# wei-zeng98/piano-a2s

Measured on AMD Instinct MI355X. Metric: training clips/sec (12 s, 5-bar), higher is better.
Workload: dtype f32

## Files before the change

### include/a2s.h

```cpp
#ifndef A2S_H
#define A2S_H
#include <stddef.h>
#include <stdint.h>
#ifdef __cplusplus
extern "C" {
#endif

#define A2S_OK 0
#define A2S_ERR_ARG (-1)
#define A2S_ERR_HIP (-2)
#define A2S_ERR_WORKSPACE (-3)

const char* a2s_last_error(void);
int a2s_version(void);
long long a2s_launch_count(void);

int a2s_gemm_f32(void* stream, int M, int N, int K, float alpha, const float* A, long sAm, long sAk,
                 const float* B, long sBk, long sBn, float beta, float* C, long ldc, const float* bias, int act,
                 int batch, long bsA, long bsB, long bsC, int splitk, float* workspace, size_t workspace_bytes);
int a2s_gemm_f32_affine(void* stream, int M, int N, int K, float alpha, const float* A, long sAm, long sAk, const float* B, long sBk,
                        long sBn, float beta, float* C, long ldc, const float* bias, int act, int batch, long bsA, long bsB, long bsC,
                        int splitk, float* workspace, size_t workspace_bytes, const float* a_scale, const float* a_shift, int a_period,
                        const float* b_scale, const float* b_shift, int b_period);
int a2s_gemm_f32_bnstats(void* stream, int M, int N, int K, const float* A, long sAm, long sAk, const float* B, long sBk, long sBn, float* C, long ldc,
                         const float* y, const float* mean, const float* invstd, const float* scale, const float* shift, int period, float* partial);
int a2s_gemm_f32_affine_scaled(void* stream, int M, int N, int K, float alpha, const float* A, long sAm, long sAk, const float* B, long sBk,
                               long sBn, float beta, float* C, long ldc, const float* bias, int act, int batch, long bsA, long bsB, long bsC,
                               int splitk, float* workspace, size_t workspace_bytes, const float* a_scale, const float* a_shift, int a_period,
                               const float* b_scale, const float* b_shift, int b_period, const float* a_absmax, const float* b_absmax);
int a2s_gemm_f32_bnstats_scaled(void* stream, int M, int N, int K, const float* A, long sAm, long sAk, const float* B, long sBk, long sBn, float* C, long ldc,
                                const float* y, const float* mean, const float* invstd, const float* scale, const float* shift, int period, float* partial,
                                const float* a_absmax, const float* b_absmax);
int a2s_linear_dgrad_bnstats(void* stream, int M, int N, int K, const float* dz, long lda, const float* Wt, float* da, long ldc, const float* y,
                             const float* mean, const float* invstd, const float* scale, const float* shift, int period, float* partial,
                             const float* dz_absmax, const float* w_absmax, float* workspace, size_t workspace_bytes, float* da_absmax_out);
int a2s_linear_fwd(void* stream, int M, int N, int K, const float* y, long lda, const float* W, float* z, long ldc, const float* scale, const float* shift,
                   int period, const float* y_absmax, const float* w_absmax, float* workspace, size_t workspace_bytes);
int a2s_linear_fwd_eligible(int M, int N, int K, int period);
int a2s_linear_wgrad(void* stream, int M, int N, int K, const float* dz, long ldz, const float* y, long lda, float* G, long ldg, const float* scale,
                     const float* shift, int period, const float* dz_absmax, const float* y_absmax, float* workspace, size_t workspace_bytes);
size_t a2s_linear_wgrad_ws_bytes(int M, int K);
int a2s_linear_wgrad_eligible(int M, int N, int K, int period);
int a2s_tallk_wgrad(void* stream, int M, int Np, int K, const float* P, long ldp, const float* A, long lda, float* G, long ldg, int transposed, float* bias,
                    const float* p_absmax, const float* a_absmax, float* workspace, size_t workspace_bytes);
size_t a2s_tallk_wgrad_ws_bytes(int M, int Np, int K);
int a2s_tallk_wgrad_eligible(int M, int Np, int K, long ldp, long lda, long ldg, int transposed);
size_t a2s_linear_dgrad_ws_bytes(int N, int K);
int a2s_linear_dgrad_blocks(int M);
int a2s_linear_dgrad_eligible(int M, int N, int K, int period);
int a2s_absmax(void* stream, const float* x, long n, float* out);
int a2s_gemm_bnstats_blocks(int M, int period);
size_t a2s_gemm_workspace_bytes(int M, int N, int batch, int splitk);
int a2s_gemm_pick_splitk(int M, int N, int K, int batch);
void a2s_gemm_debug_tile(int cfg);
int a2s_debug_set(const char* key, int value);
int a2s_debug_get(const char* key);
int a2s_env_check(void);
int a2s_persist_abort_latch(void* device_word);

int a2s_conv3x3(void* stream, const float* x, const float* w, float* y, const float* in_scale, const float* in_shift,
                float* stat_partial, int B, int T, int F, int Cin, int Cout, int flip, float* workspace);
int a2s_conv3x3_ranged(void* stream, const float* x, const float* w, float* y, const float* in_scale, const float* in_shift, const float* in_absmax,
                       float* stat_partial, float* out_absmax, int B, int T, int F, int Cin, int Cout, float* workspace);
int a2s_conv3x3_stat_blocks(int B, int T, int F, int Cin);
int a2s_conv3x3_dgrad_bnstats(void* stream, const float* dy, const float* w, float* g, const float* yl, const float* yl_mean, const float* yl_invstd,
                              const float* yl_scale, const float* yl_shift, float* stat_partial, int B, int T, int F, int Cin, int Cout,
                              float* workspace);
int a2s_bn_bwd_from_partial(void* stream, const float* g, const float* x, const float* mean, const float* invstd, const float* scale, const float* shift,
                            float* dgamma, float* dbeta, float* dx , const float* partial, int nblocks, float* c12, long rows, int C, int F);
int a2s_conv3x3_dgrad_bnstats_scaled(void* stream, const float* dy, const float* w, float* g, const float* yl, const float* yl_mean, const float* yl_invstd,
                                     const float* yl_scale, const float* yl_shift, float* stat_partial, int B, int T, int F, int Cin, int Cout,
                                     float* workspace, const float* dy_absmax);
int a2s_conv3x3_dgrad_bnstats_ranged(void* stream, const float* dy, const float* w, float* g, const float* yl, const float* yl_mean, const float* yl_invstd,
                                     const float* yl_scale, const float* yl_shift, float* stat_partial, int B, int T, int F, int Cin, int Cout,
                                     float* workspace, const float* dy_absmax, float* g_absmax_out);
int a2s_bn_bwd_from_partial_amax(void* stream, const float* g, const float* x, const float* mean, const float* invstd, const float* scale, const float* shift,
                                 float* dgamma, float* dbeta, float* dx, const float* partial, int nblocks, float* c12, long rows, int C, int F,
                                 float* dx_absmax);
size_t a2s_conv3x3_workspace_floats(int Cin);
int a2s_bn_finalize(void* stream, const float* partial, int nblocks, int C, double count, const float* gamma,
                    const float* beta, float* running_mean, float* running_var, long long* num_batches_tracked,
                    float* mean, float* invstd, float* scale, float* shift, float eps, float momentum, int training);
int a2s_bn_relu_apply(void* stream, const float* x, float* y, const float* scale, const float* shift, long n, int C, int F);
int a2s_col_stats(void* stream, const float* x, float* partial, long rows, int C, int rows_per_block);
int a2s_bn1d_relu_dropout(void* stream, const float* x, float* y, const float* scale, const float* shift,
                          const uint8_t* keep_mask, float inv_keep, long n, int C);

int a2s_gru_gates_fwd(void* stream, const float* gi, long ldgi, const float* gh, long ldgh, const float* hprev, long ldhp,
                      float* hout, long ldho, float* hout2, long ldho2, float* save, int R, int H);
int a2s_gru_seq_fwd(void* stream, const float* gi_all, long gi_bstride, long gi_tstride, const float* w_hh,
                    const float* b_hh, float* out, long out_bstride, long out_tstride, float* hbuf, float* gh,
                    float* save, float* hn, int B, int T, int H, int reverse, float* workspace, size_t workspace_bytes);

int a2s_attn_step_fwd(void* stream, const float* keys, const float* enc, const float* q, long ldq, const float* v,
                      float* ctx, long ldctx, float* ctx2, long ldctx2, float* attw, int B, int T, int H,
                      const int* n_done, int n_rows_total, float* workspace);
int a2s_attn_step_fwd_rows(void* stream, const float* keys, const float* enc, const float* q, long ldq, const float* v, float* ctx,
                           long ldctx, float* ctx2, long ldctx2, float* attw, int R, int T, int H, float* workspace, int n_clips,
                           const int* clip_order, const int* clip_rank, const int* row_until, int n_active, int step);
size_t a2s_attn_workspace_floats(int B, int T, int H);
size_t a2s_attn_workspace_floats_fused(int n_clips, int T, int H, int groups);

int a2s_log_softmax_rows(void* stream, const float* x, long ldx, float* y, long ldy, int* argmax_out, int R, int V);
int a2s_embed_rows(void* stream, const float* table, const long long* ids64, const int* ids32, long id_stride,
                   int const_id, float* out, long ldo, int col0, int R, int E, const uint8_t* keep_mask, float inv_keep);

typedef struct a2s_note_dec_args {
    const float* attn_w; const float* attn_b; const float* attn_v;
    const float* w_ih; const float* w_hh; const float* b_ih; const float* b_hh;
    const float* out_w; const float* out_b; const float* emb;
    const float* keys; const float* enc;
    float* h; float* x; float* q; float* gates; float* attw; float* o;
    float* gh; float* gi; float* logits;
    float* probs; long probs_bstride;
    const long long* gt; long gt_bstride;
    const uint8_t* tf_flags;
    const uint8_t* drop; float inv_keep;
    int* argmax_out; long am_bstride;
    int* eos_seen; long long* lengths; int* n_done;
    int* steps_exec;
    float* attn_ws;
    float* gemm_ws; size_t gemm_ws_bytes;
    int* t_base;
    const int* clip_order;
    const int* clip_rank;
    const int* row_until;
    const int* n_active;
    int n_clips;
    const int* m_active;
    const int* row_list;
    const int* n_rows_active;
    int R, T, H, E, V, steps, poll, eos_id;
    int use_graph;
    float* step_ws; size_t step_ws_floats;
    const int* tf_flags_dev;
    float* persist_ws; size_t persist_ws_bytes;
} a2s_note_dec_args;
int a2s_note_decoder_fwd(void* stream, const a2s_note_dec_args* args, int* steps_done);
int a2s_grammar_argmax_rows(void* stream, const float* x, long ldx, float* y, long ldy, const signed char* next_state, int n_states, int* row_state,
                            int* choice_out, int R, int V);
int a2s_note_decoder_fwd_grammar(void* stream, const a2s_note_dec_args* args, const signed char* next_state, int n_states, int* row_state, int* steps_done);
int a2s_grammar_launches(void);
#define A2S_BEAM_MAX 4
typedef struct a2s_beam_args {
    int K; float alpha;
    const signed char* next_state; int n_states;
    int pad_id;
    int* row_state;
    float* score; int* finished;
    int* done_count;
    int* token_hist; int* parent_hist; float* score_hist;
    float* probs_scratch;
    int* ids_out; long long* lengths_out; float* score_out;
} a2s_beam_args;
int a2s_note_decoder_fwd_beam(void* stream, const a2s_note_dec_args* args, const a2s_beam_args* beam, int* steps_done);
int a2s_beam_step(void* stream, const a2s_beam_args* beam, const float* logits, long ldl, const float* emb, float* xnext, long ldx, float* h, int h_cols,
                  float* q, int q_cols, int* n_done, int* steps_exec, int B, int V, int E, int t, int max_steps, int eos_id);
int a2s_beam_backtrack(void* stream, const a2s_beam_args* beam, float* probs, long probs_bstride, const int* steps_exec, int B, int V, int max_steps, int eos_id);
int a2s_beam_launches(void);
typedef struct a2s_align_args {
    float* attw_step;
    int* peak; float* weight; float* centroid;
    long out_stride;
    const signed char* next_state; int n_states;
    int* row_state;
} a2s_align_args;
int a2s_attn_align_rows(void* stream, const float* attw, long ldw, int R, int T, int* peak_out, float* weight_out, float* centroid_out, long out_stride);
int a2s_note_decoder_fwd_align(void* stream, const a2s_note_dec_args* args, const a2s_align_args* align, int* steps_done);
int a2s_align_launches(void);

int a2s_render_notes(void* stream, const int* programs, int rows_per_clip, int n_samples, float* wave, long wave_bstride, int B);
int a2s_render_launches(void);

int a2s_transpose_targets(void* stream, const int* new_key, const int* interval, const int* token_map, int n_rows, int V, const int* semitones,
                          const float* detune, long long* key, long long* upper, long long* lower, int bars, int U, int L, int bins_per_semitone,
                          float* eff_bins, int* counters, int B);
int a2s_shift_bins(void* stream, const float* x, float* y, const float* eff_bins, int B, int rows, int F);
int a2s_augment_launches(void);

int a2s_tempo_plan(void* stream, const float* x, int B, int rows, int F, const float* u, float R, int min_frames, int* content, int* step,
                   int* counters);
int a2s_stretch_frames(void* stream, const float* x, float* y, const int* step, int B, int rows, int F);
int a2s_tempo_launches(void);

int a2s_specaug_plan(void* stream, const float* x, int B, int rows, int F, const float* table, const unsigned* draws, int Wt, int Wf, int m,
                     int* content, int* plan, float* stats, int* counters);
int a2s_specaug_apply(void* stream, const float* x, float* y, const float* table, const int* content, const int* plan, const float* stats, int B,
                      int rows, int F);
int a2s_specaug_launches(void);

int a2s_room_ir(void* stream, const unsigned* room_seed, const int* params, int B, float* ir, long ir_bstride, int L_max);
int a2s_fir_rows(void* stream, const float* x, long x_bstride, const float* ir, long ir_bstride, const int* params, float* y, long y_bstride, int B,
                 int n_samples, int L_max);
int a2s_fir_tile_samples(void);
int a2s_fir_tap_chunk(void);
int a2s_room_launches(void);

int a2s_resample_rows(void* stream, const float* x, long x_bstride, const int* n_in, int n_in_max, int C, const float* table, int L, int M, int K, int Hh,
                      float* y, long y_bstride, int n_out_max, int B);
int a2s_resample_tile_samples(void);
int a2s_resample_launches(void);
int a2s_note_decoder_fwd_pair(void* stream_upper, void* stream_lower, const a2s_note_dec_args* upper, const a2s_note_dec_args* lower,
                              const int* pair_order, const int* pair_rank, const int* pair_n_active, int* steps_done_upper, int* steps_done_lower);
size_t a2s_note_step_workspace_floats(int H, int E);
size_t a2s_note_decoder_persist_ws_bytes(int n_clips, int R, int steps);
size_t a2s_note_decoder_bwd_persist_ws_bytes(int n_clips);

int a2s_staff_emb_fwd(void* stream, const float* note_emb, const float* const* gru_w, const long long* ids64,
                      const int* ids32, long id_bstride, const long long* lengths, long len_stride, float* out,
                      long ldo, int col0, float* hsave, int R, int maxlen, int E, int S);


int a2s_log_softmax_bwd_rows(void* stream, const float* g, const float* y, long outer_stride, int inner, float* dx,
                             int R, int V, int n_outer, int time_major);
int a2s_gru_gates_bwd(void* stream, const float* dh_a, long lda, const float* dh_b, long ldb, const float* save,
                      const float* hprev, long ldhp, float* dgi, long ldgi, float* dgh, long ldgh, float* dgh2, long ldgh2,
                      float* dhprev, long lddp, int R, int H);
int a2s_attn_step_bwd(void* stream, const float* keys, const float* enc, const float* q, long ldq, const float* v,
                      const float* attw, const float* ctx, long ldctx, const float* dctx_a, long ldda, const float* dctx_b,
                      long lddb, float* dctx_out, long lddo, float* dq, long lddq, float* ds_out, int B, int T, int H, float* workspace);
int a2s_attn_step_bwd_rows(void* stream, const float* keys, const float* enc, const float* q, long ldq, const float* v, const float* attw,
                           const float* ctx, long ldctx, const float* dctx_a, long ldda, const float* dctx_b, long lddb, float* dctx_out,
                           long lddo, float* dq, long lddq, float* ds_out, int R, int T, int H, float* workspace, int n_clips,
                           const int* clip_order, const int* clip_rank, const int* row_until, int n_active, int step);
int a2s_attn_dk_accum(void* stream, const float* keys, const float* q_all, const float* ds_all, const float* v, float* dK,
                      float* dv_partial, int B, int T, int S, int H, const int* row_until, int groups);
int a2s_attn_dk_blocks(int B, int T);
int a2s_attn_denc_accum(void* stream, const float* attw_all, const float* dctx_all, float* dEnc, int B, int T, int S, int H2,
                        const int* row_until, int groups);
int a2s_col_sum(void* stream, const float* x, long ld, float* out, long rows, int C, float alpha, float beta, float* workspace, size_t workspace_floats);
int a2s_embed_scatter_add(void* stream, float* table_grad, const long long* ids64, const int* ids32, long id_stride,
                          int const_id, const float* g, long ldg, int col0, int R, int E, const uint8_t* keep_mask, float inv_keep);
int a2s_ew_act_bwd(void* stream, const float* g, const float* y, float* dx, long n, int act);

typedef struct a2s_note_dec_bwd_args {
    const float* attn_w; const float* attn_v; const float* w_ih; const float* w_hh;
    const float* keys; const float* enc;
    const float* h; const float* x; const float* q; const float* gates; const float* attw;
    const float* do_all;
    float* dgi_all; float* dgh_all; float* dq_all; float* ds_all; float* dctx_all; float* dx;
    float* dh;
    float* attn_ws;
    float* gemm_ws; size_t gemm_ws_bytes;
    const int* clip_order;
    const int* clip_rank;
    const int* row_until;
    const int* n_active;
    int n_clips;
    const int* m_active;
    const int* row_list;
    const int* n_rows_active;
    int R, T, H, E, steps;
    float* step_ws; size_t step_ws_floats;
    float* persist_ws; size_t persist_ws_bytes;
    const float* w_ih_full;
} a2s_note_dec_bwd_args;
int a2s_note_decoder_bwd(void* stream, const a2s_note_dec_bwd_args* args);
int a2s_note_decoder_bwd_pair(void* stream_upper, void* stream_lower, const a2s_note_dec_bwd_args* upper, const a2s_note_dec_bwd_args* lower,
                              const int* pair_order, const int* pair_rank, const int* pair_n_active);

int a2s_gru_seq_bwd(void* stream, const float* dout, long do_bstride, long do_tstride, const float* out, long out_bstride,
                    long out_tstride, const float* gates, const float* w_hh, const float* dhn, float* dgi_all, float* dgh_shift,
                    float* dgh_first, float* dhbuf, float* dgh_tmp, int B, int T, int H, int reverse, float* workspace, size_t workspace_bytes);
int a2s_gru_seq_bwd_ranged(void* stream, const float* dout, long do_bstride, long do_tstride, const float* out, long out_bstride,
                           long out_tstride, const float* gates, const float* w_hh, const float* dhn, float* dgi_all, float* dgh_shift,
                           float* dgh_first, float* dhbuf, float* dgh_tmp, int B, int T, int H, int reverse, float* workspace, size_t workspace_bytes,
                           float* ranges_out, int* ranges_valid);
int a2s_staff_emb_bwd(void* stream, const float* note_emb, const float* const* gru_w, float* const* grads, float* note_emb_grad,
                      const long long* ids64, const int* ids32, long id_bstride, const long long* lengths, long len_stride,
                      const float* dout, long lddo, int col0, const float* hsave, int R, int maxlen, int E, int S);

int a2s_bn_bwd(void* stream, const float* g, const float* x, const float* mean, const float* invstd, const float* scale,
               const float* shift, const uint8_t* keep_mask, float inv_keep, float* dgamma, float* dbeta, float* dx,
               float* partial, float* c12, long rows, int C, int F);
int a2s_bn_bwd_amax(void* stream, const float* g, const float* x, const float* mean, const float* invstd, const float* scale,
                    const float* shift, const uint8_t* keep_mask, float inv_keep, float* dgamma, float* dbeta, float* dx,
                    float* partial, float* c12, long rows, int C, int F, float* dx_absmax);
size_t a2s_bn_bwd_partial_floats(long rows, int C, int F);
int a2s_bn_bwd_stats(void* stream, const float* g, const float* x, const float* mean, const float* invstd, const float* scale,
                     const float* shift, const uint8_t* keep_mask, float inv_keep, float* partial, float* sums, long rows, int C, int F);
int a2s_bn_bwd_apply(void* stream, const float* g, const float* x, const float* mean, const float* invstd, const float* scale,
                     const float* shift, const uint8_t* keep_mask, float inv_keep, const float* sums_local, const float* sums_global,
                     double count_global, float* dgamma, float* dbeta, float* dx, float* c12, long rows, int C, int F);
int a2s_bn_bwd_sums_from_partial(void* stream, const float* partial, int nblocks, int C, float* sums);
int a2s_bn_bwd_c12_from_sums(void* stream, const float* sums_local, const float* sums_global, double count_global, float* dgamma, float* dbeta,
                             float* c12, int C);
int a2s_conv3x3_wgrad(void* stream, const float* dy, const float* x, const float* in_scale, const float* in_shift, float* dW,
                      float* workspace, size_t workspace_bytes, int B, int T, int F, int Cin, int Cout);
int a2s_conv3x3_wgrad_scaled(void* stream, const float* dy, const float* x, const float* in_scale, const float* in_shift, float* dW,
                             float* workspace, size_t workspace_bytes, int B, int T, int F, int Cin, int Cout, const float* dy_absmax);
int a2s_conv3x3_wgrad_ranged(void* stream, const float* dy, const float* x, const float* in_scale, const float* in_shift, float* dW, float* workspace,
                             size_t workspace_bytes, int B, int T, int F, int Cin, int Cout, const float* dy_absmax, const float* act_absmax);
int a2s_act_bound(void* stream, const float* scale, const float* shift, const float* absmax, int C, float* out);
size_t a2s_conv3x3_wgrad_workspace_bytes(int Cin, int Cout);
int a2s_conv3x3_wgrad_bn(void* stream, const float* g, const float* y, const float* mean, const float* invstd, const float* scale, const float* shift,
                         const float* c12, float* dy_out, const float* x, const float* in_scale, const float* in_shift, float* dW, float* workspace,
                         size_t workspace_bytes, int B, int T, int F, int Cin, int Cout);
int a2s_conv3x3_wgrad_bn_ranged(void* stream, const float* g, const float* y, const float* mean, const float* invstd, const float* scale, const float* shift,
                                const float* c12, const float* g_absmax, int g_absmax_n, const float* y_absmax, float* dy_out, float* dy_absmax_out, const float* x,
                                const float* in_scale, const float* in_shift, float* dW, float* workspace, size_t workspace_bytes, int B, int T, int F,
                                int Cin, int Cout, const float* act_absmax);
int a2s_conv3x3_wgrad_bn_ranged_eligible(int F, int Cin, int Cout);

int a2s_nll_loss(void* stream, const float* logp, const long long* target, long rows, int V, long long ignore_index,
                 float* loss_out, float* dlogp, float gscale, double* partial, int nblocks);
int a2s_nll_grad(void* stream, float* dlogp, const long long* target, const float* loss_out, float gscale, long rows, int V,
                 long long ignore_index);
int a2s_clip_adadelta(void* stream, float* params, float* grads, float* square_avg, float* acc_delta, long n, const float* loss,
                      float max_norm, float lr, float rho, float eps, float* ctl, double* partial, int nblocks, int zero_grad);

int a2s_vqt_logmag(void* stream, const float* C, float* out, float* partial, int B, long rows, int bins, float top_db);
int a2s_vqt_logmag_octaves(void* stream, const float* C, float* out, float* partial, int B, long rows, int bins, int bins_per_octave, float top_db);
int a2s_vqt_decimate(void* stream, const float* ypad, long padded_len, const float* taps, int ntaps, float* out, long n_out, int B);

int a2s_edit_distance(void* stream, const int* ref, const long long* ref_off, const int* hyp, const long long* hyp_off, const int* order,
                      int n_pairs, int max_ref_len, int max_hyp_len, int* dist);
int a2s_edit_distance_max_len(void);

#define A2S_NOTE_CLS_OTHER 0
#define A2S_NOTE_CLS_TAB 1
#define A2S_NOTE_CLS_NL 2
#define A2S_NOTE_CLS_FERM 3
#define A2S_NOTE_CLS_CLOSE 4
#define A2S_NOTE_CLS_EOS 5
#define A2S_NOTE_CLS_IGNORE 6
#define A2S_NOTE_MIDI_REST (-2)
int a2s_note_match(void* stream, const int* ref, const long long* ref_off, const int* hyp, const long long* hyp_off, int n_pairs,
                   const int* dur_ticks, const int* midi, const int* cls, int V, int* out);
int a2s_note_match_max_len(void);
long a2s_note_match_launches(void);

#ifdef __cplusplus
}
#endif
#endif
```

### piano_a2s_amd/csrc/a2s_api.hip

```cpp
#define A2S_SWITCHES_IMPL
#include "a2s_internal.h"

thread_local char a2s_err_msg[512] = {0};
long long a2s_launch_counter = 0;

#define ST ((hipStream_t)stream)

extern "C" {

const char* a2s_last_error(void) { return a2s_err_msg; }
int a2s_version(void) { return 1; }
long long a2s_launch_count(void) { return __atomic_load_n(&a2s_launch_counter, __ATOMIC_RELAXED); }

int a2s_gemm_f32(void* stream, int M, int N, int K, float alpha, const float* A, long sAm, long sAk, const float* B, long sBk,
                 long sBn, float beta, float* C, long ldc, const float* bias, int act, int batch, long bsA, long bsB, long bsC,
                 int splitk, float* workspace, size_t workspace_bytes) {
    return a2s_gemm_impl(ST, M, N, K, alpha, A, sAm, sAk, B, sBk, sBn, beta, C, ldc, bias, act, batch, bsA, bsB, bsC, splitk,
                         workspace, workspace_bytes);
}
int a2s_gemm_f32_affine(void* stream, int M, int N, int K, float alpha, const float* A, long sAm, long sAk, const float* B, long sBk,
                        long sBn, float beta, float* C, long ldc, const float* bias, int act, int batch, long bsA, long bsB, long bsC,
                        int splitk, float* workspace, size_t workspace_bytes, const float* a_scale, const float* a_shift, int a_period,
                        const float* b_scale, const float* b_shift, int b_period) {
    return a2s_gemm_affine_impl(ST, M, N, K, alpha, A, sAm, sAk, B, sBk, sBn, beta, C, ldc, bias, act, batch, bsA, bsB, bsC, splitk,
                                workspace, workspace_bytes, a_scale, a_shift, a_period, b_scale, b_shift, b_period,
                                nullptr, nullptr, nullptr, nullptr, nullptr, nullptr, 0, 0, nullptr, nullptr);
}
int a2s_gemm_f32_affine_scaled(void* stream, int M, int N, int K, float alpha, const float* A, long sAm, long sAk, const float* B, long sBk,
                               long sBn, float beta, float* C, long ldc, const float* bias, int act, int batch, long bsA, long bsB, long bsC,
                               int splitk, float* workspace, size_t workspace_bytes, const float* a_scale, const float* a_shift, int a_period,
                               const float* b_scale, const float* b_shift, int b_period, const float* a_absmax, const float* b_absmax) {
    return a2s_gemm_affine_impl(ST, M, N, K, alpha, A, sAm, sAk, B, sBk, sBn, beta, C, ldc, bias, act, batch, bsA, bsB, bsC, splitk,
                                workspace, workspace_bytes, a_scale, a_shift, a_period, b_scale, b_shift, b_period,
                                nullptr, nullptr, nullptr, nullptr, nullptr, nullptr, 0, 1, a_absmax, b_absmax);
}
int a2s_gemm_f32_bnstats_scaled(void* stream, int M, int N, int K, const float* A, long sAm, long sAk, const float* B, long sBk, long sBn, float* C, long ldc,
                                const float* y, const float* mean, const float* invstd, const float* scale, const float* shift, int period, float* partial,
                                const float* a_absmax, const float* b_absmax) {
    return a2s_gemm_affine_impl(ST, M, N, K, 1.f, A, sAm, sAk, B, sBk, sBn, 0.f, C, ldc, nullptr, 0, 1, 0, 0, 0, 1, nullptr, 0,
                                nullptr, nullptr, 0, nullptr, nullptr, 0, y, mean, invstd, scale, shift, partial, period, 1, a_absmax, b_absmax);
}
int a2s_absmax(void* stream, const float* x, long n, float* out) { return a2s_absmax_impl(ST, x, n, out); }
int a2s_linear_dgrad_bnstats(void* stream, int M, int N, int K, const float* dz, long lda, const float* Wt, float* da, long ldc, const float* y,
                             const float* mean, const float* invstd, const float* scale, const float* shift, int period, float* partial,
                             const float* dz_absmax, const float* w_absmax, float* workspace, size_t workspace_bytes, float* da_absmax_out) {
    return a2s_linear_dgrad_bnstats_impl(ST, M, N, K, dz, lda, Wt, 1, K, da, ldc, y, mean, invstd, scale, shift, period, partial, dz_absmax, w_absmax,
                                         workspace, workspace_bytes, da_absmax_out);
}
size_t a2s_linear_dgrad_ws_bytes(int N, int K) { return a2s_linear_dgrad_ws_bytes_impl(N, K); }
int a2s_linear_fwd(void* stream, int M, int N, int K, const float* y, long lda, const float* W, float* z, long ldc, const float* scale, const float* shift,
                   int period, const float* y_absmax, const float* w_absmax, float* workspace, size_t workspace_bytes) {
    return a2s_linear_fwd_impl(ST, M, N, K, y, lda, W, z, ldc, scale, shift, period, y_absmax, w_absmax, workspace, workspace_bytes);
}
int a2s_linear_wgrad(void* stream, int M, int N, int K, const float* dz, long ldz, const float* y, long lda, float* G, long ldg, const float* scale,
                     const float* shift, int period, const float* dz_absmax, const float* y_absmax, float* workspace, size_t workspace_bytes) {
    return a2s_linear_wgrad_impl(ST, M, N, K, dz, ldz, y, lda, G, ldg, scale, shift, period, dz_absmax, y_absmax, workspace, workspace_bytes);
}
size_t a2s_linear_wgrad_ws_bytes(int M, int K) { return a2s_linear_wgrad_ws_bytes_impl(M, K); }
int a2s_linear_wgrad_eligible(int M, int N, int K, int period) { return a2s_linear_wgrad_ok(M, N, K, 256, 4, 4, period, nullptr, nullptr, nullptr) ? 1 : 0; }
int a2s_tallk_wgrad(void* stream, int M, int Np, int K, const float* P, long ldp, const float* A, long lda, float* G, long ldg, int transposed, float* bias,
                    const float* p_absmax, const float* a_absmax, float* workspace, size_t workspace_bytes) {
    return a2s_tallk_wgrad_impl(ST, M, Np, K, P, ldp, A, lda, G, ldg, transposed, bias, p_absmax, a_absmax, workspace, workspace_bytes);
}
size_t a2s_tallk_wgrad_ws_bytes(int M, int Np, int K) { return a2s_tallk_wgrad_ws_bytes_impl(M, Np, K); }
int a2s_tallk_wgrad_eligible(int M, int Np, int K, long ldp, long lda, long ldg, int transposed) {
    return a2s_tallk_wgrad_ok(M, Np, K, ldp, lda, ldg, transposed, nullptr, nullptr, nullptr, nullptr) ? 1 : 0;
}
int a2s_linear_fwd_eligible(int M, int N, int K, int period) { return a2s_linear_fwd_ok(M, N, K, 4, 4, period, nullptr, nullptr, nullptr) ? 1 : 0; }
int a2s_linear_dgrad_blocks(int M) { return a2s_linear_dgrad_blocks_impl(M); }
int a2s_linear_dgrad_eligible(int M, int N, int K, int period) {
    return a2s_linear_dgrad_ok(M, N, K, 4, 1, K, 4, period, nullptr, nullptr, nullptr, nullptr) ? 1 : 0;
}
int a2s_gemm_f32_bnstats(void* stream, int M, int N, int K, const float* A, long sAm, long sAk, const float* B, long sBk, long sBn, float* C, long ldc,
                         const float* y, const float* mean, const float* invstd, const float* scale, const float* shift, int period, float* partial) {
    return a2s_gemm_affine_impl(ST, M, N, K, 1.f, A, sAm, sAk, B, sBk, sBn, 0.f, C, ldc, nullptr, 0, 1, 0, 0, 0, 1, nullptr, 0,
                                nullptr, nullptr, 0, nullptr, nullptr, 0, y, mean, invstd, scale, shift, partial, period, 0, nullptr, nullptr);
}
int a2s_gemm_bnstats_blocks(int M, int period) { return a2s_cdiv(M, 128) * a2s_gemm_bnstats_slots(period); }
size_t a2s_gemm_workspace_bytes(int M, int N, int batch, int splitk) { return a2s_gemm_workspace_bytes_impl(M, N, batch, splitk); }
int a2s_gemm_pick_splitk(int M, int N, int K, int batch) { return a2s_gemm_pick_splitk_impl(M, N, K, batch); }
void a2s_gemm_debug_tile(int cfg) { a2s_gemm_debug_tile_impl(cfg); }
size_t a2s_note_step_workspace_floats(int H, int E) { return a2s_note_step_workspace_floats_impl(H, E); }
int a2s_debug_set(const char* key, int value) {
    if (!key) return A2S_ERR_ARG;
    const int id = a2s_switch_find(key);
    if (id >= 0) { a2s_switch_store(id, value); return A2S_OK; }
    if (!strcmp(key, "attn_deferred_fast")) { a2s_attn_deferred_fast = value ? 1 : 0; return A2S_OK; }
    if (!strcmp(key, "tallk_wgrad")) { a2s_tallk_wgrad_on = value ? 1 : 0; return A2S_OK; }
    if (!strcmp(key, "tallk_wgrad_max_splits")) { a2s_tallk_wgrad_max_splits = value > 0 ? value : 0; return A2S_OK; }
    if (!strcmp(key, "gemm_tile")) { a2s_gemm_debug_tile_impl(value); return A2S_OK; }
    snprintf(a2s_err_msg, sizeof(a2s_err_msg), "a2s_debug_set: unknown key %s", key);
    return A2S_ERR_ARG;
}
int a2s_env_check(void) {
    if (const char* e = a2s_switch_env_error()) A2S_FAIL(A2S_ERR_ARG, "%s: expected a decimal number >= 0", e);
    return A2S_OK;
}

int a2s_persist_abort_latch(void* device_word) { a2s_persist_latch_set(device_word); return A2S_OK; }

int a2s_debug_get(const char* key) {
    if (!key) return -1;
    const int id = a2s_switch_find(key);
    if (id == A2S_SW_attn_pair_fused_rows) return a2s_attn_pair_fused_rows();
    if (id >= 0) return a2s_sw((a2s_switch)id);
    if (!strcmp(key, "attn_pair_launches")) return (int)a2s_attn_pair_launches();
    if (!strcmp(key, "attn_pair_bwd_launches")) return (int)a2s_attn_pair_bwd_launches();
    if (!strcmp(key, "attn_deferred_fast")) return a2s_attn_deferred_fast;
    if (!strcmp(key, "tallk_wgrad")) return a2s_tallk_wgrad_on;
    if (!strcmp(key, "tallk_wgrad_max_splits")) return a2s_tallk_wgrad_max_splits;
    if (!strcmp(key, "tallk_wgrad_launches")) return (int)a2s_tallk_wgrad_launches();
    if (!strcmp(key, "attn_dk_ahead_launches")) return (int)a2s_attn_dk_ahead_launches();
    if (!strcmp(key, "attn_denc_launches")) return (int)a2s_attn_denc_launches();
    if (!strcmp(key, "dec_mid_launches")) return a2s_dec_mid_launches();
    if (!strcmp(key, "dec_persist_launches")) return a2s_dec_persist_launches();
    if (!strcmp(key, "edit_distance_launches")) return (int)a2s_edit_distance_launches();
    if (!strcmp(key, "conv_rows16_c20_launches")) return (int)a2s_conv_rows16_c20_launches();
    if (!strcmp(key, "device_cus")) return a2s_device_geometry().cus;
    if (!strcmp(key, "device_xccs")) return a2s_device_geometry().xccs;
    return -1;
}

int a2s_conv3x3(void* stream, const float* x, const float* w, float* y, const float* in_scale, const float* in_shift,
                float* stat_partial, int B, int T, int F, int Cin, int Cout, int flip, float* workspace) {
    return a2s_conv3x3_impl(ST, x, w, y, in_scale, in_shift, stat_partial, B, T, F, Cin, Cout, flip, workspace, nullptr, nullptr, nullptr, nullptr, nullptr, nullptr,
                            nullptr, nullptr);
}
int a2s_conv3x3_ranged(void* stream, const float* x, const float* w, float* y, const float* in_scale, const float* in_shift, const float* in_absmax,
                       float* stat_partial, float* out_absmax, int B, int T, int F, int Cin, int Cout, float* workspace) {
    return a2s_conv3x3_impl(ST, x, w, y, in_scale, in_shift, stat_partial, B, T, F, Cin, Cout, 0, workspace, nullptr, nullptr, nullptr, nullptr, nullptr, nullptr,
                            in_absmax, out_absmax);
}
int a2s_conv3x3_dgrad_bnstats(void* stream, const float* dy, const float* w, float* g, const float* yl, const float* yl_mean, const float* yl_invstd,
                              const float* yl_scale, const float* yl_shift, float* stat_partial, int B, int T, int F, int Cin, int Cout,
                              float* workspace) {
    if (!yl) { snprintf(a2s_err_msg, sizeof(a2s_err_msg), "conv3x3_dgrad_bnstats: yl is required"); return A2S_ERR_ARG; }
    return a2s_conv3x3_impl(ST, dy, w, g, nullptr, nullptr, stat_partial, B, T, F, Cin, Cout, 1, workspace, yl, yl_mean, yl_invstd, yl_scale, yl_shift, nullptr, nullptr, nullptr);
}
int a2s_conv3x3_dgrad_bnstats_scaled(void* stream, const float* dy, const float* w, float* g, const float* yl, const float* yl_mean, const float* yl_invstd,
                                     const float* yl_scale, const float* yl_shift, float* stat_partial, int B, int T, int F, int Cin, int Cout,
                                     float* workspace, const float* dy_absmax) {
    if (!yl) { snprintf(a2s_err_msg, sizeof(a2s_err_msg), "conv3x3_dgrad_bnstats_scaled: yl is required"); return A2S_ERR_ARG; }
    return a2s_conv3x3_impl(ST, dy, w, g, nullptr, nullptr, stat_partial, B, T, F, Cin, Cout, 1, workspace, yl, yl_mean, yl_invstd, yl_scale, yl_shift, dy_absmax, nullptr, nullptr);
}
int a2s_conv3x3_dgrad_bnstats_ranged(void* stream, const float* dy, const float* w, float* g, const float* yl, const float* yl_mean, const float* yl_invstd,
                                     const float* yl_scale, const float* yl_shift, float* stat_partial, int B, int T, int F, int Cin, int Cout,
                                     float* workspace, const float* dy_absmax, float* g_absmax_out) {
    if (!yl) { snprintf(a2s_err_msg, sizeof(a2s_err_msg), "conv3x3_dgrad_bnstats_ranged: yl is required"); return A2S_ERR_ARG; }
    return a2s_conv3x3_impl(ST, dy, w, g, nullptr, nullptr, stat_partial, B, T, F, Cin, Cout, 1, workspace, yl, yl_mean, yl_invstd, yl_scale, yl_shift, dy_absmax, nullptr, g_absmax_out);
}
int a2s_bn_bwd_from_partial(void* stream, const float* g, const float* x, const float* mean, const float* invstd, const float* scale, const float* shift,
                            float* dgamma, float* dbeta, float* dx, const float* partial, int nblocks, float* c12, long rows, int C, int F) {
    return a2s_bn_bwd_from_partial_impl(ST, g, x, mean, invstd, scale, shift, dgamma, dbeta, dx, partial, nblocks, c12, rows, C, F, nullptr);
}
int a2s_bn_bwd_from_partial_amax(void* stream, const float* g, const float* x, const float* mean, const float* invstd, const float* scale, const float* shift,
                                 float* dgamma, float* dbeta, float* dx, const float* partial, int nblocks, float* c12, long rows, int C, int F,
                                 float* dx_absmax) {
    return a2s_bn_bwd_from_partial_impl(ST, g, x, mean, invstd, scale, shift, dgamma, dbeta, dx, partial, nblocks, c12, rows, C, F, dx_absmax);
}
size_t a2s_conv3x3_workspace_floats(int Cin) { return a2s_conv3x3_workspace_floats_impl(Cin); }
int a2s_conv3x3_stat_blocks(int B, int T, int F, int Cin) { return a2s_conv3x3_stat_blocks_impl(B, T, F, Cin); }
int a2s_bn_finalize(void* stream, const float* partial, int nblocks, int C, double count, const float* gamma, const float* beta,
                    float* running_mean, float* running_var, long long* nbt, float* mean, float* invstd, float* scale,
                    float* shift, float eps, float momentum, int training) {
    return a2s_bn_finalize_impl(ST, partial, nblocks, C, count, gamma, beta, running_mean, running_var, nbt, mean, invstd, scale,
                                shift, eps, momentum, training);
}
int a2s_bn_relu_apply(void* stream, const float* x, float* y, const float* scale, const float* shift, long n, int C, int F) {
    return a2s_bn_relu_apply_impl(ST, x, y, scale, shift, n, C, F);
}
int a2s_col_stats(void* stream, const float* x, float* partial, long rows, int C, int rows_per_block) {
    return a2s_col_stats_impl(ST, x, partial, rows, C, rows_per_block);
}
int a2s_bn1d_relu_dropout(void* stream, const float* x, float* y, const float* scale, const float* shift, const uint8_t* keep_mask,
                          float inv_keep, long n, int C) {
    return a2s_bn1d_relu_dropout_impl(ST, x, y, scale, shift, keep_mask, inv_keep, n, C);
}
int a2s_gru_gates_fwd(void* stream, const float* gi, long ldgi, const float* gh, long ldgh, const float* hprev, long ldhp,
                      float* hout, long ldho, float* hout2, long ldho2, float* save, int R, int H) {
    return a2s_gru_gates_fwd_impl(ST, gi, ldgi, gh, ldgh, hprev, ldhp, hout, ldho, hout2, ldho2, save, R, H);
}
int a2s_gru_seq_fwd(void* stream, const float* gi_all, long gi_bstride, long gi_tstride, const float* w_hh, const float* b_hh,
                    float* out, long out_bstride, long out_tstride, float* hbuf, float* gh, float* save, float* hn, int B, int T,
                    int H, int reverse, float* workspace, size_t workspace_bytes) {
    return a2s_gru_seq_fwd_impl(ST, gi_all, gi_bstride, gi_tstride, w_hh, b_hh, out, out_bstride, out_tstride, hbuf, gh, save, hn,
                                B, T, H, reverse, workspace, workspace_bytes);
}
int a2s_attn_step_fwd(void* stream, const float* keys, const float* enc, const float* q, long ldq, const float* v, float* ctx,
                      long ldctx, float* ctx2, long ldctx2, float* attw, int B, int T, int H, const int* n_done, int n_rows_total, float* workspace) {
    return a2s_attn_step_fwd_impl(ST, keys, enc, q, ldq, v, ctx, ldctx, ctx2, ldctx2, attw, B, T, H, n_done, n_rows_total, workspace, nullptr);
}
int a2s_attn_step_fwd_rows(void* stream, const float* keys, const float* enc, const float* q, long ldq, const float* v, float* ctx,
                           long ldctx, float* ctx2, long ldctx2, float* attw, int R, int T, int H, float* workspace, int n_clips,
                           const int* clip_order, const int* clip_rank, const int* row_until, int n_active, int step) {
    a2s_attn_rows rows = {clip_order, clip_rank, row_until, n_clips, n_active, step};
    return a2s_attn_step_fwd_impl(ST, keys, enc, q, ldq, v, ctx, ldctx, ctx2, ldctx2, attw, R, T, H, nullptr, 0, workspace, &rows);
}
size_t a2s_attn_workspace_floats(int B, int T, int H) { return a2s_attn_workspace_floats_impl(B, T, H, 1); }
size_t a2s_attn_workspace_floats_fused(int n_clips, int T, int H, int groups) { return a2s_attn_workspace_floats_impl(n_clips, T, H, groups); }
int a2s_log_softmax_rows(void* stream, const float* x, long ldx, float* y, long ldy, int* argmax_out, int R, int V) {
    return a2s_log_softmax_rows_impl(ST, x, ldx, y, ldy, argmax_out, R, V);
}
int a2s_embed_rows(void* stream, const float* table, const long long* ids64, const int* ids32, long id_stride, int const_id,
                   float* out, long ldo, int col0, int R, int E, const uint8_t* keep_mask, float inv_keep) {
    return a2s_embed_rows_impl(ST, table, ids64, ids32, id_stride, const_id, out, ldo, col0, R, E, keep_mask, inv_keep);
}
int a2s_note_decoder_fwd(void* stream, const a2s_note_dec_args* args, int* steps_done) {
    if (!args) { snprintf(a2s_err_msg, sizeof(a2s_err_msg), "note_decoder_fwd: null args"); return A2S_ERR_ARG; }
    return a2s_note_decoder_fwd_impl(ST, *args, steps_done);
}
int a2s_grammar_argmax_rows(void* stream, const float* x, long ldx, float* y, long ldy, const signed char* next_state, int n_states, int* row_state,
                            int* choice_out, int R, int V) {
    return a2s_grammar_argmax_rows_impl(ST, x, ldx, y, ldy, next_state, n_states, row_state, choice_out, R, V);
}
int a2s_note_decoder_fwd_grammar(void* stream, const a2s_note_dec_args* args, const signed char* next_state, int n_states, int* row_state, int* steps_done) {
    if (!args) { snprintf(a2s_err_msg, sizeof(a2s_err_msg), "note_decoder_fwd_grammar: null args"); return A2S_ERR_ARG; }
    const a2s_grammar_ref g = {next_state, n_states, row_state};
    return a2s_note_decoder_fwd_grammar_impl(ST, *args, g, steps_done);
}
int a2s_grammar_launches(void) { return a2s_grammar_launches_impl(); }
int a2s_note_decoder_fwd_beam(void* stream, const a2s_note_dec_args* args, const a2s_beam_args* beam, int* steps_done) {
    if (!args || !beam) { snprintf(a2s_err_msg, sizeof(a2s_err_msg), "note_decoder_fwd_beam: null args"); return A2S_ERR_ARG; }
    return a2s_note_decoder_fwd_beam_impl(ST, *args, *beam, steps_done);
}
int a2s_beam_step(void* stream, const a2s_beam_args* beam, const float* logits, long ldl, const float* emb, float* xnext, long ldx, float* h, int h_cols,
                  float* q, int q_cols, int* n_done, int* steps_exec, int B, int V, int E, int t, int max_steps, int eos_id) {
    if (!beam) { snprintf(a2s_err_msg, sizeof(a2s_err_msg), "beam_step: null args"); return A2S_ERR_ARG; }
    const a2s_beam_args& g = *beam;
    const BeamStepArgs a = {logits, ldl, emb, xnext, ldx, h, h_cols, q, q_cols, g.next_state, g.n_states, g.row_state, g.score, g.finished, g.done_count,
                            g.token_hist, g.parent_hist, g.score_hist, g.probs_scratch, n_done, steps_exec, B, g.K, V, E, t, max_steps, eos_id, g.pad_id};
    return a2s_beam_step_finalize_impl(ST, a);
}
int a2s_beam_backtrack(void* stream, const a2s_beam_args* beam, float* probs, long probs_bstride, const int* steps_exec, int B, int V, int max_steps, int eos_id) {
    if (!beam) { snprintf(a2s_err_msg, sizeof(a2s_err_msg), "beam_backtrack: null args"); return A2S_ERR_ARG; }
    const a2s_beam_args& g = *beam;
    const BeamBackArgs a = {g.score, g.token_hist, g.parent_hist, g.probs_scratch, probs, probs_bstride, g.ids_out, (long)max_steps, g.lengths_out, g.score_out,
                            steps_exec, g.alpha, B, g.K, V, max_steps, eos_id, g.pad_id};
    return a2s_beam_backtrack_impl(ST, a);
}
int a2s_beam_launches(void) { return a2s_beam_launches_impl(); }
int a2s_attn_align_rows(void* stream, const float* attw, long ldw, int R, int T, int* peak_out, float* weight_out, float* centroid_out, long out_stride) {
    return a2s_attn_align_rows_impl(ST, attw, ldw, R, T, peak_out, weight_out, centroid_out, out_stride);
}
int a2s_note_decoder_fwd_align(void* stream, const a2s_note_dec_args* args, const a2s_align_args* align, int* steps_done) {
    if (!args || !align) { snprintf(a2s_err_msg, sizeof(a2s_err_msg), "note_decoder_fwd_align: null args"); return A2S_ERR_ARG; }
    return a2s_note_decoder_fwd_align_impl(ST, *args, *align, steps_done);
}
int a2s_align_launches(void) { return a2s_align_launches_impl(); }
int a2s_render_notes(void* stream, const int* programs, int rows_per_clip, int n_samples, float* wave, long wave_bstride, int B) {
    return a2s_render_notes_impl(ST, programs, rows_per_clip, n_samples, wave, wave_bstride, B);
}
int a2s_render_launches(void) { return a2s_render_launches_impl(); }
int a2s_transpose_targets(void* stream, const int* new_key, const int* interval, const int* token_map, int n_rows, int V, const int* semitones,
                          const float* detune, long long* key, long long* upper, long long* lower, int bars, int U, int L, int bins_per_semitone,
                          float* eff_bins, int* counters, int B) {
    return a2s_transpose_targets_impl(ST, new_key, interval, token_map, n_rows, V, semitones, detune, key, upper, lower, bars, U, L, bins_per_semitone, eff_bins,
                                      counters, B);
}
int a2s_shift_bins(void* stream, const float* x, float* y, const float* eff_bins, int B, int rows, int F) {
    return a2s_shift_bins_impl(ST, x, y, eff_bins, B, rows, F);
}
int a2s_augment_launches(void) { return a2s_augment_launches_impl(); }
int a2s_tempo_plan(void* stream, const float* x, int B, int rows, int F, const float* u, float R, int min_frames, int* content, int* step,
                   int* counters) {
    return a2s_tempo_plan_impl(ST, x, B, rows, F, u, R, min_frames, content, step, counters);
}
int a2s_stretch_frames(void* stream, const float* x, float* y, const int* step, int B, int rows, int F) {
    return a2s_stretch_frames_impl(ST, x, y, step, B, rows, F);
}
int a2s_tempo_launches(void) { return a2s_tempo_launches_impl(); }
int a2s_specaug_plan(void* stream, const float* x, int B, int rows, int F, const float* table, const unsigned* draws, int Wt, int Wf, int m,
                     int* content, int* plan, float* stats, int* counters) {
    return a2s_specaug_plan_impl(ST, x, B, rows, F, table, draws, Wt, Wf, m, content, plan, stats, counters);
}
int a2s_specaug_apply(void* stream, const float* x, float* y, const float* table, const int* content, const int* plan, const float* stats, int B,
                      int rows, int F) {
    return a2s_specaug_apply_impl(ST, x, y, table, content, plan, stats, B, rows, F);
}
int a2s_specaug_launches(void) { return a2s_specaug_launches_impl(); }
int a2s_room_ir(void* stream, const unsigned* room_seed, const int* params, int B, float* ir, long ir_bstride, int L_max) {
    return a2s_room_ir_impl(ST, room_seed, params, B, ir, ir_bstride, L_max);
}
int a2s_fir_rows(void* stream, const float* x, long x_bstride, const float* ir, long ir_bstride, const int* params, float* y, long y_bstride, int B,
                 int n_samples, int L_max) {
    return a2s_fir_rows_impl(ST, x, x_bstride, ir, ir_bstride, params, y, y_bstride, B, n_samples, L_max);
}
int a2s_fir_tile_samples(void) { return a2s_fir_tile_samples_impl(); }
int a2s_fir_tap_chunk(void) { return a2s_fir_tap_chunk_impl(); }
int a2s_room_launches(void) { return a2s_room_launches_impl(); }
int a2s_resample_rows(void* stream, const float* x, long x_bstride, const int* n_in, int n_in_max, int C, const float* table, int L, int M, int K, int Hh,
                      float* y, long y_bstride, int n_out_max, int B) {
    return a2s_resample_rows_impl(ST, x, x_bstride, n_in, n_in_max, C, table, L, M, K, Hh, y, y_bstride, n_out_max, B);
}
int a2s_resample_tile_samples(void) { return a2s_resample_tile_samples_impl(); }
int a2s_resample_launches(void) { return a2s_resample_launches_impl(); }
int a2s_note_decoder_fwd_pair(void* stream_upper, void* stream_lower, const a2s_note_dec_args* upper, const a2s_note_dec_args* lower,
                              const int* pair_order, const int* pair_rank, const int* pair_n_active, int* steps_done_upper, int* steps_done_lower) {
    if (!upper || !lower) { snprintf(a2s_err_msg, sizeof(a2s_err_msg), "note_decoder_fwd_pair: null args"); return A2S_ERR_ARG; }
    return a2s_note_decoder_fwd_pair_impl((hipStream_t)stream_upper, (hipStream_t)stream_lower, *upper, *lower, pair_order, pair_rank, pair_n_active,
                                          steps_done_upper, steps_done_lower);
}
int a2s_staff_emb_fwd(void* stream, const float* note_emb, const float* const* gru_w, const long long* ids64, const int* ids32,
                      long id_bstride, const long long* lengths, long len_stride, float* out, long ldo, int col0, float* hsave,
                      int R, int maxlen, int E, int S) {
    if (!gru_w) { snprintf(a2s_err_msg, sizeof(a2s_err_msg), "staff_emb_fwd: null weight table"); return A2S_ERR_ARG; }
    return a2s_staff_emb_fwd_impl(ST, note_emb, gru_w, ids64, ids32, id_bstride, lengths, len_stride, out, ldo, col0, hsave, R,
                                  maxlen, E, S);
}

int a2s_log_softmax_bwd_rows(void* stream, const float* g, const float* y, long outer_stride, int inner, float* dx, int R, int V,
                             int n_outer, int time_major) {
    return a2s_log_softmax_bwd_rows_impl(ST, g, y, outer_stride, inner, dx, R, V, n_outer, time_major);
}
int a2s_gru_gates_bwd(void* stream, const float* dh_a, long lda, const float* dh_b, long ldb, const float* save, const float* hprev,
                      long ldhp, float* dgi, long ldgi, float* dgh, long ldgh, float* dgh2, long ldgh2, float* dhprev, long lddp, int R, int H) {
    return a2s_gru_gates_bwd_impl(ST, dh_a, lda, dh_b, ldb, save, hprev, ldhp, dgi, ldgi, dgh, ldgh, dgh2, ldgh2, dhprev, lddp, R, H);
}
int a2s_attn_step_bwd(void* stream, const float* keys, const float* enc, const float* q, long ldq, const float* v, const float* attw,
                      const float* ctx, long ldctx, const float* dctx_a, long ldda, const float* dctx_b, long lddb, float* dctx_out,
                      long lddo, float* dq, long lddq, float* ds_out, int B, int T, int H, float* workspace) {
    return a2s_attn_step_bwd_impl(ST, keys, enc, q, ldq, v, attw, ctx, ldctx, dctx_a, ldda, dctx_b, lddb, dctx_out, lddo, dq, lddq, ds_out, B, T, H, workspace, nullptr);
}
int a2s_attn_step_bwd_rows(void* stream, const float* keys, const float* enc, const float* q, long ldq, const float* v, const float* attw,
                           const float* ctx, long ldctx, const float* dctx_a, long ldda, const float* dctx_b, long lddb, float* dctx_out,
                           long lddo, float* dq, long lddq, float* ds_out, int R, int T, int H, float* workspace, int n_clips,
                           const int* clip_order, const int* clip_rank, const int* row_until, int n_active, int step) {
    a2s_attn_rows rows = {clip_order, clip_rank, row_until, n_clips, n_active, step};
    return a2s_attn_step_bwd_impl(ST, keys, enc, q, ldq, v, attw, ctx, ldctx, dctx_a, ldda, dctx_b, lddb, dctx_out, lddo, dq, lddq, ds_out, R, T, H, workspace, &rows);
}
int a2s_attn_dk_accum(void* stream, const float* keys, const float* q_all, const float* ds_all, const float* v, float* dK,
                      float* dv_partial, int B, int T, int S, int H, const int* row_until, int groups) {
    return a2s_attn_dk_accum_impl(ST, keys, q_all, ds_all, v, dK, dv_partial, B, T, S, H, row_until, groups);
}
int a2s_attn_dk_blocks(int B, int T) { return B * ((T + 15) / 16); }
int a2s_attn_denc_accum(void* stream, const float* attw_all, const float* dctx_all, float* dEnc, int B, int T, int S, int H2,
                        const int* row_until, int groups) {
    return a2s_attn_denc_accum_impl(ST, attw_all, dctx_all, dEnc, B, T, S, H2, row_until, groups);
}
int a2s_col_sum(void* stream, const float* x, long ld, float* out, long rows, int C, float alpha, float beta, float* workspace, size_t workspace_floats) {
    return a2s_col_sum_impl(ST, x, ld, out, rows, C, alpha, beta, workspace, workspace_floats);
}
int a2s_embed_scatter_add(void* stream, float* table_grad, const long long* ids64, const int* ids32, long id_stride, int const_id,
                          const float* g, long ldg, int col0, int R, int E, const uint8_t* keep_mask, float inv_keep) {
    return a2s_embed_scatter_add_impl(ST, table_grad, ids64, ids32, id_stride, const_id, g, ldg, col0, R, E, keep_mask, inv_keep);
}
int a2s_ew_act_bwd(void* stream, const float* g, const float* y, float* dx, long n, int act) { return a2s_ew_act_bwd_impl(ST, g, y, dx, n, act); }
int a2s_note_decoder_bwd(void* stream, const a2s_note_dec_bwd_args* args) {
    if (!args) { snprintf(a2s_err_msg, sizeof(a2s_err_msg), "note_decoder_bwd: null args"); return A2S_ERR_ARG; }
    return a2s_note_decoder_bwd_impl(ST, *args);
}
int a2s_note_decoder_bwd_pair(void* stream_upper, void* stream_lower, const a2s_note_dec_bwd_args* upper, const a2s_note_dec_bwd_args* lower,
                              const int* pair_order, const int* pair_rank, const int* pair_n_active) {
    if (!upper || !lower) { snprintf(a2s_err_msg, sizeof(a2s_err_msg), "note_decoder_bwd_pair: null args"); return A2S_ERR_ARG; }
    return a2s_note_decoder_bwd_pair_impl((hipStream_t)stream_upper, (hipStream_t)stream_lower, *upper, *lower, pair_order, pair_rank, pair_n_active);
}
int a2s_gru_seq_bwd(void* stream, const float* dout, long do_bstride, long do_tstride, const float* out, long out_bstride, long out_tstride,
                    const float* gates, const float* w_hh, const float* dhn, float* dgi_all, float* dgh_shift, float* dgh_first,
                    float* dhbuf, float* dgh_tmp, int B, int T, int H, int reverse, float* workspace, size_t workspace_bytes) {
    return a2s_gru_seq_bwd_impl(ST, dout, do_bstride, do_tstride, out, out_bstride, out_tstride, gates, w_hh, dhn, dgi_all, dgh_shift,
                                dgh_first, dhbuf, dgh_tmp, B, T, H, reverse, workspace, workspace_bytes, nullptr, nullptr);
}
int a2s_gru_seq_bwd_ranged(void* stream, const float* dout, long do_bstride, long do_tstride, const float* out, long out_bstride, long out_tstride,
                           const float* gates, const float* w_hh, const float* dhn, float* dgi_all, float* dgh_shift, float* dgh_first,
                           float* dhbuf, float* dgh_tmp, int B, int T, int H, int reverse, float* workspace, size_t workspace_bytes,
                           float* ranges_out, int* ranges_valid) {
    if (!ranges_out || !ranges_valid) { snprintf(a2s_err_msg, sizeof(a2s_err_msg), "gru_seq_bwd_ranged: null ranges_out / ranges_valid"); return A2S_ERR_ARG; }
    return a2s_gru_seq_bwd_impl(ST, dout, do_bstride, do_tstride, out, out_bstride, out_tstride, gates, w_hh, dhn, dgi_all, dgh_shift,
                                dgh_first, dhbuf, dgh_tmp, B, T, H, reverse, workspace, workspace_bytes, ranges_out, ranges_valid);
}
int a2s_staff_emb_bwd(void* stream, const float* note_emb, const float* const* gru_w, float* const* grads, float* note_emb_grad,
                      const long long* ids64, const int* ids32, long id_bstride, const long long* lengths, long len_stride,
                      const float* dout, long lddo, int col0, const float* hsave, int R, int maxlen, int E, int S) {
    if (!gru_w) { snprintf(a2s_err_msg, sizeof(a2s_err_msg), "staff_emb_bwd: null weight table"); return A2S_ERR_ARG; }
    return a2s_staff_emb_bwd_impl(ST, note_emb, gru_w, grads, note_emb_grad, ids64, ids32, id_bstride, lengths, len_stride, dout, lddo,
                                  col0, hsave, R, maxlen, E, S);
}

int a2s_bn_bwd(void* stream, const float* g, const float* x, const float* mean, const float* invstd, const float* scale, const float* shift,
               const uint8_t* keep_mask, float inv_keep, float* dgamma, float* dbeta, float* dx, float* partial, float* c12, long rows, int C, int F) {
    return a2s_bn_bwd_impl(ST, g, x, mean, invstd, scale, shift, keep_mask, inv_keep, dgamma, dbeta, dx, partial, c12, rows, C, F, nullptr);
}
int a2s_bn_bwd_amax(void* stream, const float* g, const float* x, const float* mean, const float* invstd, const float* scale, const float* shift,
                    const uint8_t* keep_mask, float inv_keep, float* dgamma, float* dbeta, float* dx, float* partial, float* c12, long rows, int C, int F,
                    float* dx_absmax) {
    return a2s_bn_bwd_impl(ST, g, x, mean, invstd, scale, shift, keep_mask, inv_keep, dgamma, dbeta, dx, partial, c12, rows, C, F, dx_absmax);
}
size_t a2s_bn_bwd_partial_floats(long rows, int C, int F) { return a2s_bn_bwd_partial_floats_impl(rows, C, F); }
int a2s_conv3x3_wgrad(void* stream, const float* dy, const float* x, const float* in_scale, const float* in_shift, float* dW, float* workspace,
                      size_t workspace_bytes, int B, int T, int F, int Cin, int Cout) {
    return a2s_conv3x3_wgrad_impl(ST, dy, x, in_scale, in_shift, dW, workspace, workspace_bytes, B, T, F, Cin, Cout, nullptr, nullptr, nullptr, nullptr,
                                  nullptr, nullptr, nullptr, nullptr, nullptr);
}
int a2s_conv3x3_wgrad_ranged(void* stream, const float* dy, const float* x, const float* in_scale, const float* in_shift, float* dW, float* workspace,
                             size_t workspace_bytes, int B, int T, int F, int Cin, int Cout, const float* dy_absmax, const float* act_absmax) {
    return a2s_conv3x3_wgrad_impl(ST, dy, x, in_scale, in_shift, dW, workspace, workspace_bytes, B, T, F, Cin, Cout, nullptr, nullptr, nullptr, nullptr,
                                  nullptr, nullptr, nullptr, dy_absmax, act_absmax);
}
int a2s_act_bound(void* stream, const float* scale, const float* shift, const float* absmax, int C, float* out) {
    return a2s_act_bound_impl(ST, scale, shift, absmax, C, out);
}
int a2s_conv3x3_wgrad_scaled(void* stream, const float* dy, const float* x, const float* in_scale, const float* in_shift, float* dW, float* workspace,
                             size_t workspace_bytes, int B, int T, int F, int Cin, int Cout, const float* dy_absmax) {
    return a2s_conv3x3_wgrad_impl(ST, dy, x, in_scale, in_shift, dW, workspace, workspace_bytes, B, T, F, Cin, Cout, nullptr, nullptr, nullptr, nullptr,
                                  nullptr, nullptr, nullptr, dy_absmax, nullptr);
}
int a2s_conv3x3_wgrad_bn(void* stream, const float* g, const float* y, const float* mean, const float* invstd, const float* scale, const float* shift,
                         const float* c12, float* dy_out, const float* x, const float* in_scale, const float* in_shift, float* dW, float* workspace,
                         size_t workspace_bytes, int B, int T, int F, int Cin, int Cout) {
    if (!y) { snprintf(a2s_err_msg, sizeof(a2s_err_msg), "conv3x3_wgrad_bn: y is required"); return A2S_ERR_ARG; }
    return a2s_conv3x3_wgrad_impl(ST, g, x, in_scale, in_shift, dW, workspace, workspace_bytes, B, T, F, Cin, Cout, y, mean, invstd, scale, shift, c12, dy_out, nullptr, nullptr);
}
size_t a2s_conv3x3_wgrad_workspace_bytes(int Cin, int Cout) { return a2s_conv3x3_wgrad_workspace_bytes_impl(Cin, Cout); }
int a2s_conv3x3_wgrad_bn_ranged_eligible(int F, int Cin, int Cout) { return (a2s_wgrad_rows_eligible(F, Cin, Cout) && !(Cin == 40 && Cout == 20)) ? 1 : 0; }
// ... 64 lines not shown
```

### piano_a2s_amd/csrc/a2s_internal.h

```cpp
#pragma once
#include "a2s_common.h"
#include "../../include/a2s.h"
#include "a2s_switches.h"

static inline int a2s_attn_pair_fused_rows(void) {
    const int cap = a2s_sw(A2S_SW_dec_fused_max_rows), v = a2s_sw(A2S_SW_attn_pair_fused_rows);
    return v < cap ? v : cap;
}
static inline unsigned a2s_persist_dbg(void) {
    return (a2s_sw(A2S_SW_persist_force_agent) ? PERSIST_DBG_FORCE_AGENT : 0u) | (a2s_sw(A2S_SW_persist_inject_abort) ? PERSIST_DBG_INJECT_ABORT : 0u);
}

int a2s_absmax_impl(hipStream_t st, const float* x, long n, float* out);
size_t a2s_gemm_workspace_bytes_impl(int M, int N, int batch, int splitk);
int a2s_gemm_pick_splitk_impl(int M, int N, int K, int batch);
int a2s_gemm_bnstats_slots(int period);
void a2s_gemm_debug_tile_impl(int cfg);
int a2s_gemm_affine_impl(hipStream_t st, int M, int N, int K, float alpha, const float* A, long sAm, long sAk,
    const float* B, long sBk, long sBn, float beta, float* C, long ldc, const float* bias, int act,
    int batch, long bsA, long bsB, long bsC, int splitk, float* ws, size_t ws_bytes,
    const float* a_scale, const float* a_shift, int a_period, const float* b_scale, const float* b_shift, int b_period,
    const float* ep_y, const float* ep_mean, const float* ep_invstd, const float* ep_scale, const float* ep_shift,
    float* ep_partial, int ep_period, int two_term, const float* a_absmax, const float* b_absmax);
int a2s_gemm_impl(hipStream_t st, int M, int N, int K, float alpha, const float* A, long sAm, long sAk,
    const float* B, long sBk, long sBn, float beta, float* C, long ldc, const float* bias, int act,
    int batch, long bsA, long bsB, long bsC, int splitk, float* ws, size_t ws_bytes);

size_t a2s_linear_dgrad_ws_bytes_impl(int N, int K);
int a2s_linear_dgrad_blocks_impl(int M);
bool a2s_linear_dgrad_ok(int M, int N, int K, long lda, long sBk, long sBn, long ldc, int period, const void* A, const void* B, const void* C, const void* y);
int a2s_linear_dgrad_bnstats_impl(hipStream_t st, int M, int N, int K, const float* A, long lda, const float* Wt, long sBk, long sBn, float* C, long ldc,
    const float* ep_y, const float* mean, const float* invstd, const float* scale, const float* shift, int period,
    float* partial, const float* a_absmax, const float* b_absmax, float* ws, size_t ws_bytes, float* c_absmax_out);
bool a2s_linear_fwd_ok(int M, int N, int K, long lda, long ldc, int period, const void* A, const void* W, const void* C);
int a2s_linear_fwd_impl(hipStream_t st, int M, int N, int K, const float* A, long lda, const float* W, float* C, long ldc, const float* a_scale,
    const float* a_shift, int period, const float* a_absmax, const float* w_absmax, float* ws, size_t ws_bytes);
size_t a2s_linear_wgrad_ws_bytes_impl(int M, int K);
bool a2s_linear_wgrad_ok(int M, int N, int K, long ldz, long lda, long ldg, int period, const void* dz, const void* A, const void* G);
int a2s_linear_wgrad_impl(hipStream_t st, int M, int N, int K, const float* dz, long ldz, const float* A, long lda, float* G, long ldg, const float* a_scale,
    const float* a_shift, int period, const float* dz_absmax, const float* a_absmax, float* ws, size_t ws_bytes);
extern int a2s_tallk_wgrad_on;
extern int a2s_tallk_wgrad_max_splits;
long a2s_tallk_wgrad_launches(void);
size_t a2s_tallk_wgrad_ws_bytes_impl(int M, int Np, int K);
bool a2s_tallk_wgrad_ok(int M, int Np, int K, long ldp, long lda, long ldg, int transposed, const void* P, const void* A, const void* G, const void* bias);
int a2s_tallk_wgrad_impl(hipStream_t st, int M, int Np, int K, const float* P, long ldp, const float* A, long lda, float* G, long ldg, int transposed,
    float* bias, const float* p_absmax, const float* a_absmax, float* ws, size_t ws_bytes);

int a2s_act_bound_impl(hipStream_t st, const float* scale, const float* shift, const float* absmax, int C, float* out);
size_t a2s_conv3x3_workspace_floats_impl(int Cin);
int a2s_conv3x3_impl(hipStream_t st, const float* x, const float* w, float* y, const float* in_scale,
    const float* in_shift, float* stat_partial, int B, int T, int F, int Cin, int Cout, int flip, float* ws,
    const float* yl, const float* yl_mean, const float* yl_invstd, const float* yl_scale, const float* yl_shift,
    const float* x_absmax, const float* in_absmax, float* out_absmax);
int a2s_conv3x3_stat_blocks_impl(int B, int T, int F, int Cin);
int a2s_bn_finalize_impl(hipStream_t st, const float* partial, int nblocks, int C, double count, const float* gamma,
    const float* beta, float* running_mean, float* running_var, long long* nbt, float* mean,
    float* invstd, float* scale, float* shift, float eps, float momentum, int training);
int a2s_bn_relu_apply_impl(hipStream_t st, const float* x, float* y, const float* scale, const float* shift, long n, int C, int F);
int a2s_col_stats_impl(hipStream_t st, const float* x, float* partial, long rows, int C, int rows_per_block);
int a2s_bn1d_relu_dropout_impl(hipStream_t st, const float* x, float* y, const float* scale, const float* shift,
    const uint8_t* mask, float inv_keep, long n, int C);
size_t a2s_conv3x3_wgrad_workspace_bytes_impl(int Cin, int Cout);
int a2s_conv3x3_wgrad_impl(hipStream_t st, const float* dy, const float* x, const float* in_scale, const float* in_shift, float* dW,
    float* ws, size_t ws_bytes, int B, int T, int F, int Cin, int Cout, const float* bn_y, const float* bn_mean,
    const float* bn_invstd, const float* bn_scale, const float* bn_shift, const float* bn_c12, float* dy_out,
    const float* dy_absmax, const float* act_absmax);
int a2s_bn_bwd_impl(hipStream_t st, const float* g, const float* x, const float* mean, const float* invstd, const float* scale,
    const float* shift, const uint8_t* mask, float inv_keep, float* dgamma, float* dbeta, float* dx, float* partial,
    float* c12, long rows, int C, int F, float* dx_absmax);
int a2s_bn_bwd_from_partial_impl(hipStream_t st, const float* g, const float* x, const float* mean, const float* invstd, const float* scale,
    const float* shift, float* dgamma, float* dbeta, float* dx, const float* partial, int nblocks, float* c12,
    long rows, int C, int F, float* dx_absmax);
int a2s_bn_bwd_stats_impl(hipStream_t st, const float* g, const float* x, const float* mean, const float* invstd, const float* scale,
    const float* shift, const uint8_t* mask, float inv_keep, float* partial, float* sums, long rows, int C, int F);
int a2s_bn_bwd_apply_impl(hipStream_t st, const float* g, const float* x, const float* mean, const float* invstd, const float* scale,
    const float* shift, const uint8_t* mask, float inv_keep, const float* sums_local, const float* sums_global,
    double count_global, float* dgamma, float* dbeta, float* dx, float* c12, long rows, int C, int F);
int a2s_bn_bwd_sums_from_partial_impl(hipStream_t st, const float* partial, int nblocks, int C, float* sums);
int a2s_bn_bwd_c12_from_sums_impl(hipStream_t st, const float* sums_local, const float* sums_global, double count_global, float* dgamma, float* dbeta,
    float* c12, int C);
size_t a2s_bn_bwd_partial_floats_impl(long rows, int C, int F);

int a2s_channel_absmax_impl(hipStream_t st, const float* x, long rows, int C, int F, float* out);
bool a2s_conv_rows_eligible(int F, int Cin);
int a2s_conv_rows_blocks(int B, int T, int F);
size_t a2s_conv_rows_workspace_floats(int Cin);
long a2s_conv_rows16_c20_launches(void);
int a2s_conv3x3_rows_impl(hipStream_t st, const float* x, const float* w, float* y, const float* in_scale, const float* in_shift,
    const float* in_absmax, float* stat_partial, float* out_absmax, int B, int T, int F, int Cin, int Cout, int flip,
    float* ws, const float* yl, const float* yl_mean, const float* yl_invstd, const float* yl_scale, const float* yl_shift,
    const float* x_absmax);

bool a2s_wgrad_rows_eligible(int F, int Cin, int Cout);
int a2s_conv3x3_wgrad_rows_bn_impl(hipStream_t st, const float* g, const float* y, const float* mean, const float* invstd, const float* scale,
    const float* shift, const float* c12, const float* g_absmax, int g_absmax_n, const float* y_absmax, float* dz_out,
    float* dz_absmax_out, const float* x, const float* in_scale, const float* in_shift, float* dW, float* ws, size_t ws_bytes,
    int B, int T, int F, int Cin, int Cout, const float* act_absmax);
int a2s_conv3x3_wgrad_rows_impl(hipStream_t st, const float* dy, const float* x, const float* in_scale, const float* in_shift, float* dW, float* ws,
    size_t ws_bytes, int B, int T, int F, int Cin, int Cout, const float* dy_absmax, const float* act_absmax);

struct StepFinArgs {
    const float* logits; long ldl;
    float* probs; long probs_bstride;
    const long long* gt; long gt_bstride;
    const float* emb;
    float* xnext; long ldx;
    const uint8_t* drop; float inv_keep;
    int* argmax_out; long am_bstride;
    int* eos_seen; long long* lengths; int* n_done; int* steps_exec;
    const int* t_base;
    const int* row_until;
    int n_clips;
    int R, V, E, t, teacher_force, eos_id, max_t;
};
struct a2s_grammar_ref { const signed char* next; int n_states; int* row_state; };
int a2s_gru_gates_fwd_impl(hipStream_t st, const float* gi, long ldgi, const float* gh, long ldgh, const float* hprev,
    long ldhp, float* hout, long ldho, float* hout2, long ldho2, float* save, int R, int H);
int a2s_gru_bptt_step_impl(hipStream_t st, const float* dgh, const float* w_hh_t, const float* dhz_in, const float* dout, long ld_dout,
    const float* save, const float* hprev, long ld_hprev, float* dgi, long ld_dgi, float* dgh_out, float* dgh2,
    long ld_dgh2, float* dhz_out, int R, int H);
int a2s_skinny_gemm_acc_impl(hipStream_t st, const float* A, long lda, const float* Bt, long ldb, float* Cm, long ldc, int R, int N, int K);
int a2s_gru_seq_fwd_impl(hipStream_t st, const float* gi_all, long gi_bstride, long gi_tstride, const float* w_hh,
    const float* b_hh, float* out, long out_bstride, long out_tstride, float* hbuf, float* gh,
    float* save, float* hn, int B, int T, int H, int reverse, float* ws, size_t ws_bytes);
int a2s_attn_step_fwd_impl(hipStream_t st, const float* Kmat, const float* enc, const float* q, long ldq, const float* v,
    float* ctx, long ldctx, float* ctx2, long ldctx2, float* attw, int B, int T, int H,
    const int* n_done, int n_rows_total, float* ws, const a2s_attn_rows* rows = nullptr, a2s_attn_deferred* defer = nullptr);
int a2s_log_softmax_rows_impl(hipStream_t st, const float* x, long ldx, float* y, long ldy, int* argmax_out, int R, int V);
int a2s_embed_rows_impl(hipStream_t st, const float* table, const long long* ids64, const int* ids32, long id_stride,
    int const_id, float* out, long ldo, int col0, int R, int E, const uint8_t* drop, float inv_keep);
int a2s_note_decoder_fwd_impl(hipStream_t st, const a2s_note_dec_args& a, int* steps_done);
int a2s_note_decoder_fwd_grammar_impl(hipStream_t st, const a2s_note_dec_args& a, const a2s_grammar_ref& g, int* steps_done);
int a2s_note_decoder_fwd_pair_impl(hipStream_t su, hipStream_t sl, const a2s_note_dec_args& au, const a2s_note_dec_args& al, const int* pair_order,
    const int* pair_rank, const int* pair_n_active, int* done_u, int* done_l);
int a2s_staff_emb_fwd_impl(hipStream_t st, const float* note_emb, const float* const* w ,
    const long long* ids64, const int* ids32, long id_bstride, const long long* lengths,
    long len_stride, float* out, long ldo, int col0, float* hsave, int R, int maxlen, int E, int S);
int a2s_note_decoder_zero_unwritten(hipStream_t st, const a2s_note_dec_args& a, const char* who );
size_t a2s_attn_workspace_floats_impl(int B, int T, int H, int groups);
size_t a2s_attn_bulk_lds(size_t shm, int n_active, int backward);
long a2s_attn_pair_launches(void);
struct AttnPairStep { const int* clip_order; const int* clip_rank; int n_clips; int n_active; int step; int G; int chunk; };
int a2s_pair_events(const char* who, hipEvent_t** ev_out);
static inline int a2s_record_wait(hipEvent_t ev, hipStream_t from, hipStream_t to, const char* who) {
    hipError_t e = hipEventRecord(ev, from);
    if (e == hipSuccess) e = hipStreamWaitEvent(to, ev, 0);
    if (e != hipSuccess) A2S_FAIL(A2S_ERR_HIP, "%s: event: %s", who, hipGetErrorString(e));
    return A2S_OK;
}

int a2s_log_softmax_bwd_rows_impl(hipStream_t st, const float* g, const float* y, long outer_stride, int inner, float* dx,
    int R, int V, int n_outer, int time_major);
int a2s_gru_gates_bwd_impl(hipStream_t st, const float* dh_a, long lda, const float* dh_b, long ldb, const float* save,
    const float* hprev, long ldhp, float* dgi, long ldgi, float* dgh, long ldgh, float* dgh2, long ldgh2,
    float* dhprev, long lddp, int R, int H);
int a2s_attn_step_bwd_impl(hipStream_t st, const float* Kmat, const float* enc, const float* q, long ldq, const float* v,
    const float* attw, const float* ctx, long ldctx, const float* dctx_a, long ldda, const float* dctx_b,
    long lddb, float* dctx_out, long lddo, float* dq, long lddq, float* ds_out, int B, int T, int H, float* ws,
    const a2s_attn_rows* rows = nullptr);
int a2s_attn_dk_accum_impl(hipStream_t st, const float* Kmat, const float* q_all, const float* ds_all, const float* v,
    float* dK, float* dv_partial, int B, int T, int S, int H, const int* row_until, int groups);
int a2s_attn_denc_accum_impl(hipStream_t st, const float* attw_all, const float* dctx_all, float* dEnc, int B, int T, int S, int H2,
    const int* row_until, int groups);
long a2s_attn_dk_ahead_launches(void);
long a2s_attn_denc_launches(void);
int a2s_col_sum_impl(hipStream_t st, const float* x, long ld, float* out, long rows, int C, float alpha, float beta, float* ws, size_t ws_floats);
int a2s_embed_scatter_add_impl(hipStream_t st, float* table_grad, const long long* ids64, const int* ids32, long id_stride,
    int const_id, const float* g, long ldg, int col0, int R, int E, const uint8_t* drop, float inv_keep);
int a2s_ew_act_bwd_impl(hipStream_t st, const float* g, const float* y, float* dx, long n, int act);
int a2s_note_decoder_bwd_impl(hipStream_t st, const a2s_note_dec_bwd_args& a);
int a2s_note_decoder_bwd_pair_impl(hipStream_t su, hipStream_t sl, const a2s_note_dec_bwd_args& au, const a2s_note_dec_bwd_args& al, const int* pair_order,
    const int* pair_rank, const int* pair_n_active);
int a2s_gru_seq_bwd_impl(hipStream_t st, const float* dout, long do_bstride, long do_tstride, const float* out, long out_bstride,
    long out_tstride, const float* gates, const float* w_hh, const float* dhn, float* dgi_all, float* dgh_shift,
    float* dgh_first, float* dhbuf, float* dgh_tmp, int B, int T, int H, int reverse, float* ws, size_t ws_bytes,
    float* ranges_out, int* ranges_valid);
int a2s_staff_emb_bwd_impl(hipStream_t st, const float* note_emb, const float* const* w, float* const* grads_dev, float* note_emb_grad,
    const long long* ids64, const int* ids32, long id_bstride, const long long* lengths, long len_stride,
    const float* dout, long lddo, int col0, const float* hsave, int R, int maxlen, int E, int S);
long a2s_attn_pair_bwd_launches(void);

size_t a2s_note_step_fused_head_floats(void);
size_t a2s_note_step_workspace_floats_impl(int H, int E);
int a2s_dec_mid_launches(void);
bool a2s_dec_step_fusable(int R, int H, int E, int V, const void* const* ptrs, int nptrs, const float* ws, size_t ws_floats, bool greedy = false);
int a2s_note_step_fused_fwd(hipStream_t st, const a2s_note_dec_args& a, int si, int so, int sv, int sv_next, int t, const int* t_base, int tf, bool last,
    int nrows, const int* rowmap, const a2s_attn_deferred* defer = nullptr);
int a2s_note_step_fused_bwd_prepare(hipStream_t st, const a2s_note_dec_bwd_args& a);
int a2s_note_step_fused_bwd(hipStream_t st, const a2s_note_dec_bwd_args& a, int s, const float* dh_in, float* dh_out, const a2s_attn_rows* rows,
    int nrows, const int* rowmap);
bool a2s_note_step_mid_ok(int H, int E, const void* const* ptrs, int nptrs);
int a2s_note_step_mid_gru(hipStream_t st, const a2s_note_dec_args& a, int si, int so, int sv, int sv_next, int nrows, const int* rowmap);
bool a2s_note_step_mid_bwd_ok(const a2s_note_dec_bwd_args& a);
int a2s_note_step_mid_bwd(hipStream_t st, const a2s_note_dec_bwd_args& a, int s, float* dh_out, int nrows, const int* rowmap);
int a2s_note_step_mid_bwd_query(hipStream_t st, const a2s_note_dec_bwd_args& a, int s, float* dh_out, int nrows, const int* rowmap);

bool a2s_grammar_ref_ok(const a2s_grammar_ref& g, int R, int V);
int a2s_grammar_argmax_rows_impl(hipStream_t st, const float* x, long ldx, float* y, long ldy, const signed char* next, int n_states, int* row_state,
    int* choice_out, int R, int V);
int a2s_grammar_step_finalize_impl(hipStream_t st, const StepFinArgs& a, const a2s_grammar_ref& g);
int a2s_grammar_launches_impl(void);

int a2s_attn_align_rows_impl(hipStream_t st, const float* attw, long ldw, int R, int T, int* peak_out, float* weight_out, float* centroid_out,
    long out_stride, const int* n_done = nullptr, int n_rows_total = 0);
int a2s_align_launches_impl(void);
int a2s_note_decoder_fwd_align_impl(hipStream_t st, const a2s_note_dec_args& a, const a2s_align_args& g, int* steps_done);

int a2s_render_notes_impl(hipStream_t st, const int* programs, int rows_per_clip, int n_samples, float* wave, long wave_bstride, int B);
int a2s_render_launches_impl(void);

int a2s_transpose_targets_impl(hipStream_t st, const int* new_key, const int* interval, const int* token_map, int n_rows, int V, const int* semitones,
    const float* detune, long long* key, long long* upper, long long* lower, int bars, int U, int L, int bins_per_semitone, float* eff_bins, int* counters,
    int B);
int a2s_shift_bins_impl(hipStream_t st, const float* x, float* y, const float* eff_bins, int B, int rows, int F);
int a2s_augment_launches_impl(void);

#define A2S_ROW_TX 128
#define A2S_ROW_TY 2
#define A2S_ROW_TILE 16
#define A2S_ROW_NR (A2S_ROW_TILE / A2S_ROW_TY)
#ifdef __HIPCC__
template <int VEC> struct a2s_row_vec { typedef float type; };
template <> struct a2s_row_vec<4> { typedef f32x4 type; };
static inline int a2s_row_vec_width(int F, const void* y) { return (F % 4 == 0 && ((uintptr_t)y & 15) == 0) ? 4 : 1; }
static inline bool a2s_row_grid(int B, int rows, int F, int vec, dim3* grid) {
    *grid = dim3(a2s_cdiv(rows, A2S_ROW_TILE), B, a2s_cdiv(F, A2S_ROW_TX * vec));
    return grid->z <= 65535;
}
#define A2S_ROW_LAUNCH(kernel, vec, grid, st, ...)                                                                   \
    do {                                                                                                             \
        if ((vec) == 4) hipLaunchKernelGGL(kernel<4>, grid, dim3(A2S_ROW_TX, A2S_ROW_TY), 0, st, __VA_ARGS__);       \
        else hipLaunchKernelGGL(kernel<1>, grid, dim3(A2S_ROW_TX, A2S_ROW_TY), 0, st, __VA_ARGS__);                  \
    } while (0)
#endif

int a2s_tempo_plan_impl(hipStream_t st, const float* x, int B, int rows, int F, const float* u, float R, int min_frames, int* content, int* step,
    int* counters);
int a2s_stretch_frames_impl(hipStream_t st, const float* x, float* y, const int* step, int B, int rows, int F);
int a2s_tempo_launches_impl(void);

#define A2S_CONTENT_CHUNK 16
#ifdef __HIPCC__
template <int THREADS>
__device__ __forceinline__ int a2s_content_rows(const float* __restrict__ xb, int rows, int F, int* s_last) {
    const int tid = threadIdx.x;
    for (int r1 = rows; r1 > 0; r1 -= A2S_CONTENT_CHUNK) {
        const int r0 = r1 > A2S_CONTENT_CHUNK ? r1 - A2S_CONTENT_CHUNK : 0;
        const float* xc = xb + (long)r0 * F;
        const long len = (long)(r1 - r0) * F;
        long last = -1;
#pragma unroll 4
        for (long i = tid; i < len; i += THREADS)
            if (xc[i] != 0.0f) last = i;
        if (tid == 0) *s_last = -1;
        __syncthreads();
        if (last >= 0) atomicMax(s_last, (int)(last / F));
        __syncthreads();
        const int got = *s_last;
        __syncthreads();
        if (got >= 0) return r0 + got + 1;
    }
    return 0;
}
#endif

int a2s_specaug_plan_impl(hipStream_t st, const float* x, int B, int rows, int F, const float* table, const unsigned* draws, int Wt, int Wf, int m,
    int* content, int* plan, float* stats, int* counters);
int a2s_specaug_apply_impl(hipStream_t st, const float* x, float* y, const float* table, const int* content, const int* plan, const float* stats, int B,
    int rows, int F);
int a2s_specaug_launches_impl(void);

int a2s_room_ir_impl(hipStream_t st, const unsigned* room_seed, const int* params, int B, float* ir, long ir_bstride, int L_max);
int a2s_fir_rows_impl(hipStream_t st, const float* x, long x_bstride, const float* ir, long ir_bstride, const int* params, float* y, long y_bstride, int B,
                      int n_samples, int L_max);
int a2s_fir_tile_samples_impl(void);
int a2s_fir_tap_chunk_impl(void);
int a2s_room_launches_impl(void);

int a2s_resample_rows_impl(hipStream_t st, const float* x, long x_bstride, const int* n_in, int n_in_max, int C, const float* table, int L, int M, int K,
                           int Hh, float* y, long y_bstride, int n_out_max, int B);
int a2s_resample_tile_samples_impl(void);
int a2s_resample_launches_impl(void);

struct BeamStepArgs {
    const float* logits; long ldl;
    const float* emb;
    float* xnext; long ldx;
    float* h; int h_cols;
    float* q; int q_cols;
    const signed char* next; int n_states; int* row_state;
    float* score; int* finished; int* done_count;
    int* token_hist; int* parent_hist; float* score_hist;
    float* probs_scratch;
    int* n_done; int* steps_exec;
    int B, K, V, E, t, max_t, eos_id, pad_id;
};
struct BeamBackArgs {
    const float* score; const int* token_hist; const int* parent_hist; const float* probs_scratch;
    float* probs; long probs_bstride;
    int* ids_out; long ids_bstride; long long* lengths_out; float* score_out;
    const int* steps_exec;
    float alpha;
    int B, K, V, max_t, eos_id, pad_id;
};
bool a2s_beam_args_ok(const a2s_beam_args& g, int R, int n_clips, int V);
int a2s_beam_init_impl(hipStream_t st, const a2s_beam_args& g, int* n_done, int B, int steps);
int a2s_beam_step_finalize_impl(hipStream_t st, const BeamStepArgs& a);
int a2s_beam_backtrack_impl(hipStream_t st, const BeamBackArgs& a);
int a2s_beam_launches_impl(void);
int a2s_note_decoder_fwd_beam_impl(hipStream_t st, const a2s_note_dec_args& a, const a2s_beam_args& g, int* steps_done);

unsigned* a2s_persist_latch_ptr(void);
void a2s_persist_latch_set(void* p);
a2s_device_geom a2s_device_geometry(void);
bool a2s_gru_seq_fwd_persist_ok(const float* w_hh, const float* gi, int B, int T, int H, float* ws, size_t ws_bytes);
int a2s_gru_seq_fwd_persist_impl(hipStream_t st, const float* gi_all, long gi_bstride, long gi_tstride, const float* w_hh, const float* b_hh, float* out,
    long out_bstride, long out_tstride, float* save, float* hn, int B, int T, int H, int reverse, float* ws, size_t ws_bytes);
bool a2s_gru_seq_bwd_persist_ok(int B, int T, int H, float* ws, size_t ws_bytes, size_t ws_used);
int a2s_gru_seq_bwd_persist_impl(hipStream_t st, const float* dout, long do_bstride, long do_tstride, const float* out, long out_bstride, long out_tstride,
    const float* gates, const float* w_hh_t, const float* dhn, float* dgi_all, float* dgh_shift, float* dgh_first, int B, int T,
    int H, int reverse, float* ws, size_t ws_off, size_t ws_bytes, float* ranges_out);

int a2s_dec_persist_launches(void);
bool a2s_note_decoder_fwd_persist_ok(const a2s_note_dec_args& a);
int a2s_note_decoder_fwd_persist(hipStream_t st, const a2s_note_dec_args& a, int* steps_done);
bool a2s_note_decoder_bwd_persist_ok(const a2s_note_dec_bwd_args& a);
int a2s_note_decoder_bwd_persist(hipStream_t st, const a2s_note_dec_bwd_args& a);

int a2s_nll_loss_impl(hipStream_t st, const float* logp, const long long* target, long rows, int V, long long ignore_index,
    float* loss_out , float* dlogp , float gscale, double* partial, int nblocks);
int a2s_nll_grad_impl(hipStream_t st, float* dlogp, const long long* target, const float* loss_out, float gscale, long rows, int V, long long ignore_index);
int a2s_clip_adadelta_impl(hipStream_t st, float* params, float* grads, float* square_avg, float* acc_delta, long n, const float* loss,
    float max_norm, float lr, float rho, float eps, float* ctl , double* partial, int nblocks, int zero_grad);

int a2s_edit_distance_max_len_impl(void);
long a2s_edit_distance_launches(void);
int a2s_edit_distance_impl(hipStream_t st, const int* ref, const long long* ref_off, const int* hyp, const long long* hyp_off, const int* order,
    int n_pairs, int max_ref_len, int max_hyp_len, int* dist);

int a2s_note_match_max_len_impl(void);
long a2s_note_match_launches_impl(void);
int a2s_note_match_impl(hipStream_t st, const int* ref, const long long* ref_off, const int* hyp, const long long* hyp_off, int n_pairs,
    const int* dur_ticks, const int* midi, const int* cls, int V, int* out);

int a2s_vqt_logmag_impl(hipStream_t st, const float* C, float* out, float* partial, int B, long rows, int bins, float top_db);
int a2s_vqt_decimate_impl(hipStream_t st, const float* ypad, long plen, const float* taps, int ntaps, float* out, long n_out, int B);
int a2s_vqt_logmag_octaves_impl(hipStream_t st, const float* C, float* out, float* partial, int B, long rows, int bins, int bpo, float top_db);
```

### piano_a2s_amd/csrc/a2s_linear.hip

```cpp
#include "a2s_internal.h"

#define LIN_BM 128
#define LIN_K 256
#define LIN_RS 288
#define LIN_NTH 512
#define LIN_LDS (2 * 2 * LIN_BM * LIN_RS)

typedef unsigned lu32x4 __attribute__((ext_vector_type(4)));

struct LinDgradArgs {
    const float* A; long lda;
    const unsigned char* planes;
    float* C; long ldc;
    const float* ep_y;
    const float* mean; const float* invstd; const float* scale; const float* shift;
    float* partial;
    const float* a_absmax; const float* b_absmax;
    int M, N, period, channels;
    float* c_absmax_out;
};

__global__ __launch_bounds__(256) void lin_pack_planes_k(const float* __restrict__ W, long ld, int N, int K, const float* __restrict__ absmax,
                                                         unsigned char* __restrict__ out) {
    const long id = (long)blockIdx.x * 256 + threadIdx.x;
// ... 69 lines not shown
    if (wave * 32 < a.N) { load_b(wave * 32, 0, bf[0]); load_b(wave * 32, 1, bf[1]); }
    for (int j = 0; j < ntiles; ++j) {
        const int n0 = j * 256 + wave * 32;
        if (n0 >= a.N) break;
        f32x4 yq[8][2];
        auto load_y = [&](int mt) {
            const int m = m0 + mt * 16 + lr;
#pragma unroll
            for (int nt = 0; nt < 2; ++nt) {
#if defined(LIN_X) && LIN_X >= 1 && LIN_X != 4
                yq[mt][nt] = (f32x4){1.f, 1.f, 1.f, 1.f};
#else
                yq[mt][nt] = (f32x4){0.f, 0.f, 0.f, 0.f};
                if (m < a.M)
                    yq[mt][nt] = *reinterpret_cast<const f32x4*>(reinterpret_cast<const char*>(a.ep_y + (long)(m0 + mt * 16) * a.ldc + n0 + nt * 16) + lane_off);
#endif
            }
        };
#pragma unroll
        for (int mt = 0; mt < 3; ++mt) load_y(mt);
        f32x4 acc[8][2];
#pragma unroll
        for (int mt = 0; mt < 8; ++mt)
#pragma unroll
            for (int nt = 0; nt < 2; ++nt) acc[mt][nt] = (f32x4){0.f, 0.f, 0.f, 0.f};
#pragma unroll
        for (int ks = 0; ks < 8; ++ks) {
#if defined(LIN_X) && LIN_X >= 3
            if (ks + 2 < 8 && a.M < 0) load_b(n0, ks + 2, bf[(ks + 2) % 3]);
#else
            if (ks + 2 < 8) load_b(n0, ks + 2, bf[(ks + 2) % 3]);
#endif
#pragma unroll
            for (int half = 0; half < 2; ++half) {
                lu32x4 af[2][4];
#pragma unroll
                for (int sp = 0; sp < 2; ++sp)
#pragma unroll
                    for (int q = 0; q < 4; ++q)
                        af[sp][q] = *reinterpret_cast<const lu32x4*>(lds + (((ks >> 2) * 2 + sp) * LIN_BM + (half * 4 + q) * 16 + lr) * LIN_RS + (ks & 3) * 64 + lk * 16);
#define LIN_PRODUCT(SA, SB)                                                                                                   \
                _Pragma("unroll") for (int nt = 0; nt < 2; ++nt)                                                              \
                    _Pragma("unroll") for (int q = 0; q < 4; ++q)                                                             \
                        acc[half * 4 + q][nt] = __builtin_amdgcn_mfma_f32_16x16x32_f16(__builtin_bit_cast(f16x8, bf[ks % 3][nt][SB]), \
                                                                                       __builtin_bit_cast(f16x8, af[SA][q]), acc[half * 4 + q][nt], 0, 0, 0);
                LIN_PRODUCT(1, 0) LIN_PRODUCT(0, 1) LIN_PRODUCT(0, 0)
#undef LIN_PRODUCT
            }
        }
        if (n0 + 256 < a.N) { load_b(n0 + 256, 0, bf[0]); load_b(n0 + 256, 1, bf[1]); }
#pragma unroll
        for (int mt = 3; mt < 8; ++mt) load_y(mt);
        const int c = n0 / a.period;
        if (c != cur_c) { flush(); s1 = 0.f; s2 = 0.f; cur_c = c; }
        const float mean = a.mean[c], invstd = a.invstd[c], sc = a.scale[c], sh = a.shift[c];
#pragma unroll
        for (int mt = 0; mt < 8; ++mt) {
            const int m = m0 + mt * 16 + lr;
            if (m >= a.M) continue;
#pragma unroll
            for (int nt = 0; nt < 2; ++nt) {
                f32x4 v = acc[mt][nt];
#pragma unroll
                for (int r = 0; r < 4; ++r) { v[r] *= unscale; vmax = fmaxf(vmax, fabsf(v[r])); }
#if defined(LIN_X) && LIN_X >= 2
                if (v[0] == 123.456f)
#endif
                *reinterpret_cast<f32x4*>(reinterpret_cast<char*>(a.C + (long)(m0 + mt * 16) * a.ldc + n0 + nt * 16) + lane_off) = v;
#pragma unroll
                for (int r = 0; r < 4; ++r) {
                    const float gm = (fmaf(yq[mt][nt][r], sc, sh) > 0.f) ? v[r] : 0.f;
                    s1 += gm; s2 = fmaf(gm * (yq[mt][nt][r] - mean), invstd, s2);
                }
            }
        }
    }
    flush();
    if (a.c_absmax_out) {
        const float m = wave_max(vmax);
        if (lane == 0 && m > 0.f) atomicMax(reinterpret_cast<unsigned*>(a.c_absmax_out), __float_as_uint(m));
    }
}

size_t a2s_linear_dgrad_ws_bytes_impl(int N, int K) { return (K > 0 && K % 32 == 0 && N > 0) ? (size_t)N * K * 2 * 2 : 0; }
int a2s_linear_dgrad_blocks_impl(int M) { return M > 0 ? ((M + LIN_BM - 1) / LIN_BM) * 8 : 0; }

bool a2s_linear_dgrad_ok(int M, int N, int K, long lda, long sBk, long sBn, long ldc, int period, const void* A, const void* B, const void* C, const void* y) {
    return K == LIN_K && M >= LIN_BM && N >= 256 && N % 32 == 0 && period > 0 && period % 32 == 0 && N % period == 0 && N / period <= 4096 && sBk == 1 && sBn == K &&
           lda % 4 == 0 && ldc % 4 == 0 && (((uintptr_t)A | (uintptr_t)B | (uintptr_t)C | (uintptr_t)y) % 16 == 0);
}

int a2s_linear_dgrad_bnstats_impl(hipStream_t st, int M, int N, int K, const float* A, long lda, const float* Wt, long sBk, long sBn, float* C, long ldc,
                                  const float* ep_y, const float* mean, const float* invstd, const float* scale, const float* shift, int period,
                                  float* partial, const float* a_absmax, const float* b_absmax, float* ws, size_t ws_bytes, float* c_absmax_out) {
    A2S_REQUIRE(A && Wt && C && ep_y && mean && invstd && scale && shift && partial && a_absmax && b_absmax && ws, "linear_dgrad_bnstats: null argument");
    A2S_REQUIRE(a2s_linear_dgrad_ok(M, N, K, lda, sBk, sBn, ldc, period, A, Wt, C, ep_y),
                "linear_dgrad_bnstats: needs K = 256, M >= 128, N >= 256, N %% 32 == 0, period %% 32 == 0, a k-contiguous weight (N x K) and 16-byte aligned rows");
    A2S_REQUIRE(((uintptr_t)ws % 16 == 0) && ws_bytes >= a2s_linear_dgrad_ws_bytes_impl(N, K), "linear_dgrad_bnstats: workspace too small (%zu bytes needed)",
                a2s_linear_dgrad_ws_bytes_impl(N, K));
    const int channels = N / period, nblk = a2s_linear_dgrad_blocks_impl(M);
    hipError_t e = hipMemsetAsync(partial, 0, sizeof(float) * 2 * (size_t)nblk * channels, st);
    if (e != hipSuccess) A2S_FAIL(A2S_ERR_HIP, "linear_dgrad_bnstats memset: %s", hipGetErrorString(e));
    unsigned char* planes = reinterpret_cast<unsigned char*>(ws);
    hipLaunchKernelGGL(lin_pack_planes_k, dim3((unsigned)(((long)N * (K / 8) + 255) / 256)), dim3(256), 0, st, Wt, (long)K, N, K, b_absmax, planes);
    A2S_CHECK_LAUNCH("lin_pack_planes_k");
    LinDgradArgs a{A, lda, planes, C, ldc, ep_y, mean, invstd, scale, shift, partial, a_absmax, b_absmax, M, N, period, channels, c_absmax_out};
    hipLaunchKernelGGL(lin_dgrad_bnstats, dim3((M + LIN_BM - 1) / LIN_BM), dim3(LIN_NTH), 0, st, a);
    A2S_CHECK_LAUNCH("lin_dgrad_bnstats");
    return A2S_OK;
}

#define LF_RS 160
#define LF_STAGE (2 * LIN_BM * LF_RS)
#define LF_NS 3

struct LinFwdArgs {
    const float* A; long lda;
    const unsigned char* planes;
    float* C; long ldc;
    const float* a_scale; const float* a_shift;
    const float* a_absmax; const float* b_absmax;
    int M, K, period;
};

__global__ __launch_bounds__(LIN_NTH) void lin_fwd_roles(LinFwdArgs a) {
    __shared__ __attribute__((aligned(16))) unsigned char lds[LF_NS * LF_STAGE];
    const int tid = threadIdx.x, lane = tid & 63, lr = lane & 15, lk = lane >> 4;
    const int wave = __builtin_amdgcn_readfirstlane(tid >> 6);
    const int m0 = blockIdx.x * LIN_BM;
    const int ka = a.a_absmax ? pow2_scale_exp(*a.a_absmax, 12) : 0, kb = pow2_scale_exp(*a.b_absmax, 12);
    const float psa = ldexpf(1.f, ka), unscale = ldexpf(1.f, -(ka + kb));
    const int nks = a.K >> 5, nblk = a.K >> 6, kpc = a.period >> 5;
    const bool affine = a.a_scale != nullptr;
    if (wave >= 4) {
        const int st_ = tid - 256;
        const int sk = (st_ & 15) * 4;
        const bool second = sk >= 32;
        f32x4 ar[2][8];
        auto issue_a = [&](int blk, f32x4 (&r)[8]) {
#pragma unroll
            for (int i = 0; i < 8; ++i) {
                const int row = (st_ + 256 * i) >> 4;
                r[i] = (f32x4){0.f, 0.f, 0.f, 0.f};
                if (m0 + row < a.M && blk < nblk) r[i] = __builtin_nontemporal_load(reinterpret_cast<const f32x4*>(a.A + (long)(m0 + row) * a.lda + (long)blk * 64 + sk));
            }
        };
        auto commit_a = [&](int blk, const f32x4 (&r)[8]) {
            if (blk >= nblk) return;
            const int c0 = (2 * blk) / kpc, c1 = (2 * blk + 1) / kpc;
            const float sc = affine ? (second ? a.a_scale[c1] : a.a_scale[c0]) * psa : psa, sh = affine ? (second ? a.a_shift[c1] : a.a_shift[c0]) * psa : 0.f;
            const float floor_ = affine ? 0.f : -INFINITY;
            unsigned char* st = lds + (blk % LF_NS) * LF_STAGE;
#pragma unroll
            for (int i = 0; i < 8; ++i) {
                const int row = (st_ + 256 * i) >> 4;
                float x[4];
#pragma unroll
                for (int j = 0; j < 4; ++j) x[j] = __builtin_amdgcn_fmed3f(fmaxf(fmaf(r[i][j], sc, sh), floor_), -65000.f, 65000.f);
                uint2 hi, lo;
                split2_pair_f16(x[0], x[1], hi.x, lo.x);
                split2_pair_f16(x[2], x[3], hi.y, lo.y);
                *reinterpret_cast<uint2*>(st + (0 * LIN_BM + row) * LF_RS + sk * 2) = hi;
                *reinterpret_cast<uint2*>(st + (1 * LIN_BM + row) * LF_RS + sk * 2) = lo;
            }
        };
        issue_a(0, ar[0]);
        commit_a(0, ar[0]);
        issue_a(1, ar[1]); issue_a(2, ar[0]);
#pragma unroll 1
        for (int b0 = 0; b0 < nblk; b0 += 2) {
            __syncthreads();
            commit_a(b0 + 1, ar[1]); issue_a(b0 + 3, ar[1]);
            if (b0 + 1 < nblk) {
                __syncthreads();
                commit_a(b0 + 2, ar[0]); issue_a(b0 + 4, ar[0]);
            }
        }
        return;
    }
    lu32x4 bf[2][4][2];
    auto load_b = [&](int ks, lu32x4 (&dst)[4][2]) {
        if (ks >= nks) return;
#pragma unroll
        for (int nt = 0; nt < 4; ++nt)
#pragma unroll
            for (int sp = 0; sp < 2; ++sp)
                dst[nt][sp] = *reinterpret_cast<const lu32x4*>(a.planes + (((long)(wave * 4 + nt) * nks + ks) * 2 + sp) * 1024 + (unsigned)lane * 16u);
    };
    f32x4 acc[8][4];
#pragma unroll
    for (int mt = 0; mt < 8; ++mt)
#pragma unroll
        for (int nt = 0; nt < 4; ++nt) acc[mt][nt] = (f32x4){0.f, 0.f, 0.f, 0.f};
    load_b(0, bf[0]);
    auto load_af = [&](const unsigned char* st, int h, int qt, lu32x4 (&af)[2][2]) {
#pragma unroll
        for (int sp = 0; sp < 2; ++sp)
#pragma unroll
            for (int q = 0; q < 2; ++q) af[sp][q] = *reinterpret_cast<const lu32x4*>(st + (sp * LIN_BM + (qt * 2 + q) * 16 + lr) * LF_RS + h * 64 + lk * 16);
    };
    auto multiply = [&](int qt, const lu32x4 (&af)[2][2], const lu32x4 (&b)[4][2]) {
#define LR_PRODUCT(SA, SB)                                                                                                        \
        _Pragma("unroll") for (int nt = 0; nt < 4; ++nt)                                                                          \
            _Pragma("unroll") for (int q = 0; q < 2; ++q)                                                                         \
                acc[qt * 2 + q][nt] = __builtin_amdgcn_mfma_f32_16x16x32_f16(__builtin_bit_cast(f16x8, b[nt][SB]),                \
                                                                             __builtin_bit_cast(f16x8, af[SA][q]), acc[qt * 2 + q][nt], 0, 0, 0);
        LR_PRODUCT(1, 0) LR_PRODUCT(0, 1) LR_PRODUCT(0, 0)
#undef LR_PRODUCT
    };
#pragma unroll 1
    for (int blk = 0; blk < nblk; ++blk) {
        __syncthreads();
        const unsigned char* st = lds + (blk % LF_NS) * LF_STAGE;
        lu32x4 fa[2][2], fb[2][2];
        load_af(st, 0, 0, fa);
        load_b(2 * blk + 1, bf[1]);
        __builtin_amdgcn_sched_barrier(0);
        load_af(st, 0, 1, fb); multiply(0, fa, bf[0]);
        __builtin_amdgcn_sched_barrier(0);
        load_af(st, 0, 2, fa); multiply(1, fb, bf[0]);
        __builtin_amdgcn_sched_barrier(0);
        load_af(st, 0, 3, fb); multiply(2, fa, bf[0]);
        __builtin_amdgcn_sched_barrier(0);
        load_af(st, 1, 0, fa); multiply(3, fb, bf[0]);
        __builtin_amdgcn_sched_barrier(0);
        load_b(2 * blk + 2, bf[0]);
        load_af(st, 1, 1, fb); multiply(0, fa, bf[1]);
        __builtin_amdgcn_sched_barrier(0);
        load_af(st, 1, 2, fa); multiply(1, fb, bf[1]);
        __builtin_amdgcn_sched_barrier(0);
        load_af(st, 1, 3, fb); multiply(2, fa, bf[1]);
        __builtin_amdgcn_sched_barrier(0);
        multiply(3, fb, bf[1]);
        __builtin_amdgcn_sched_barrier(0);
    }
#pragma unroll
    for (int mt = 0; mt < 8; ++mt) {
        const int m = m0 + mt * 16 + lr;
        if (m >= a.M) continue;
#pragma unroll
        for (int nt = 0; nt < 4; ++nt) {
            f32x4 v = acc[mt][nt];
#pragma unroll
            for (int r = 0; r < 4; ++r) v[r] *= unscale;
            *reinterpret_cast<f32x4*>(a.C + (long)m * a.ldc + wave * 64 + nt * 16 + lk * 4) = v;
        }
    }
}

bool a2s_linear_fwd_ok(int M, int N, int K, long lda, long ldc, int period, const void* A, const void* W, const void* C) {
    return N == 256 && M >= 1 && K >= 128 && K % 64 == 0 && (period == 0 || (period % 32 == 0 && K % period == 0)) && lda % 4 == 0 && ldc % 4 == 0 &&
           (((uintptr_t)A | (uintptr_t)W | (uintptr_t)C) % 16 == 0);
}

int a2s_linear_fwd_impl(hipStream_t st, int M, int N, int K, const float* A, long lda, const float* W, float* C, long ldc, const float* a_scale,
                        const float* a_shift, int period, const float* a_absmax, const float* w_absmax, float* ws, size_t ws_bytes) {
    A2S_REQUIRE(A && W && C && w_absmax && ws && ((a_scale == nullptr) == (a_shift == nullptr)), "linear_fwd: null argument");
    A2S_REQUIRE(a2s_linear_fwd_ok(M, N, K, lda, ldc, a_scale ? period : 0, A, W, C),
                "linear_fwd: needs N = 256, K %% 64 == 0, period %% 32 == 0 and 16-byte aligned rows");
    A2S_REQUIRE(((uintptr_t)ws % 16 == 0) && ws_bytes >= (size_t)N * K * 4, "linear_fwd: workspace too small (%zu bytes needed)", (size_t)N * K * 4);
    unsigned char* planes = reinterpret_cast<unsigned char*>(ws);
    hipLaunchKernelGGL(lin_pack_planes_k, dim3((unsigned)(((long)N * (K / 8) + 255) / 256)), dim3(256), 0, st, W, (long)K, N, K, w_absmax, planes);
    A2S_CHECK_LAUNCH("lin_pack_planes_k");
    LinFwdArgs a{A, lda, planes, C, ldc, a_scale, a_shift, a_absmax, w_absmax, M, K, a_scale ? period : K};
    hipLaunchKernelGGL(lin_fwd_roles, dim3((M + LIN_BM - 1) / LIN_BM), dim3(LIN_NTH), 0, st, a);
    A2S_CHECK_LAUNCH("lin_fwd");
    return A2S_OK;
}

struct LinWgradArgs {
    const float* A; long lda;
    const unsigned char* planes;
    float* partial;
    const float* a_scale; const float* a_shift;
    const float* a_absmax; const float* d_absmax;
    int M, K, period, nblk, blk_per_split;
    long plane_stride; int np;
    float* bias_partial;
};

__global__ __launch_bounds__(256) void lin_pack_dz_planes(const float* __restrict__ dz, long ld, int M, int nsteps, const float* __restrict__ absmax,
                                                          unsigned char* __restrict__ out) {
    const long id = (long)blockIdx.x * 256 + threadIdx.x;
    const int n = (int)(id & 255), lk = (int)((id >> 8) & 3), s = (int)(id >> 10);
    if (s >= nsteps) return;
    dz += blockIdx.y * 256;
    out += (size_t)blockIdx.y * nsteps * (16 * 2 * 1024);
    float ps = ldexpf(1.f, pow2_scale_exp(*absmax, 12));
    if ((s >> 3) & 1) ps = -ps;
    float x[8];
#pragma unroll
    for (int j = 0; j < 8; ++j) {
        const int m = s * 32 + lk * 8 + j;
        x[j] = m < M ? __builtin_amdgcn_fmed3f(dz[(long)m * ld + n] * ps, -65000.f, 65000.f) : 0.f;
    }
    lu32x4 hi, lo;
#pragma unroll
    for (int i = 0; i < 4; ++i) { unsigned h, l; split2_pair_f16(x[2 * i], x[2 * i + 1], h, l); hi[i] = h; lo[i] = l; }
    unsigned char* o = out + ((((long)s * 16 + (n >> 4)) * 2) * 64 + (lk * 16 + (n & 15))) * 16;
    *reinterpret_cast<lu32x4*>(o) = hi;
    *reinterpret_cast<lu32x4*>(o + 64 * 16) = lo;
}

template <bool BIAS>
__global__ __launch_bounds__(LIN_NTH) void lin_wgrad_roles(LinWgradArgs a) {
    __shared__ __attribute__((aligned(16))) unsigned char lds[LF_NS * LF_STAGE];
    const int tid = threadIdx.x, lane = tid & 63, lr = lane & 15, lk = lane >> 4;
    const int wave = __builtin_amdgcn_readfirstlane(tid >> 6);
    const int k0 = blockIdx.x * LIN_BM;
    const int b_lo = blockIdx.y * a.blk_per_split, b_hi = min(a.nblk, b_lo + a.blk_per_split);
    const int ka = a.a_absmax ? pow2_scale_exp(*a.a_absmax, 12) : 0, kd = pow2_scale_exp(*a.d_absmax, 12);
    const float psa = ldexpf(1.f, ka), unscale = ldexpf(1.f, -(ka + kd));
    const bool affine = a.a_scale != nullptr;
    if (wave >= 4) {
        const int st_ = tid - 256;
        const int rq = st_ & 15, cq0 = st_ >> 4;
        float sc[2], sh[2];
#pragma unroll
        for (int u = 0; u < 2; ++u) {
            const int ch = affine ? (k0 + 4 * (cq0 + 16 * u)) / a.period : 0;
            sc[u] = affine ? a.a_scale[ch] * psa : psa; sh[u] = affine ? a.a_shift[ch] * psa : 0.f;
        }
        const float floor_ = affine ? 0.f : -INFINITY;
        f32x4 ar[2][8];
        f32x4 bs[2] = {(f32x4){0.f, 0.f, 0.f, 0.f}, (f32x4){0.f, 0.f, 0.f, 0.f}};
        auto issue_a = [&](int blk, f32x4 (&r)[8]) {
#pragma unroll
            for (int u = 0; u < 2; ++u)
#pragma unroll
                for (int j = 0; j < 4; ++j) {
                    const int m = blk * 64 + 4 * rq + j;
                    r[4 * u + j] = (f32x4){0.f, 0.f, 0.f, 0.f};
                    if (m < a.M && blk < b_hi) r[4 * u + j] = __builtin_nontemporal_load(reinterpret_cast<const f32x4*>(a.A + (long)m * a.lda + k0 + 4 * (cq0 + 16 * u)));
                }
        };
        auto commit_a = [&](int blk, const f32x4 (&r)[8]) {
            if (blk >= b_hi) return;
            unsigned char* st = lds + (blk % LF_NS) * LF_STAGE;
            if (BIAS) {
#pragma unroll
                for (int u = 0; u < 2; ++u)
#pragma unroll
                    for (int j = 0; j < 4; ++j)
#pragma unroll
                        for (int c = 0; c < 4; ++c) bs[u][c] += r[4 * u + j][c];
            }
#pragma unroll
            for (int u = 0; u < 2; ++u)
#pragma unroll
                for (int c = 0; c < 4; ++c) {
                    float x[4];
#pragma unroll
                    for (int j = 0; j < 4; ++j) x[j] = __builtin_amdgcn_fmed3f(fmaxf(fmaf(r[4 * u + j][c], sc[u], sh[u]), floor_), -65000.f, 65000.f);
                    uint2 hi, lo;
                    split2_pair_f16(x[0], x[1], hi.x, lo.x);
                    split2_pair_f16(x[2], x[3], hi.y, lo.y);
                    *reinterpret_cast<uint2*>(st + (0 * LIN_BM + 4 * (cq0 + 16 * u) + c) * LF_RS + rq * 8) = hi;
                    *reinterpret_cast<uint2*>(st + (1 * LIN_BM + 4 * (cq0 + 16 * u) + c) * LF_RS + rq * 8) = lo;
                }
        };
        if (b_lo < b_hi) {
            issue_a(b_lo, ar[0]);
            commit_a(b_lo, ar[0]);
            issue_a(b_lo + 1, ar[1]); issue_a(b_lo + 2, ar[0]);
        }
#pragma unroll 1
        for (int b = b_lo; b < b_hi; b += 2) {
            __syncthreads();
            commit_a(b + 1, ar[1]); issue_a(b + 3, ar[1]);
            if (b + 1 < b_hi) {
                __syncthreads();
                commit_a(b + 2, ar[0]); issue_a(b + 4, ar[0]);
            }
        }
        if (BIAS && blockIdx.z == 0) {
#pragma unroll
            for (int u = 0; u < 2; ++u) {
#pragma unroll
                for (int c = 0; c < 4; ++c)
#pragma unroll
                    for (int o = 1; o < 16; o <<= 1) bs[u][c] += __shfl_xor(bs[u][c], o, 64);
                if (rq == 0) *reinterpret_cast<f32x4*>(a.bias_partial + (long)blockIdx.y * a.K + k0 + 4 * (cq0 + 16 * u)) = bs[u];
            }
        }
        return;
    }
    lu32x4 df[2][4][2];
    const unsigned char* planes = a.planes + blockIdx.z * a.plane_stride;
    auto load_d = [&](int step, lu32x4 (&dst)[4][2]) {
        if (step >= 2 * b_hi) return;
#pragma unroll
        for (int nt = 0; nt < 4; ++nt)
#pragma unroll
            for (int sp = 0; sp < 2; ++sp)
                dst[nt][sp] = *reinterpret_cast<const lu32x4*>(planes + ((((long)step) * 16 + wave * 4 + nt) * 2 + sp) * 1024 + (unsigned)lane * 16u);
    };
    f32x4 acc[8][4];
#pragma unroll
    for (int kt = 0; kt < 8; ++kt)
#pragma unroll
        for (int nt = 0; nt < 4; ++nt) acc[kt][nt] = (f32x4){0.f, 0.f, 0.f, 0.f};
    bool neg = false;
    auto flip = [&]() {
#pragma unroll
        for (int kt = 0; kt < 8; ++kt)
#pragma unroll
            for (int nt = 0; nt < 4; ++nt)
#pragma unroll
                for (int r = 0; r < 4; ++r) acc[kt][nt][r] = -acc[kt][nt][r];
    };
    auto load_bf = [&](const unsigned char* st, int h, int qt, lu32x4 (&f)[2][2]) {
#pragma unroll
        for (int sp = 0; sp < 2; ++sp)
#pragma unroll
            for (int q = 0; q < 2; ++q) f[sp][q] = *reinterpret_cast<const lu32x4*>(st + (sp * LIN_BM + (qt * 2 + q) * 16 + lr) * LF_RS + h * 64 + lk * 16);
    };
    auto multiply = [&](int qt, const lu32x4 (&f)[2][2], const lu32x4 (&d)[4][2]) {
#define LW_PRODUCT(SX, SD)                                                                                                        \
        _Pragma("unroll") for (int nt = 0; nt < 4; ++nt)                                                                          \
            _Pragma("unroll") for (int q = 0; q < 2; ++q)                                                                         \
                acc[qt * 2 + q][nt] = __builtin_amdgcn_mfma_f32_16x16x32_f16(__builtin_bit_cast(f16x8, f[SX][q]),                 \
                                                                             __builtin_bit_cast(f16x8, d[nt][SD]), acc[qt * 2 + q][nt], 0, 0, 0);
        LW_PRODUCT(1, 0) LW_PRODUCT(0, 1) LW_PRODUCT(0, 0)
#undef LW_PRODUCT
    };
    load_d(2 * b_lo, df[0]);
#pragma unroll 1
    for (int blk = b_lo; blk < b_hi; ++blk) {
        const bool want = ((2 * blk) >> 3) & 1;
        if (want != neg) { flip(); neg = want; }
        __syncthreads();
        const unsigned char* st = lds + (blk % LF_NS) * LF_STAGE;
        lu32x4 fa[2][2], fb[2][2];
        load_bf(st, 0, 0, fa);
        load_d(2 * blk + 1, df[1]);
        __builtin_amdgcn_sched_barrier(0);
        load_bf(st, 0, 1, fb); multiply(0, fa, df[0]);
        __builtin_amdgcn_sched_barrier(0);
        load_bf(st, 0, 2, fa); multiply(1, fb, df[0]);
        __builtin_amdgcn_sched_barrier(0);
        load_bf(st, 0, 3, fb); multiply(2, fa, df[0]);
        __builtin_amdgcn_sched_barrier(0);
        load_bf(st, 1, 0, fa); multiply(3, fb, df[0]);
        __builtin_amdgcn_sched_barrier(0);
        load_d(2 * blk + 2, df[0]);
        load_bf(st, 1, 1, fb); multiply(0, fa, df[1]);
        __builtin_amdgcn_sched_barrier(0);
        load_bf(st, 1, 2, fa); multiply(1, fb, df[1]);
        __builtin_amdgcn_sched_barrier(0);
        load_bf(st, 1, 3, fb); multiply(2, fa, df[1]);
        __builtin_amdgcn_sched_barrier(0);
        multiply(3, fb, df[1]);
        __builtin_amdgcn_sched_barrier(0);
    }
    if (neg) flip();
    float* slab = a.partial + ((long)blockIdx.y * a.np + blockIdx.z * 256) * a.K;
#pragma unroll
    for (int kt = 0; kt < 8; ++kt)
#pragma unroll
        for (int nt = 0; nt < 4; ++nt) {
            f32x4 v = acc[kt][nt];
#pragma unroll
            for (int r = 0; r < 4; ++r) v[r] *= unscale;
            *reinterpret_cast<f32x4*>(slab + (long)(wave * 64 + nt * 16 + lr) * a.K + k0 + kt * 16 + lk * 4) = v;
        }
}

template <bool TR>
__global__ __launch_bounds__(256) void lin_wgrad_reduce(const float* __restrict__ partial, int splits, long n, float* __restrict__ G, long ldg, int K,
                                                        const float* __restrict__ bias_partial, float* __restrict__ bias) {
    const long i = ((long)blockIdx.x * 256 + threadIdx.x) * 4;
    if (i >= n) {
        const long k = i - n;
        if (!bias_partial || k >= K) return;
        f32x4 s = *reinterpret_cast<const f32x4*>(bias_partial + k);
        for (int p = 1; p < splits; ++p) {
            const f32x4 v = *reinterpret_cast<const f32x4*>(bias_partial + (long)p * K + k);
#pragma unroll
            for (int r = 0; r < 4; ++r) s[r] += v[r];
        }
#pragma unroll
        for (int r = 0; r < 4; ++r) bias[k + r] += s[r];
        return;
    }
    f32x4 s = *reinterpret_cast<const f32x4*>(partial + i);
    for (int p = 1; p < splits; ++p) {
        const f32x4 v = *reinterpret_cast<const f32x4*>(partial + (long)p * n + i);
#pragma unroll
        for (int r = 0; r < 4; ++r) s[r] += v[r];
    }
    if (TR) {
        float* g = G + (i % K) * ldg + (i / K);
#pragma unroll
        for (int r = 0; r < 4; ++r) g[r * ldg] += s[r];
        return;
    }
    float* g = G + (i / K) * ldg + (i % K);
    const f32x4 o = *reinterpret_cast<const f32x4*>(g);
#pragma unroll
    for (int r = 0; r < 4; ++r) s[r] += o[r];
    *reinterpret_cast<f32x4*>(g) = s;
}

static int lin_wgrad_splits(int M, int K) {
    const int ncol = K / LIN_BM, nblk = (M + 63) / 64;
    int s = (768 + ncol - 1) / ncol;
    if (s > 16) s = 16;
    if (s > nblk) s = nblk;
    return s < 1 ? 1 : s;
}
size_t a2s_linear_wgrad_ws_bytes_impl(int M, int K) {
    if (M < 1 || K < LIN_BM || K % LIN_BM) return 0;
    const size_t nsteps = 2 * (size_t)((M + 63) / 64);
    return nsteps * 16 * 2 * 1024 + (size_t)lin_wgrad_splits(M, K) * 256 * K * sizeof(float);
}
bool a2s_linear_wgrad_ok(int M, int N, int K, long ldz, long lda, long ldg, int period, const void* dz, const void* A, const void* G) {
    return N == 256 && M >= 64 && K >= LIN_BM && K % LIN_BM == 0 && (period == 0 || (period % 4 == 0 && K % period == 0)) && lda % 4 == 0 && ldg % 4 == 0 && ldz >= 256 &&
           (((uintptr_t)dz | (uintptr_t)A | (uintptr_t)G) % 16 == 0);
}
int a2s_linear_wgrad_impl(hipStream_t st, int M, int N, int K, const float* dz, long ldz, const float* A, long lda, float* G, long ldg, const float* a_scale,
                          const float* a_shift, int period, const float* dz_absmax, const float* a_absmax, float* ws, size_t ws_bytes) {
    A2S_REQUIRE(dz && A && G && dz_absmax && ws && ((a_scale == nullptr) == (a_shift == nullptr)), "linear_wgrad: null argument");
    A2S_REQUIRE(a2s_linear_wgrad_ok(M, N, K, ldz, lda, ldg, a_scale ? period : 0, dz, A, G), "linear_wgrad: needs N = 256, K %% 128 == 0, period %% 4 == 0, 16-byte aligned rows");
    A2S_REQUIRE(((uintptr_t)ws % 16 == 0) && ws_bytes >= a2s_linear_wgrad_ws_bytes_impl(M, K), "linear_wgrad: workspace too small (%zu bytes needed)",
                a2s_linear_wgrad_ws_bytes_impl(M, K));
    const int nblk = (M + 63) / 64, nsteps = 2 * nblk, splits = lin_wgrad_splits(M, K);
    unsigned char* planes = reinterpret_cast<unsigned char*>(ws);
    float* partial = reinterpret_cast<float*>(planes + (size_t)nsteps * 16 * 2 * 1024);
    hipLaunchKernelGGL(lin_pack_dz_planes, dim3((unsigned)(((long)nsteps * 1024 + 255) / 256)), dim3(256), 0, st, dz, ldz, M, nsteps, dz_absmax, planes);
    A2S_CHECK_LAUNCH("lin_pack_dz_planes");
    LinWgradArgs a{A, lda, planes, partial, a_scale, a_shift, a_absmax, dz_absmax, M, K, a_scale ? period : K, nblk, (nblk + splits - 1) / splits, 0, 256, nullptr};
    hipLaunchKernelGGL(lin_wgrad_roles<false>, dim3(K / LIN_BM, splits), dim3(LIN_NTH), 0, st, a);
    A2S_CHECK_LAUNCH("lin_wgrad");
    const long n = 256L * K;
    hipLaunchKernelGGL(lin_wgrad_reduce<false>, dim3((unsigned)((n / 4 + 255) / 256)), dim3(256), 0, st, partial, splits, n, G, ldg, K, nullptr, nullptr);
    A2S_CHECK_LAUNCH("lin_wgrad_reduce");
    return A2S_OK;
}

#define TALLK_SLAB_BYTES (64u << 20)
int a2s_tallk_wgrad_on = 1;
int a2s_tallk_wgrad_max_splits = 0;
static long long g_tallk_launches = 0;
long a2s_tallk_wgrad_launches(void) { return (long)__atomic_load_n(&g_tallk_launches, __ATOMIC_RELAXED); }

static int tallk_splits(int M, int Np, int K) {
    const int tiles = (K / LIN_BM) * (Np / 256), nblk = (M + 63) / 64;
    int cus = a2s_device_geometry().cus;
    if (cus < 1) cus = 256;
    int s = cus / tiles;
    const size_t slab = (size_t)Np * K * sizeof(float);
    if ((size_t)s * slab > TALLK_SLAB_BYTES) s = (int)(TALLK_SLAB_BYTES / slab);
    if (s > nblk) s = nblk;
    if (a2s_tallk_wgrad_max_splits > 0 && s > a2s_tallk_wgrad_max_splits) s = a2s_tallk_wgrad_max_splits;
    return s < 1 ? 1 : s;
}
bool a2s_tallk_wgrad_ok(int M, int Np, int K, long ldp, long lda, long ldg, int transposed, const void* P, const void* A, const void* G, const void* bias) {
    return a2s_tallk_wgrad_on && M >= 64 && Np >= 256 && Np % 256 == 0 && Np <= 2048 && K >= LIN_BM && K % LIN_BM == 0 && K <= 4096 && ldp >= Np && lda >= K &&
           lda % 4 == 0 && ldg % 4 == 0 && ldg >= (transposed ? Np : K) && (((uintptr_t)P | (uintptr_t)A | (uintptr_t)G | (uintptr_t)bias) % 16 == 0);
}
size_t a2s_tallk_wgrad_ws_bytes_impl(int M, int Np, int K) {
    if (M < 1 || Np < 256 || Np % 256 || K < LIN_BM || K % LIN_BM) return 0;
    const size_t nsteps = 2 * (size_t)((M + 63) / 64), splits = (size_t)tallk_splits(M, Np, K);
    return (size_t)(Np / 256) * nsteps * 16 * 2 * 1024 + splits * Np * K * sizeof(float) + splits * K * sizeof(float);
}
int a2s_tallk_wgrad_impl(hipStream_t st, int M, int Np, int K, const float* P, long ldp, const float* A, long lda, float* G, long ldg, int transposed,
                         float* bias, const float* p_absmax, const float* a_absmax, float* ws, size_t ws_bytes) {
    A2S_REQUIRE(P && A && G && p_absmax && a_absmax && ws, "tallk_wgrad: null argument");
    A2S_REQUIRE(a2s_tallk_wgrad_ok(M, Np, K, ldp, lda, ldg, transposed, P, A, G, bias),
                "tallk_wgrad: needs M >= 64, Np %% 256 == 0, K %% 128 == 0, 16-byte aligned bases and rows (or the switch \"tallk_wgrad\" is off)");
    A2S_REQUIRE(((uintptr_t)ws % 16 == 0) && ws_bytes >= a2s_tallk_wgrad_ws_bytes_impl(M, Np, K), "tallk_wgrad: workspace too small (%zu bytes needed)",
                a2s_tallk_wgrad_ws_bytes_impl(M, Np, K));
    const int nblk = (M + 63) / 64, nsteps = 2 * nblk, splits = tallk_splits(M, Np, K), npb = Np / 256;
    const size_t plane_stride = (size_t)nsteps * 16 * 2 * 1024;
    unsigned char* planes = reinterpret_cast<unsigned char*>(ws);
    float* partial = reinterpret_cast<float*>(planes + npb * plane_stride);
    float* bias_partial = partial + (size_t)splits * Np * K;
    hipLaunchKernelGGL(lin_pack_dz_planes, dim3((unsigned)(((long)nsteps * 1024 + 255) / 256), npb), dim3(256), 0, st, P, ldp, M, nsteps, p_absmax, planes);
    A2S_CHECK_LAUNCH("lin_pack_dz_planes");
    LinWgradArgs a{A, lda, planes, partial, nullptr, nullptr, a_absmax, p_absmax, M, K, K, nblk, (nblk + splits - 1) / splits, (long)plane_stride, Np,
                   bias ? bias_partial : nullptr};
    if (bias) hipLaunchKernelGGL(lin_wgrad_roles<true>, dim3(K / LIN_BM, splits, npb), dim3(LIN_NTH), 0, st, a);
    else hipLaunchKernelGGL(lin_wgrad_roles<false>, dim3(K / LIN_BM, splits, npb), dim3(LIN_NTH), 0, st, a);
    A2S_CHECK_LAUNCH("lin_wgrad (tall-K)");
    const long n = (long)Np * K, nthreads = (n + (bias ? K : 0)) / 4;
    const dim3 rgrid((unsigned)((nthreads + 255) / 256));
    if (transposed) hipLaunchKernelGGL(lin_wgrad_reduce<true>, rgrid, dim3(256), 0, st, partial, splits, n, G, ldg, K, bias ? bias_partial : nullptr, bias);
    else hipLaunchKernelGGL(lin_wgrad_reduce<false>, rgrid, dim3(256), 0, st, partial, splits, n, G, ldg, K, bias ? bias_partial : nullptr, bias);
    A2S_CHECK_LAUNCH("lin_wgrad_reduce");
    __atomic_fetch_add(&g_tallk_launches, 1LL, __ATOMIC_RELAXED);
    return A2S_OK;
}
```

### piano_a2s_amd/engine_bwd.py

```python
import ctypes as C
import os
import threading

import torch

from . import hip
from .spec import SOS, VOCAB_SIZE


def _os_env(name, default):
    return os.environ.get(name, default)


def _ptr(t, off=0):
    return C.c_void_p(t.data_ptr() + 4 * off)


_COLSUM_WS = {}


def _colsum(x, ld, out, rows, ncol, x_off=0, out_off=0, beta=1.0):
    ws = None
    if rows >= 2048:
        key = (x.device, torch.cuda.current_stream().cuda_stream, threading.get_ident())
# ... 209 lines not shown
        H2 = 2 * H
        self.names = [k for k in S if not is_buffer(k)]
        self.offs, self.total = flat_layout([S[k].numel() for k in self.names])
        self.flat_full = torch.zeros(self.total + 1, dtype=torch.float32, device=dev)
        self.flat = self.flat_full[:self.total]
        self.G = {k: self.flat[off:off + S[k].numel()].view(S[k].shape) for k, off in zip(self.names, self.offs)}
        ptrs_host = torch.tensor([self.G[f"decoder.staff_emb.{w}_{sfx}"].data_ptr() for sfx in ("l0", "l0_reverse")
                                  for w in ("weight_ih", "weight_hh", "bias_ih", "bias_hh")], dtype=torch.int64).pin_memory()
        self.G["__staff_emb_ptrs__"] = ptrs_host.to(dev, non_blocking=True)
        self.keep_alive = [ptrs_host]
        self.dEnc = torch.zeros((B, T, H2), dtype=torch.float32, device=dev)
        self.dK = {p: torch.zeros((B, T, H), dtype=torch.float32, device=dev) for p in ("decoder", "decoder.upper_decoder", "decoder.lower_decoder")}
        self.concurrent = bool(concurrent)
        self.dEnc_staff = [torch.zeros_like(self.dEnc), torch.zeros_like(self.dEnc)] if self.concurrent else [self.dEnc, self.dEnc]
        self.bar_major = bool(bar_major)
        self.use_deferred = False
        lw = getattr(eng, "late_wgrads", None)
        self.late_wgrads = True if lw is None else bool(lw)
        self.late = []
        self.clip_groups = list(clip_groups) if clip_groups else [(0, B)]
        self.two_term = True
        self.d_hidden = torch.empty((B, H2), dtype=torch.float32, device=dev)
        self.group_flat = [self.flat] + [torch.zeros_like(self.flat) for _ in self.clip_groups[1:]]
        self.group_ptrs = [self.G["__staff_emb_ptrs__"]]
        for gf in self.group_flat[1:]:
            ph = (ptrs_host + (gf.data_ptr() - self.flat.data_ptr())).pin_memory()
            self.keep_alive.append(ph)
            self.group_ptrs.append(ph.to(dev, non_blocking=True))

    def decoder_group(self, gidx, gs, dts_g, dkey_g, dup_g, dlo_g):
        from .engine import fork_on_streams, staff_streams
        eng, S, G, dev, T = self.eng, self.S, self.G, self.dev, self.T
        names, offs, group_flat, group_ptrs = self.names, self.offs, self.group_flat, self.group_ptrs
        dEnc, dK, dEnc_staff, d_hidden = self.dEnc, self.dK, self.dEnc_staff, self.d_hidden
        concurrent, bar_major, use_deferred = self.concurrent, self.bar_major, self.use_deferred
        L = hip.lib()
        cfg = eng.cfg
        H, Sz = cfg["hidden_size"], cfg["staff_emb_size"]
        te, ke, bars = cfg["time_sig_emb_size"], cfg["key_emb_size"], cfg["max_bars"]
        tokw = 4 * Sz + te + ke
        H2 = 2 * H
        b0, b1 = gs["range"]
        Bg = b1 - b0
        Gg = G if gidx == 0 else {k: group_flat[gidx][off:off + S[k].numel()].view(S[k].shape) for k, off in zip(names, offs)}
        Gg["__staff_emb_ptrs__"] = group_ptrs[gidx]
        enc_g, keys_g = gs["enc"], gs["keys"]
        enc_amax_g = hip.absmax(enc_g) if (self.two_term and enc_g.is_contiguous()) else None
        dEnc_g = dEnc[b0:b1]
        dK_g = {p: t[b0:b1] for p, t in dK.items()}
        dEnc_staff_g = [t[b0:b1] for t in dEnc_staff]
        ts_out_g, key_out_g, up_out_g, lo_out_g = gs["outs"]
        persist_g = any(seg["staff"][k][2].get("persist_ws") is not None for seg in gs["segments"] for k in ("up", "lo"))
        from .engine import staves_concurrent
        concurrent_g = concurrent and staves_concurrent(gidx, len(self.clip_groups)) and not persist_g
        streams = staff_streams(dev, gidx) if concurrent_g else None
        use_deferred_g = use_deferred and gidx == 0
        deferred_streams = _deferred_streams(dev, gidx) if use_deferred_g else None
        deferred_done = []
        seg_dh0 = {}

        def segment_decoders_bwd(si_seg):
            seg = gs["segments"][si_seg]
            bar0, nb = seg["bars"][0], len(seg["bars"])
            calls = []
            for si, (name, prefix, dout, out_t) in enumerate((("up", "decoder.upper_decoder", dup_g, up_out_g), ("lo", "decoder.lower_decoder", dlo_g, lo_out_g))):
                if bar_major:
                    maxs = out_t.shape[2]
                    dpr, pr = dout[bar0:bar0 + nb].view(nb * Bg, maxs, -1), out_t[bar0:bar0 + nb].view(nb * Bg, maxs, -1)
                else:
                    dpr, pr = dout[:, bar0], out_t[:, bar0]
                calls.append((eng, S, Gg, seg["staff"][name][2], keys_g[prefix], enc_g, dpr, pr, dK_g[prefix], dEnc_staff_g[si], Bg, T,
                              deferred_streams[si] if use_deferred_g else None, enc_amax_g, self.late if self.late_wgrads else None))
            if concurrent_g and seg.get("pair") is not None and L.a2s_debug_get(b"attn_pair"):
                (res,), events = fork_on_streams(dev, [streams[1]], [lambda: _note_decoder_bwd_pair(calls, streams, seg["pair"])])(wait=False)
                seg_dh0[si_seg] = ([r[0] for r in res], events)
                deferred_done.extend(r[1] for r in res if r[1] is not None)
            elif concurrent_g:
                res, events = fork_on_streams(dev, streams, [lambda args=args: _note_decoder_bwd(*args) for args in calls])(wait=False)
                seg_dh0[si_seg] = ([r[0] for r in res], events)
                deferred_done.extend(r[1] for r in res if r[1] is not None)
            else:
                seg_dh0[si_seg] = ([_note_decoder_bwd(*args)[0] for args in calls], [])

        for si_seg in reversed(range(len(gs["segments"]))):
            segment_decoders_bwd(si_seg)

        bar_attn = []
        d_hid_carry = None
        d_token_next = None
        for bar in reversed(range(bars)):
            b = gs["bars"][bar]
            if d_token_next is not None:
                for rec in b["tok_rec"]:
                    _staff_token_bwd(eng, S, Gg, rec, d_token_next)
                ts_ids, key_ids, i64, stride = b["next_ids"]
                for table, ids_, col, width in (("decoder.time_sig_emb.weight", ts_ids, 4 * Sz, te), ("decoder.key_emb.weight", key_ids, 4 * Sz + te, ke)):
                    hip.check(L.a2s_embed_scatter_add(hip.stream(), hip._p(Gg[table]), hip._p(ids_) if i64 else None, None if i64 else hip._p(ids_), stride, 0,
                                                      hip._p(d_token_next), tokw, col, Bg, width, None, 1.0), "scatter ts/key")
            d_headin = torch.zeros((Bg, 4 * H), dtype=torch.float32, device=dev)
            for hname, dout, out_t, nc in (("time_sig_out", dts_g, ts_out_g, cfg["num_time_sig"]), ("key_out", dkey_g, key_out_g, cfg["num_keys"])):
                t1, t2, lg, _ = b["heads"][hname]
                dlg = torch.empty((Bg, nc), dtype=torch.float32, device=dev)
                hip.check(L.a2s_log_softmax_bwd_rows(hip.stream(), _ptr(dout, bar * nc), _ptr(out_t, bar * nc), bars * nc, 1, hip._p(dlg), Bg, nc, Bg, 0),
                          "lsm bwd head")
                p = f"decoder.{hname}"
                dt2 = torch.empty_like(t2)
                _linear_bwd(t2, S[p + ".4.weight"], dlg, Gg, p + ".4.weight", p + ".4.bias", dx=dt2)
                hip.check(L.a2s_ew_act_bwd(hip.stream(), hip._p(dt2), hip._p(t2), hip._p(dt2), dt2.numel(), 1), "relu bwd")
                dt1 = torch.empty_like(t1)
                _linear_bwd(t1, S[p + ".2.weight"], dt2, Gg, p + ".2.weight", p + ".2.bias", dx=dt1)
                hip.check(L.a2s_ew_act_bwd(hip.stream(), hip._p(dt1), hip._p(t1), hip._p(dt1), dt1.numel(), 1), "relu bwd")
                _linear_bwd(b["headin"], S[p + ".0.weight"], dt1, Gg, p + ".0.weight", p + ".0.bias", dx=d_headin, dx_beta=1.0)
            d_hnew = torch.zeros((Bg, H2), dtype=torch.float32, device=dev)
            si_seg, j = b["seg"]
            dh0s, events = seg_dh0[si_seg]
            for ev in events:
                torch.cuda.current_stream().wait_event(ev)
            for dh0 in dh0s:
                d_hnew.add_(dh0[j * Bg:(j + 1) * Bg])
            d_hnew.add_(d_headin[:, :H2])
            if d_hid_carry is not None:
                d_hnew.add_(d_hid_carry)
            ldxb = tokw + H2
            dgi, dgh = torch.empty((Bg, 3 * H2), device=dev), torch.empty((Bg, 3 * H2), device=dev)
            dhp = torch.empty((Bg, H2), device=dev)
            hip.check(L.a2s_gru_gates_bwd(hip.stream(), hip._p(d_hnew), H2, None, 0, hip._p(b["gates"]), hip._p(b["hprev"]), H2, hip._p(dgi), 3 * H2, hip._p(dgh),
                                          3 * H2, None, 0, hip._p(dhp), H2, Bg, H2), "gates bwd bar")
            d_xbar = torch.empty((Bg, ldxb), device=dev)
            _linear_bwd(b["xbar"], S["decoder.gru.weight_ih_l0"], dgi, Gg, "decoder.gru.weight_ih_l0", "decoder.gru.bias_ih_l0", dx=d_xbar)
            _linear_bwd(b["hprev"], S["decoder.gru.weight_hh_l0"], dgh, Gg, "decoder.gru.weight_hh_l0", "decoder.gru.bias_hh_l0", dx=dhp, dx_beta=1.0)
            dq, ds = torch.empty((Bg, H), device=dev), torch.empty((1, Bg, T), device=dev)
            dctx = torch.empty((1, Bg, H2), device=dev)
            from .engine import bar_attn_workspace
            bar_ws = bar_attn_workspace(dev, gidx, Bg, T, H)
            if bar_ws is not None:
                ctx_c, dctx_c = b["xbar"][:, tokw:].contiguous(), d_xbar[:, tokw:].contiguous()
                hip.check(L.a2s_attn_step_bwd(hip.stream(), hip._p(keys_g["decoder"]), hip._p(enc_g), hip._p(b["qb"]), H, hip._p(S["decoder.attn.v.weight"]),
                                              hip._p(b["attw"]), hip._p(ctx_c), H2, hip._p(dctx_c), H2, _ptr(d_headin, H2), 4 * H, hip._p(dctx), H2, hip._p(dq), H,
                                              hip._p(ds), Bg, T, H, hip._p(bar_ws)), "attn bwd bar")
            else:
                hip.check(L.a2s_attn_step_bwd(hip.stream(), hip._p(keys_g["decoder"]), hip._p(enc_g), hip._p(b["qb"]), H, hip._p(S["decoder.attn.v.weight"]),
                                              hip._p(b["attw"]), _ptr(b["xbar"], tokw), ldxb, _ptr(d_xbar, tokw), ldxb, _ptr(d_headin, H2), 4 * H, hip._p(dctx), H2,
                                              hip._p(dq), H, hip._p(ds), Bg, T, H, None), "attn bwd bar")
            Wa = S["decoder.attn.attn.weight"]
            hip.gemm(dq, H, 1, Wa, 4 * H, 1, dhp, H2, Bg, H2, H, beta=1.0)
            hip.gemm(dq, 1, H, b["hprev"], H2, 1, Gg["decoder.attn.attn.weight"], 4 * H, H, H2, Bg, beta=1.0)
            _colsum(dq, H, Gg["decoder.attn.attn.bias"], Bg, H)
            bar_attn.append((b["qb"].view(1, Bg, H), ds, b["attw"].view(1, Bg, T), dctx))
            d_hid_carry = dhp
            d_token = d_xbar[:, :tokw].contiguous()
            if b["keep"] is not None:
                d_token = d_token * b["keep"] / 0.9
            d_token_next = d_token
        qs, dss, aws, dcs = [torch.cat(t, 0) for t in zip(*bar_attn)]
        _attn_deferred(eng, S, Gg, "decoder.attn", keys_g["decoder"], enc_g, qs, dss, aws, dcs, dK_g["decoder"], dEnc_g, Bg, T, H, len(bar_attn))
        d_sos = d_token_next.clone()
        d_sos[:, :2 * Sz] += d_sos[:, 2 * Sz:4 * Sz]
        _staff_token_bwd(eng, S, Gg, gs["sos_rec"][0], d_sos)
        for table, cid, col, width in (("decoder.time_sig_emb.weight", cfg["num_time_sig"], 4 * Sz, te), ("decoder.key_emb.weight", cfg["num_keys"], 4 * Sz + te, ke)):
            hip.check(L.a2s_embed_scatter_add(hip.stream(), hip._p(Gg[table]), None, None, 0, cid, hip._p(d_token_next), tokw, col, Bg, width, None, 1.0),
                      "scatter sos ts/key")
        d_hidden[b0:b1].copy_(d_hid_carry)
        for ev in deferred_done:
            torch.cuda.current_stream().wait_event(ev)
        return None


    def finish(self, grad_ready=None):
        eng, S, G, dev = self.eng, self.S, self.G, self.dev
        B, T, F = self.B, self.T, self.F
        names, offs, total, flat = self.names, self.offs, self.total, self.flat
        dEnc, dK = self.dEnc, self.dK
        sv = eng.saved
        assert sv["training"], "backward needs a forward run with training=True (batch statistics / saved activations)"
        L = hip.lib()
        H = eng.cfg["hidden_size"]
        H2 = 2 * H
        enc = sv["enc_out"]
        G["__staff_emb_ptrs__"] = self.group_ptrs[0]
        late_join = None
        if self.late:
            dec_lo = next(off for k, off in zip(names, offs) if k.startswith("decoder."))
            assert all(k.startswith("decoder.") for k, off in zip(names, offs) if off >= dec_lo), "the decoder's parameters must be the tail of the flat layout"
            wg = _weight_grad_stream(dev)
            wg.wait_stream(torch.cuda.current_stream())
            with torch.cuda.stream(wg):
                for fn, ev, tensors in self.late:
                    wg.wait_event(ev)
                    for t in tensors:
                        if t is not None:
                            t.record_stream(wg)
                    fn()
            late_join = dec_lo
            self.late = []
        else:
            for gf in self.group_flat[1:]:
                flat.add_(gf)
        d_hid_carry = self.d_hidden
        if self.concurrent:
            dEnc.add_(self.dEnc_staff[0]).add_(self.dEnc_staff[1])
        enc2d = enc.view(B * T, H2)
        enc_amax = hip.absmax(enc) if self.two_term else None
        for p, dKp in dK.items():
            Wn = p + ".attn.attn.weight"
            dk_amax = hip.absmax(dKp) if self.two_term else None
            if not hip.tallk_wgrad(dKp, 0, H, enc2d, 0, H2, G[Wn], H2, 4 * H, B * T, H, H2, dk_amax, enc_amax):
                sk = L.a2s_gemm_pick_splitk(H, H2, B * T, 1)
                hip.gemm(dKp, 1, H, enc2d, H2, 1, G[Wn], 4 * H, H, H2, B * T, beta=1.0, splitk=sk, c_off=H2,
                         two_term=(dk_amax, enc_amax) if self.two_term else None)
            hip.gemm(dKp, H, 1, S[Wn], 4 * H, 1, dEnc, H2, B * T, H2, H, beta=1.0, b_off=H2,
                     two_term=(dk_amax, hip.absmax(S[Wn])) if self.two_term else None)
        if late_join is not None:
            wg = _weight_grad_stream(dev)
            wg.wait_stream(torch.cuda.current_stream())
            with torch.cuda.stream(wg):
                for gf in self.group_flat[1:]:
                    flat[late_join:].add_(gf[late_join:])
                if Backward.check_fold:
                    for gi, gf in enumerate(self.group_flat[1:], 1):
                        assert not bool(gf[:late_join].any()), f"clip group {gi}: non-decoder gradients in the group buffer would be lost by the late fold"
        defer = True
        d_conv = _encoder_bwd(eng, S, G, sv["enc"], dEnc, d_hid_carry, B, T, wait_weight_grads=not defer)
        n_conv = next(off for k, off in zip(names, offs) if not k.startswith("convstack."))
        if grad_ready is not None:
            if defer:
                with torch.cuda.stream(_weight_grad_stream(dev)):
                    grad_ready(self.flat_full, n_conv, total + 1)
            else:
                grad_ready(self.flat_full, n_conv, total + 1)
        if getattr(eng, "conv_unperm", None) is not None:
            d_conv = d_conv.reshape(B, T, -1).index_select(0, eng.conv_unperm)
        _convstack_bwd(eng, S, G, sv["conv"], d_conv, B, T, F)
        if defer:
            torch.cuda.current_stream().wait_stream(_weight_grad_stream(dev))
        if grad_ready is not None:
            grad_ready(flat, 0, n_conv)
        G[None] = flat
        G["__loss_gate__"] = self.flat_full[total:]
        eng._keep_alive = self.keep_alive
        return G




def backward(eng, S, grad_outputs, grad_ready=None, loss_total=None):
    from .engine import group_views, run_clip_groups
    sv = eng.saved
    assert sv["training"], "backward needs a forward run with training=True (batch statistics / saved activations)"
    dev = sv["enc_out"].device
    clip_groups = sv.get("clip_groups") or [(0, sv["shape"][0])]
    ctx = Backward(eng, S, sv["shape"], dev, clip_groups, sv.get("concurrent"), sv.get("bar_major"))
    dts, dkey, dup, dlo = [g.contiguous() for g in grad_outputs]

    def group(gidx):
        b0, b1 = clip_groups[gidx]
        if ctx.bar_major:
            dup_g, dlo_g = group_views(dup, clip_groups, gidx), group_views(dlo, clip_groups, gidx)
        else:
            dup_g, dlo_g = dup[b0:b1], dlo[b0:b1]
        ctx.decoder_group(gidx, sv["groups"][gidx], dts[b0:b1], dkey[b0:b1], dup_g, dlo_g)

    run_clip_groups(dev, [lambda gi=gi: group(gi) for gi in range(len(clip_groups))])
    if loss_total is not None:
        ctx.flat_full[ctx.total:].copy_(loss_total.reshape(1))
    return ctx.finish(grad_ready)


_WG_STREAMS = {}
_DEFERRED_STREAMS = {}


def _deferred_streams(dev, group=0):
    idx = torch.device(dev).index if torch.device(dev).index is not None else torch.cuda.current_device()
    key = (idx, group)
    if key not in _DEFERRED_STREAMS:
        _DEFERRED_STREAMS[key] = (torch.cuda.Stream(device=idx), torch.cuda.Stream(device=idx))
    return _DEFERRED_STREAMS[key]



def _weight_grad_stream(dev):
    from .engine import group_stream
    return group_stream(dev, 1)


def _encoder_bwd(eng, S, G, es, dEnc, d_hidden, B, T, wait_weight_grads=True):
    L = hip.lib()
    H = eng.cfg["hidden_size"]
    dev = dEnc.device
    W = S["encoder.fc.weight"]
    dpre = torch.empty_like(d_hidden)
    hip.check(L.a2s_ew_act_bwd(hip.stream(), hip._p(d_hidden), hip._p(es["hidden"]), hip._p(dpre), dpre.numel(), 2), "tanh bwd")
    dhn = []
    for l in (0, 1):
        for half, hfin in enumerate((es["finals"][2 * l], es["finals"][2 * l + 1])):
            d = torch.empty((B, H), device=dev)
            hip.gemm(dpre, 2 * H, 1, W, 2 * H, 1, d, H, B, H, H, a_off=l * H, b_off=half * H)
            hip.gemm(dpre, 1, 2 * H, hfin, H, 1, G["encoder.fc.weight"], 2 * H, H, H, B, beta=1.0, a_off=l * H, c_off=half * H)
            dhn.append(d)
        _colsum(dpre, 2 * H, G["encoder.fc.bias"], B, H, x_off=l * H)
    gws = [hip.gemm_workspace(B, dev), hip.gemm_workspace(B, dev)]
    two_term = True
    in_amax = hip.absmax(es["layers"][0]["in"]) if two_term else None
    dout = dEnc
    for layer in (1, 0):
        ls = es["layers"][layer]
        inp = ls["in"]
        I = inp.shape[1]
        out = ls["out"]
        dX = torch.empty((B * T, I), device=dev)
        from .engine import encoder_streams, fork_on_streams
        streams = encoder_streams(dev, B)

        def direction(d, sfx):
            dgi = torch.empty((B, T, 3 * H), device=dev)
            dghs = torch.empty((B, T, 3 * H), device=dev)
            dgh_first, dhbuf, dgh_tmp = torch.empty((B, 3 * H), device=dev), torch.empty((2, B, H), device=dev), torch.empty((B, 3 * H), device=dev)
            ranges, valid = torch.empty(2, device=dev), C.c_int(0)
            if two_term and L.a2s_debug_get(b"tallk_wgrad") > 0:
                hip.check(L.a2s_gru_seq_bwd_ranged(hip.stream(), _ptr(dout, d * H), T * 2 * H, 2 * H, _ptr(out, d * H), T * 2 * H, 2 * H, hip._p(ls["dirs"][d]["gates"]),
                                                   hip._p(S[f"encoder.gru.weight_hh_{sfx}"]), hip._p(dhn[2 * layer + d]), hip._p(dgi), hip._p(dghs), hip._p(dgh_first),
                                                   hip._p(dhbuf), hip._p(dgh_tmp), B, T, H, d, hip._p(gws[d]), gws[d].numel() * 4, hip._p(ranges), C.byref(valid)),
                          "a2s_gru_seq_bwd_ranged")
            else:
                hip.check(L.a2s_gru_seq_bwd(hip.stream(), _ptr(dout, d * H), T * 2 * H, 2 * H, _ptr(out, d * H), T * 2 * H, 2 * H, hip._p(ls["dirs"][d]["gates"]),
                                            hip._p(S[f"encoder.gru.weight_hh_{sfx}"]), hip._p(dhn[2 * layer + d]), hip._p(dgi), hip._p(dghs), hip._p(dgh_first),
                                            hip._p(dhbuf), hip._p(dgh_tmp), B, T, H, d, hip._p(gws[d]), gws[d].numel() * 4), "a2s_gru_seq_bwd")
            return (dgi, dghs, dgh_first, dhbuf, dgh_tmp, ranges if valid.value else None)

        res = fork_on_streams(dev, streams, [lambda d=d, sfx=sfx: direction(d, sfx) for d, sfx in enumerate((f"l{layer}", f"l{layer}_reverse"))])()
        dgi_amax = []
        for d, sfx in enumerate((f"l{layer}", f"l{layer}_reverse")):
            dgi2 = res[d][0].view(B * T, 3 * H)
            Wih = S[f"encoder.gru.weight_ih_{sfx}"]
            ranges = res[d][5]
            tt = (ranges[0:1] if ranges is not None else hip.absmax(dgi2), hip.absmax(Wih)) if two_term else None
            dgi_amax.append(tt[0] if tt else None)
            if L.a2s_debug_get(b"gemm_bf16x3") > 0:
                hip.gemm(dgi2, 3 * H, 1, Wih.t().contiguous(), 1, 3 * H, dX, I, B * T, I, 3 * H, beta=0.0 if d == 0 else 1.0, two_term=tt)
            else:
                hip.gemm(dgi2, 3 * H, 1, Wih, I, 1, dX, I, B * T, I, 3 * H, beta=0.0 if d == 0 else 1.0, two_term=tt)
        wg = _weight_grad_stream(dev)
        ev = torch.cuda.Event()
        ev.record()
        wg.wait_event(ev)
        for d, sfx in enumerate((f"l{layer}", f"l{layer}_reverse")):
            dgi, dghs, dgh_first, ranges = res[d][0], res[d][1], res[d][2], res[d][5]
            for t in (dgi, dghs, dgh_first, dgi_amax[d], in_amax, ranges):
                if t is not None:
                    t.record_stream(wg)
            with torch.cuda.stream(wg):
                dgi2, dghs2 = dgi.view(B * T, 3 * H), dghs.view(B * T, 3 * H)
                x_bound = ((in_amax if layer == 0 else hip.one(dev)) if two_term else None)
                if not hip.tallk_wgrad(inp, 0, I, dgi2, 0, 3 * H, G[f"encoder.gru.weight_ih_{sfx}"], 0, I, B * T, I, 3 * H, x_bound, dgi_amax[d],
                                       transposed=True, bias=G[f"encoder.gru.bias_ih_{sfx}"]):
                    _linear_bwd(inp, S[f"encoder.gru.weight_ih_{sfx}"], dgi2, G, f"encoder.gru.weight_ih_{sfx}", f"encoder.gru.bias_ih_{sfx}",
                                dy_amax=dgi_amax[d], x_bound=x_bound)
                dghs_amax = (ranges[1:2] if ranges is not None else hip.absmax(dghs2)) if two_term else None
                if not hip.tallk_wgrad(out, d * H, 2 * H, dghs2, 0, 3 * H, G[f"encoder.gru.weight_hh_{sfx}"], 0, H, B * T, H, 3 * H,
                                       hip.one(dev) if two_term else None, dghs_amax, transposed=True, bias=G[f"encoder.gru.bias_hh_{sfx}"]):
                    sk = L.a2s_gemm_pick_splitk(3 * H, H, B * T, 1)
                    hip.gemm(dghs2, 1, 3 * H, out, 2 * H, 1, G[f"encoder.gru.weight_hh_{sfx}"], H, 3 * H, H, B * T, beta=1.0, splitk=sk, b_off=d * H,
                             two_term=(dghs_amax, hip.one(dev)) if two_term else None)
                    _colsum(dghs2, 3 * H, G[f"encoder.gru.bias_hh_{sfx}"], B * T, 3 * H)
                _colsum(dgh_first, 3 * H, G[f"encoder.gru.bias_hh_{sfx}"], B, 3 * H)
        dout = dX.view(B, T, I)
    if wait_weight_grads:
        torch.cuda.current_stream().wait_stream(_weight_grad_stream(dev))
    return dout


_FUSE_BN_APPLY = False
_FUSE_BN_APPLY_L1 = True
_DGRAD_BNSTATS = True
_SYNC_FUSED = True
_LIN_WGRAD_AT = "before"
_FUSE_BN_ROWS = os.environ.get("A2S_FUSE_BN_ROWS", "1") != "0"


def _linear_dgrad_generic(L, dev, rows, F, Cf, dz, Wout, da, y4, bn4, dz_amax, w_amax):
    nblk = L.a2s_gemm_bnstats_blocks(rows, F)
    part = torch.empty((nblk, 40, 2), dtype=torch.float32, device=dev)
    if L.a2s_debug_get(b"gemm_bf16x3") > 0:
        Wt = Wout.t().contiguous()
        wb, s_bk, s_bn = Wt, 1, Cf
    else:
        wb, s_bk, s_bn = Wout, 40 * F, 1
    hip.check(L.a2s_gemm_f32_bnstats_scaled(hip.stream(), rows, 40 * F, Cf, hip._p(dz), Cf, 1, hip._p(wb), s_bk, s_bn, hip._p(da), 40 * F, hip._p(y4), hip._p(bn4[0]),
                                            hip._p(bn4[1]), hip._p(bn4[2]), hip._p(bn4[3]), F, hip._p(part), hip._p(dz_amax), hip._p(w_amax)),
              "a2s_gemm_f32_bnstats_scaled")
    return part, nblk


def _convstack_bwd(eng, S, G, cs, d_out, B, T, F):
    L = hip.lib()
    dev = d_out.device
    Cf = eng.cfg["conv_feature_size"]
    rows = B * T

    def bn_bwd(g, x, bn, name, mask, n_rows, C_, F_, stats_only=False, partial=None, amax=None):
        mean, invstd, scale, shift = bn
        if partial is not None and eng.sync_bn and stats_only:
            import torch.distributed as dist
            local = torch.empty(2 * C_, dtype=torch.float32, device=dev)
            hip.check(L.a2s_bn_bwd_sums_from_partial(hip.stream(), hip._p(partial[0]), partial[1], C_, hip._p(local)), "a2s_bn_bwd_sums_from_partial")
            glob = local.clone()
            dist.all_reduce(glob)
            c12 = torch.empty(2 * C_, dtype=torch.float32, device=dev)
            hip.check(L.a2s_bn_bwd_c12_from_sums(hip.stream(), hip._p(local), hip._p(glob), eng.bn_counts[name], hip._p(G[name + ".weight"]), hip._p(G[name + ".bias"]),
                                                 hip._p(c12), C_), "a2s_bn_bwd_c12_from_sums")
            return c12
        if partial is not None and not eng.sync_bn:
            c12 = torch.empty(2 * C_, dtype=torch.float32, device=dev)
            hip.check(L.a2s_bn_bwd_from_partial_amax(hip.stream(), hip._p(g), hip._p(x), hip._p(mean), hip._p(invstd), hip._p(scale), hip._p(shift),
                                                     hip._p(G[name + ".weight"]), hip._p(G[name + ".bias"]), None if stats_only else hip._p(g), hip._p(partial[0]),
                                                     partial[1], hip._p(c12), n_rows, C_, F_, hip._p(amax)), "a2s_bn_bwd_from_partial")
            return c12 if stats_only else g
        part = torch.empty(L.a2s_bn_bwd_partial_floats(n_rows, C_, F_), dtype=torch.float32, device=dev)
        c12 = torch.empty(2 * C_, dtype=torch.float32, device=dev)
        if eng.sync_bn:
            import torch.distributed as dist
            local = torch.empty(2 * C_, dtype=torch.float32, device=dev)
            hip.check(L.a2s_bn_bwd_stats(hip.stream(), hip._p(g), hip._p(x), hip._p(mean), hip._p(invstd), hip._p(scale), hip._p(shift), hip._p(mask), 1.0 / 0.8,
                                         hip._p(part), hip._p(local), n_rows, C_, F_), "a2s_bn_bwd_stats")
            glob = local.clone()
            dist.all_reduce(glob)
            hip.check(L.a2s_bn_bwd_apply(hip.stream(), hip._p(g), hip._p(x), hip._p(mean), hip._p(invstd), hip._p(scale), hip._p(shift), hip._p(mask), 1.0 / 0.8,
                                         hip._p(local), hip._p(glob), eng.bn_counts[name], hip._p(G[name + ".weight"]), hip._p(G[name + ".bias"]), hip._p(g),
                                         hip._p(c12), n_rows, C_, F_), "a2s_bn_bwd_apply")
            return g
        hip.check(L.a2s_bn_bwd_amax(hip.stream(), hip._p(g), hip._p(x), hip._p(mean), hip._p(invstd), hip._p(scale), hip._p(shift), hip._p(mask), 1.0 / 0.8,
                                    hip._p(G[name + ".weight"]), hip._p(G[name + ".bias"]), None if stats_only else hip._p(g), hip._p(part), hip._p(c12), n_rows, C_, F_,
                                    hip._p(amax)), "a2s_bn_bwd")
        return c12 if stats_only else g

    g = d_out.reshape(rows, Cf).contiguous()
    dz_amax = torch.zeros(1, dtype=torch.float32, device=dev)
    dz = bn_bwd(g, cs["z"], cs["out_bn"], "convstack.out_bn", cs["drop"], rows, Cf, 1, amax=dz_amax)
    if eng.sync_bn:
        hip.absmax(dz, dz_amax)
    w_amax = cs.get("w_out_amax")
    a4 = cs["a4"]
    g_partial = None
    g_amax = None
    Wout = S["convstack.out.weight"]
    if a4 is None:
        y4 = cs["y"][3].view(rows, 40 * F)
        da = torch.empty_like(y4)
        bn4 = cs["bn"][3]
        def lin_wgrad():
            if not hip.linear_wgrad(dz, y4, (bn4[2], bn4[3], F), dz_amax, cs["abound"][3], G["convstack.out.weight"]):
                _linear_bwd(y4, Wout, dz, G, "convstack.out.weight", None, x_affine=(bn4[2], bn4[3], F), dy_amax=dz_amax, x_bound=cs["abound"][3])
        lin_at = _LIN_WGRAD_AT
        lin_overlap = lin_at != "before"

        def lin_wgrad_side():
            wg_stream = _weight_grad_stream(dev)
            ev = torch.cuda.Event()
            ev.record()
            wg_stream.wait_event(ev)
            with torch.cuda.stream(wg_stream):
                lin_wgrad()
        if lin_at == "beside":
            lin_wgrad_side()
        elif lin_at == "before":
            lin_wgrad()
        if _DGRAD_BNSTATS and (not eng.sync_bn or _SYNC_FUSED) and F >= 128 and F % 4 == 0 and rows > 64:
            if w_amax is None:
                w_amax = hip.absmax(Wout)
            if hip.LINEAR_KERNELS and L.a2s_linear_dgrad_eligible(rows, 40 * F, Cf, F):
                nblk = L.a2s_linear_dgrad_blocks(rows)
                part = torch.empty((nblk, 40, 2), dtype=torch.float32, device=dev)
                Wt = Wout.t().contiguous()
                nb = L.a2s_linear_dgrad_ws_bytes(40 * F, Cf)
                lws = torch.empty(nb // 4, dtype=torch.float32, device=dev)
                g_amax = torch.zeros(1, dtype=torch.float32, device=dev)
                hip.check(L.a2s_linear_dgrad_bnstats(hip.stream(), rows, 40 * F, Cf, hip._p(dz), Cf, hip._p(Wt), hip._p(da), 40 * F, hip._p(y4), hip._p(bn4[0]),
                                                     hip._p(bn4[1]), hip._p(bn4[2]), hip._p(bn4[3]), F, hip._p(part), hip._p(dz_amax), hip._p(w_amax), hip._p(lws), nb,
                                                     hip._p(g_amax)), "a2s_linear_dgrad_bnstats")
                g_partial = (part, nblk)
            else:
                g_partial = _linear_dgrad_generic(L, dev, rows, F, Cf, dz, Wout, da, y4, bn4, dz_amax, w_amax)
        else:
            hip.gemm(dz, Cf, 1, Wout, 40 * F, 1, da, 40 * F, rows, 40 * F, Cf)
    else:
        da = torch.empty_like(a4)
        _linear_bwd(a4, Wout, dz, G, "convstack.out.weight", None, dx=da)
    chans = [(1, 20), (20, 20), (20, 40), (40, 40)]
    g = da.view(B, T, 40, F)
    for i in (4, 3, 2, 1):
        ci, co = chans[i - 1]
        y = cs["y"][i - 1]
        x_in = cs["y"][i - 2] if i > 1 else cs["x0"]
        in_bn = cs["bn"][i - 2] if i > 1 else None
        nb = L.a2s_conv3x3_wgrad_workspace_bytes(ci, co)
        ws = torch.empty(nb // 4, dtype=torch.float32, device=dev)
        fuse_here = _FUSE_BN_APPLY or (i == 1 and _FUSE_BN_APPLY_L1)
        dy_amax = torch.zeros(1, dtype=torch.float32, device=dev) if (i > 1 and (not eng.sync_bn or _SYNC_FUSED)) else None
        fuse_rows = (_FUSE_BN_ROWS and (not eng.sync_bn or _SYNC_FUSED) and i > 1 and g_amax is not None and g_partial is not None and in_bn is not None
                     and L.a2s_conv3x3_wgrad_bn_ranged_eligible(F, ci, co))
        if a4 is None and lin_at == i:
            lin_wgrad_side()
        if fuse_rows:
            bn_i = cs["bn"][i - 1]
            c12 = bn_bwd(g, y, bn_i, f"convstack.bn{i}", None, rows, co, F, stats_only=True, partial=g_partial)
            dy = g
            hip.check(L.a2s_conv3x3_wgrad_bn_ranged(hip.stream(), hip._p(g), hip._p(y), hip._p(bn_i[0]), hip._p(bn_i[1]), hip._p(bn_i[2]), hip._p(bn_i[3]), hip._p(c12),
                                                    hip._p(g_amax), g_amax.numel(), hip._p(cs["yabs"][i - 1]), hip._p(dy), hip._p(dy_amax), hip._p(x_in),
                                                    hip._p(in_bn[2]), hip._p(in_bn[3]), hip._p(G[f"convstack.conv{i}.weight"]), hip._p(ws), nb, B, T, F, ci, co,
                                                    hip._p(cs["abound"][i - 2])), "a2s_conv3x3_wgrad_bn_ranged")
        elif eng.sync_bn or not fuse_here:
            dy = bn_bwd(g, y, cs["bn"][i - 1], f"convstack.bn{i}", None, rows, co, F, partial=g_partial, amax=dy_amax)
            if eng.sync_bn and dy_amax is not None:
                hip.absmax(dy, dy_amax)
            hip.conv3x3_wgrad(dy, x_in.view(B, T, ci, F), in_bn[2] if in_bn else None, in_bn[3] if in_bn else None, G[f"convstack.conv{i}.weight"], ws,
                              dy_amax, cs["abound"][i - 2] if in_bn else None)
        else:
            bn_i = cs["bn"][i - 1]
            c12 = bn_bwd(g, y, bn_i, f"convstack.bn{i}", None, rows, co, F, stats_only=True, partial=g_partial)
            dy = torch.empty_like(g) if i > 1 else None
            hip.check(L.a2s_conv3x3_wgrad_bn(hip.stream(), hip._p(g), hip._p(y), hip._p(bn_i[0]), hip._p(bn_i[1]), hip._p(bn_i[2]), hip._p(bn_i[3]), hip._p(c12),
                                             hip._p(dy), hip._p(x_in), hip._p(in_bn[2]) if in_bn else None, hip._p(in_bn[3]) if in_bn else None,
                                             hip._p(G[f"convstack.conv{i}.weight"]), hip._p(ws), nb, B, T, F, ci, co), "a2s_conv3x3_wgrad_bn")
        if i > 1:
            gprev = torch.empty((B, T, ci, F), dtype=torch.float32, device=dev)
            cws = hip.conv_workspace(co, dev)
            if _DGRAD_BNSTATS and (not eng.sync_bn or _SYNC_FUSED):
                bn_l = cs["bn"][i - 2]
                nblk = L.a2s_conv3x3_stat_blocks(B, T, F, co)
                part = torch.empty((nblk, ci, 2), dtype=torch.float32, device=dev)
                g_amax_next = torch.empty(ci, dtype=torch.float32, device=dev) if (_FUSE_BN_ROWS and i > 2) else None
                hip.check(L.a2s_conv3x3_dgrad_bnstats_ranged(hip.stream(), hip._p(dy), hip._p(S[f"convstack.conv{i}.weight"]), hip._p(gprev), hip._p(cs["y"][i - 2]),
                                                             hip._p(bn_l[0]), hip._p(bn_l[1]), hip._p(bn_l[2]), hip._p(bn_l[3]), hip._p(part), B, T, F, co, ci,
                                                             hip._p(cws), hip._p(dy_amax) if not fuse_here else None, hip._p(g_amax_next)), "a2s_conv3x3_dgrad_bnstats")
                g_partial = (part, nblk)
            else:
                hip.check(L.a2s_conv3x3(hip.stream(), hip._p(dy), hip._p(S[f"convstack.conv{i}.weight"]), hip._p(gprev), None, None, None, B, T, F, co, ci, 1,
                                        hip._p(cws)), "a2s_conv3x3 dgrad")
                g_partial = None
            g = gprev
            g_amax = g_amax_next if (_DGRAD_BNSTATS and (not eng.sync_bn or _SYNC_FUSED)) else None
    if a4 is None and lin_overlap:
        torch.cuda.current_stream().wait_stream(_weight_grad_stream(dev))
```

### piano_a2s_amd/hip.py

```python
import ctypes as C
import os
import threading

import torch

from .abi import PROTOTYPES, STRUCTS, A2SError
from .build import LIB

LIB = os.environ.get("A2S_LIB", LIB)

NoteDecArgs, NoteDecBwdArgs, BeamArgs, AlignArgs = (STRUCTS[n] for n in ("a2s_note_dec_args", "a2s_note_dec_bwd_args", "a2s_beam_args", "a2s_align_args"))
_lib = None


def set_row_plan(a, active):
    active = active or {}
    for field, key in (("clip_order", "order"), ("clip_rank", "rank"), ("row_until", "until"), ("row_list", "row_list")):
        setattr(a, field, active[key].data_ptr() if active.get(key) is not None else None)
    for field, key in (("n_active", "n_active"), ("m_active", "m_active"), ("n_rows_active", "n_rows_active")):
        host = active.get(key) if (key != "n_rows_active" or active.get("row_list") is not None) else None
        setattr(a, field, C.cast(host, C.c_void_p).value if host is not None else None)
    a.n_clips = active.get("n_clips", 0)


# ... 375 lines not shown

def specaug_launches():
    return int(lib().a2s_specaug_launches())


def _room_table(fn, params, seeds=None):
    _need(torch.is_tensor(params) and params.dtype == torch.int32 and params.dim() == 2 and params.shape[1] == 4 and params.is_contiguous() and params.is_cuda,
          fn, "params", "must be a contiguous (B, 4) int32 tensor on the device: [pre, L, wet f32 bits, decay f32 bits] per clip")
    if seeds is not None:
        _need(torch.is_tensor(seeds) and seeds.dtype == torch.int32 and tuple(seeds.shape) == (params.shape[0],) and seeds.is_contiguous()
              and seeds.device == params.device, fn, "seeds", f"must be a contiguous int32 tensor (the 32 bits of every clip's seed) of {params.shape[0]} elements on the table's device")
    return params.shape[0]


def _rows(fn, name, t, B, n, device):
    _need(torch.is_tensor(t) and t.dtype == torch.float32 and t.dim() == 2 and t.shape[0] >= B and t.shape[1] >= n and t.device == device
          and (t.shape[1] == 1 or t.stride(1) == 1) and (t.shape[0] <= 1 or t.stride(0) >= n), fn, name,
          f"must be a float32 tensor of at least {B} rows of at least {n} elements with unit stride on the table's device")
    return t.stride(0) if t.shape[0] > 1 else max(t.stride(0), n)


def room_ir(seeds, params, L_max, ir=None):
    fn = "room_ir"
    B = _room_table(fn, params, seeds)
    L_max = int(L_max)
    _need(L_max >= 1, fn, "L_max", f"must be >= 1 (got {L_max})")
    if ir is None:
        ir = torch.empty((B, L_max), dtype=torch.float32, device=params.device)
    stride = _rows(fn, "ir", ir, B, L_max, params.device)
    if B == 0:
        return ir
    check(lib().a2s_room_ir(stream(), _p(seeds), _p(params), B, _p(ir), stride, L_max), "a2s_room_ir")
    return ir


def fir_rows(x, ir, params, L_max, y=None, n_samples=None):
    fn = "fir_rows"
    B = _room_table(fn, params)
    L_max = int(L_max)
    _need(L_max >= 1, fn, "L_max", f"must be >= 1 (got {L_max})")
    _need(torch.is_tensor(x) and x.dim() == 2, fn, "x", "must be a 2-D float32 tensor")
    n = x.shape[1] if n_samples is None else int(n_samples)
    _need(n >= 1 or B == 0, fn, "n_samples", f"must be >= 1 (got {n})")
    xs = _rows(fn, "x", x, B, n, params.device)
    irs = _rows(fn, "ir", ir, B, L_max, params.device)
    if y is None:
        y = torch.empty((B, n), dtype=torch.float32, device=params.device)
    ys = _rows(fn, "y", y, B, n, params.device)
    if B == 0:
        return y
    _need(x.data_ptr() != y.data_ptr(), fn, "y", "must not be x (the convolution works out of place)")
    check(lib().a2s_fir_rows(stream(), _p(x), xs, _p(ir), irs, _p(params), _p(y), ys, B, n, L_max), "a2s_fir_rows")
    return y


def fir_tile_samples():
    return int(lib().a2s_fir_tile_samples())


def fir_tap_chunk():
    return int(lib().a2s_fir_tap_chunk())


def room_launches():
    return int(lib().a2s_room_launches())


def resample_rows(x, n_in, table, M, Hh, channels=1, y=None, n_out_max=None, n_in_max=None):
    fn = "resample_rows"
    _need(torch.is_tensor(table) and table.dtype == torch.float32 and table.dim() == 2 and table.is_contiguous() and table.is_cuda and table.numel() > 0, fn,
          "table", "must be a contiguous (L, K) float32 tensor on the device")
    L, K = table.shape
    try:
        M, Hh, C = int(M), int(Hh), int(channels)
    except (TypeError, ValueError):
        raise A2SError(f"{fn}: `M`, `Hh` and `channels` must be whole numbers (got {M!r}, {Hh!r}, {channels!r})") from None
    _need(1 <= C <= 8, fn, "channels", f"must be in 1 .. 8 (got {C})")
    _need(1 <= L <= 4096, fn, "table", f"must have 1 .. 4096 rows (got {L})")
    _need(1 <= K <= 8192, fn, "table", f"must have 1 .. 8192 columns (got {K})")
    _need(1 <= M <= 4096, fn, "M", f"must be in 1 .. 4096 (got {M})")
    _need(0 <= Hh < K, fn, "Hh", f"must be in 0 .. K - 1 = {K - 1} (got {Hh})")
    _need(torch.is_tensor(n_in) and n_in.dtype == torch.int32 and n_in.dim() == 1 and n_in.is_contiguous() and n_in.device == table.device, fn, "n_in",
          "must be a contiguous int32 tensor of one element per clip on the table's device")
    B = n_in.shape[0]
    _need(torch.is_tensor(x) and x.dim() == 2, fn, "x", "must be a 2-D float32 tensor of interleaved frames")
    nim = x.shape[1] // C if n_in_max is None else int(n_in_max)
    _need(nim >= 0, fn, "n_in_max", f"must be >= 0 (got {nim})")
    nom = -(-nim * L // M) if n_out_max is None else int(n_out_max)
    _need(nom >= 1 or B == 0, fn, "n_out_max", f"must be >= 1 (got {nom})")
    xs = _rows(fn, "x", x, B, nim * C, table.device)
    if y is None:
        y = torch.empty((B, max(nom, 0)), dtype=torch.float32, device=table.device)
    ys = _rows(fn, "y", y, B, nom, table.device)
    if B == 0:
        return y
    _need(x.data_ptr() != y.data_ptr(), fn, "y", "must not be x (the resampler works out of place)")
    check(lib().a2s_resample_rows(stream(), _p(x), xs, _p(n_in), nim, C, _p(table), L, M, K, Hh, _p(y), ys, nom, B), "a2s_resample_rows")
    return y


def resample_tile_samples():
    return int(lib().a2s_resample_tile_samples())


def resample_launches():
    return int(lib().a2s_resample_launches())


def note_match(ref, ref_off, hyp, hyp_off, n_pairs, dur_ticks, midi, cls, out):
    fn = "note_match"
    for name, t, dtype in (("ref", ref, torch.int32), ("hyp", hyp, torch.int32), ("ref_off", ref_off, torch.int64), ("hyp_off", hyp_off, torch.int64)):
        _need(isinstance(t, int) or (torch.is_tensor(t) and t.dtype == dtype and t.is_contiguous()), fn, name, f"must be a contiguous {dtype} tensor or an address")
    for name, t in (("ref_off", ref_off), ("hyp_off", hyp_off)):
        _need(isinstance(t, int) or t.numel() == n_pairs + 1, fn, name, f"must have n_pairs + 1 = {n_pairs + 1} elements")
    for name, t in (("dur_ticks", dur_ticks), ("midi", midi), ("cls", cls)):
        _need(torch.is_tensor(t) and t.dtype == torch.int32 and t.is_contiguous() and t.dim() == 1 and t.numel() == dur_ticks.numel(), fn, name,
              "must be a contiguous int32 tensor (V,)")
    _need(torch.is_tensor(out) and out.dtype == torch.int32 and out.is_contiguous() and out.numel() == 8 * n_pairs, fn, "out",
          f"must be a contiguous int32 tensor of 8 * n_pairs = {8 * n_pairs} elements")
    if n_pairs == 0:
        return out
    check(lib().a2s_note_match(stream(), _p(ref), _p(ref_off), _p(hyp), _p(hyp_off), n_pairs, _p(dur_ticks), _p(midi), _p(cls), dur_ticks.numel(), _p(out)),
          "a2s_note_match")
    return out


def note_match_launches():
    return int(lib().a2s_note_match_launches())


def align_buffers(R, max_steps, T, device):
    t = dict(attw_step=torch.zeros((R, T), dtype=torch.float32, device=device),
             peak=torch.full((R, max_steps), -1, dtype=torch.int32, device=device),
             weight=torch.zeros((R, max_steps), dtype=torch.float32, device=device),
             centroid=torch.full((R, max_steps), -1.0, dtype=torch.float32, device=device))
    g = AlignArgs()
    for name in ("attw_step", "peak", "weight", "centroid"):
        setattr(g, name, t[name].data_ptr())
    g.out_stride = max_steps
    g.next_state, g.n_states, g.row_state = None, 0, None
    return g, t


def check(rc, what):
    if rc != 0:
        raise A2SError(f"{what} failed ({rc}): {lib().a2s_last_error().decode()}")


def f32(x):
    return C.c_float(float(x))


def gemm(A, sAm, sAk, B, sBk, sBn, Cout, ldc, M, N, K, alpha=1.0, beta=0.0, bias=None, act=0,
         batch=1, bsA=0, bsB=0, bsC=0, splitk=1, a_off=0, b_off=0, c_off=0, a_affine=None, b_affine=None, two_term=None):
    L = lib()
    ws, ws_bytes = None, 0
    if splitk > 1:
        ws_bytes = L.a2s_gemm_workspace_bytes(M, N, batch, splitk)
        ws = torch.empty(ws_bytes // 4, dtype=torch.float32, device=Cout.device)
    pa = C.c_void_p(A.data_ptr() + 4 * a_off)
    pb = C.c_void_p(B.data_ptr() + 4 * b_off)
    pc = C.c_void_p(Cout.data_ptr() + 4 * c_off)
    if a_affine is None and b_affine is None and two_term is None:
        check(L.a2s_gemm_f32(stream(), M, N, K, alpha, pa, sAm, sAk, pb, sBk, sBn, beta, pc, ldc, _p(bias), act, batch, bsA, bsB, bsC, splitk, _p(ws), ws_bytes),
              "a2s_gemm_f32")
        return
    asc, ash, ap = a_affine if a_affine is not None else (None, None, 0)
    bsc, bsh, bp = b_affine if b_affine is not None else (None, None, 0)
    if two_term is not None:
        check(L.a2s_gemm_f32_affine_scaled(stream(), M, N, K, alpha, pa, sAm, sAk, pb, sBk, sBn, beta, pc, ldc, _p(bias), act, batch, bsA, bsB, bsC, splitk, _p(ws),
                                           ws_bytes, _p(asc), _p(ash), ap, _p(bsc), _p(bsh), bp, _p(two_term[0]), _p(two_term[1])), "a2s_gemm_f32_affine_scaled")
        return
    check(L.a2s_gemm_f32_affine(stream(), M, N, K, alpha, pa, sAm, sAk, pb, sBk, sBn, beta, pc, ldc, _p(bias), act, batch, bsA, bsB, bsC, splitk, _p(ws), ws_bytes,
                                _p(asc), _p(ash), ap, _p(bsc), _p(bsh), bp), "a2s_gemm_f32_affine")


_ONES = {}


def one(device):
    key = torch.device(device).index
    if key not in _ONES:
        _ONES[key] = torch.ones(1, dtype=torch.float32, device=device)
    return _ONES[key]


def absmax(x, out=None):
    if out is None:
        out = torch.empty(1, dtype=torch.float32, device=x.device)
    check(lib().a2s_absmax(stream(), _p(x), x.numel(), _p(out)), "a2s_absmax")
    return out


def linear(x2d, weight, bias=None, act=0, out=None, beta=0.0, x_affine=None, two_term=None):
    M, K = x2d.shape
    N = weight.shape[0]
    if out is None:
        out = torch.empty((M, N), dtype=torch.float32, device=x2d.device)
    gemm(x2d, x2d.stride(0), x2d.stride(1), weight, weight.stride(1), weight.stride(0), out, out.stride(0), M, N, K,
         bias=bias, act=act, beta=beta, a_affine=x_affine, two_term=two_term)
    return out


def conv3x3_forward(x, w, y, scale, shift, partial, cws, in_absmax=None, out_absmax=None):
    B, T, Cin, F = x.shape
    check(lib().a2s_conv3x3_ranged(stream(), _p(x), _p(w), _p(y), _p(scale), _p(shift), _p(in_absmax), _p(partial), _p(out_absmax),
                                   B, T, F, Cin, y.shape[2], _p(cws)), "a2s_conv3x3_ranged")


def conv3x3_dgrad_for_test(dy, w, yl):
    L = lib()
    B, T, Cout, F = dy.shape
    Cin = w.shape[1]
    dev = dy.device
    dx = torch.full((B, T, Cin, F), float("nan"), device=dev)
    amax = absmax(dy)
    part = torch.zeros(L.a2s_conv3x3_stat_blocks(B, T, F, Cout), Cin, 2, device=dev)
    cws = conv_workspace(Cout, dev)
    zeros, ones = torch.zeros(Cin, device=dev), torch.ones(Cin, device=dev)
    check(L.a2s_conv3x3_dgrad_bnstats_scaled(stream(), _p(dy), _p(w), _p(dx), _p(yl), _p(zeros), _p(ones), _p(ones), _p(zeros), _p(part),
                                             B, T, F, Cout, Cin, _p(cws), _p(amax)), "a2s_conv3x3_dgrad_bnstats_scaled")
    torch.cuda.synchronize()
    return dx


def act_bound(scale, shift, x_absmax):
    out = torch.empty(1, dtype=torch.float32, device=scale.device)
    check(lib().a2s_act_bound(stream(), _p(scale), _p(shift), _p(x_absmax), scale.numel(), _p(out)), "a2s_act_bound")
    return out


def conv3x3_wgrad(dy, x, scale, shift, dW, ws, dy_absmax, act_absmax):
    B, T, Cout, F = dy.shape
    Cin = x.shape[2]
    check(lib().a2s_conv3x3_wgrad_ranged(stream(), _p(dy), _p(x), _p(scale), _p(shift), _p(dW), _p(ws), ws.numel() * 4, B, T, F, Cin, Cout, _p(dy_absmax),
                                         _p(act_absmax)), "a2s_conv3x3_wgrad_ranged")


def conv3x3_wgrad_for_test(dy, x, scale, shift):
    L = lib()
    B, T, Cout, F = dy.shape
    Cin = x.shape[2]
    dev = dy.device
    dW = torch.zeros(Cout, Cin, 3, 3, device=dev)
    ws = torch.empty(L.a2s_conv3x3_wgrad_workspace_bytes(Cin, Cout) // 4, device=dev)
    bound = act_bound(scale, shift, x.abs().amax(dim=(0, 1, 3)).contiguous())
    conv3x3_wgrad(dy, x, scale, shift, dW, ws, absmax(dy), bound)
    torch.cuda.synchronize()
    return dW


def linear_forward(x2d, weight, x_affine, x_bound, w_absmax, out=None):
    M, K = x2d.shape
    N = weight.shape[0]
    L = lib()
    period = x_affine[2]
    if (LINEAR_KERNELS and x2d.is_contiguous() and weight.is_contiguous() and x_bound is not None
            and L.a2s_linear_fwd_eligible(M, N, K, period)):
        if out is None:
            out = torch.empty((M, N), dtype=torch.float32, device=x2d.device)
        nb = L.a2s_linear_dgrad_ws_bytes(N, K)
        ws = torch.empty(nb // 4, dtype=torch.float32, device=x2d.device)
        check(L.a2s_linear_fwd(stream(), M, N, K, _p(x2d), K, _p(weight), _p(out), N, _p(x_affine[0]), _p(x_affine[1]), period, _p(x_bound), _p(w_absmax), _p(ws), nb),
              "a2s_linear_fwd")
        return out
    return linear(x2d, weight, out=out, x_affine=x_affine, two_term=(x_bound, w_absmax))


def linear_wgrad(dz, x2d, x_affine, dz_absmax, x_bound, G):
    M, K = x2d.shape
    N = dz.shape[1]
    L = lib()
    if (not LINEAR_KERNELS or not (x2d.is_contiguous() and dz.is_contiguous() and G.is_contiguous()) or dz_absmax is None
            or x_bound is None or not L.a2s_linear_wgrad_eligible(M, N, K, x_affine[2])):
        return False
    nb = L.a2s_linear_wgrad_ws_bytes(M, K)
    ws = torch.empty(nb // 4, dtype=torch.float32, device=x2d.device)
    check(L.a2s_linear_wgrad(stream(), M, N, K, _p(dz), N, _p(x2d), K, _p(G), K, _p(x_affine[0]), _p(x_affine[1]), x_affine[2], _p(dz_absmax), _p(x_bound), _p(ws), nb),
          "a2s_linear_wgrad")
    return True


_TALLK_WS = {}


def tallk_wgrad(P, p_off, ldp, A, a_off, lda, G, g_off, ldg, M, Np, K, p_absmax, a_absmax, transposed=False, bias=None):
    L = lib()
    if not hasattr(L, "a2s_tallk_wgrad_eligible"):
        return False
    pp, pa, pg = P.data_ptr() + 4 * p_off, A.data_ptr() + 4 * a_off, G.data_ptr() + 4 * g_off
    if (p_absmax is None or a_absmax is None or (pp | pa | pg | (bias.data_ptr() if bias is not None else 0)) % 16
            or not L.a2s_tallk_wgrad_eligible(M, Np, K, ldp, lda, ldg, int(transposed))):
        return False
    nb = L.a2s_tallk_wgrad_ws_bytes(M, Np, K)
    key = (A.device, torch.cuda.current_stream().cuda_stream, threading.get_ident())
    ws = _TALLK_WS.get(key)
    if ws is None or ws.numel() * 4 < nb:
        ws = _TALLK_WS[key] = torch.empty((nb + 3) // 4, dtype=torch.float32, device=A.device)
    check(L.a2s_tallk_wgrad(stream(), M, Np, K, C.c_void_p(pp), ldp, C.c_void_p(pa), lda, C.c_void_p(pg), ldg, int(transposed), _p(bias), _p(p_absmax), _p(a_absmax),
                            _p(ws), ws.numel() * 4), "a2s_tallk_wgrad")
    return True


def linear_forward_for_test(x, w, aff):
    period = aff[2]
    xmax = x.view(x.shape[0], -1, period).abs().amax(dim=(0, 2)).contiguous()
    return linear_forward(x, w, aff, act_bound(aff[0], aff[1], xmax), absmax(w))
```

Before: 634.4.

## Share packed GRU activation planes across tall-K weight-grad calls and pair plane blocks

Splits the tall-K weight-gradient path into a separate pack step and a packed GEMM step. The encoder backward packs each GRU layer's input and output activations into planes once, on the weight-grad stream, and reuses them across both directions' weight_ih and weight_hh gradients instead of repacking per call. The wgrad kernel gains an NPB=2 variant where each block handles two 256-column plane blocks over half the K width, which reuses each A tile across two plane blocks. This costs extra persistent plane buffers and an upfront stream sync, and it changes the kernel's schedule.

```diff
diff --git a/include/a2s.h b/include/a2s.h
--- a/include/a2s.h
+++ b/include/a2s.h
@@ -45,6 +45,11 @@
                     const float* p_absmax, const float* a_absmax, float* workspace, size_t workspace_bytes);
 size_t a2s_tallk_wgrad_ws_bytes(int M, int Np, int K);
 int a2s_tallk_wgrad_eligible(int M, int Np, int K, long ldp, long lda, long ldg, int transposed);
+int a2s_tallk_pack(void* stream, int M, int Np, const float* P, long ldp, const float* p_absmax, void* planes, size_t planes_bytes);
+int a2s_tallk_wgrad_packed(void* stream, int M, int K, const void* planes, int planes_blocks, int first_block, int nblocks, const float* A, long lda, float* G,
+                           long ldg, int transposed, float* bias, const float* p_absmax, const float* a_absmax, float* workspace, size_t workspace_bytes);
+size_t a2s_tallk_planes_bytes(int M, int Np);
+size_t a2s_tallk_wgrad_packed_ws_bytes(int M, int Np, int K);
 size_t a2s_linear_dgrad_ws_bytes(int N, int K);
 int a2s_linear_dgrad_blocks(int M);
 int a2s_linear_dgrad_eligible(int M, int N, int K, int period);
diff --git a/piano_a2s_amd/csrc/a2s_api.hip b/piano_a2s_amd/csrc/a2s_api.hip
--- a/piano_a2s_amd/csrc/a2s_api.hip
+++ b/piano_a2s_amd/csrc/a2s_api.hip
@@ -63,6 +63,16 @@
     return a2s_tallk_wgrad_impl(ST, M, Np, K, P, ldp, A, lda, G, ldg, transposed, bias, p_absmax, a_absmax, workspace, workspace_bytes);
 }
 size_t a2s_tallk_wgrad_ws_bytes(int M, int Np, int K) { return a2s_tallk_wgrad_ws_bytes_impl(M, Np, K); }
+int a2s_tallk_pack(void* stream, int M, int Np, const float* P, long ldp, const float* p_absmax, void* planes, size_t planes_bytes) {
+    return a2s_tallk_pack_impl(ST, M, Np, P, ldp, p_absmax, planes, planes_bytes);
+}
+int a2s_tallk_wgrad_packed(void* stream, int M, int K, const void* planes, int planes_blocks, int first_block, int nblocks, const float* A, long lda, float* G,
+                           long ldg, int transposed, float* bias, const float* p_absmax, const float* a_absmax, float* workspace, size_t workspace_bytes) {
+    return a2s_tallk_wgrad_packed_impl(ST, M, K, planes, planes_blocks, first_block, nblocks, A, lda, G, ldg, transposed, bias, p_absmax, a_absmax, workspace,
+                                       workspace_bytes);
+}
+size_t a2s_tallk_planes_bytes(int M, int Np) { return a2s_tallk_planes_bytes_impl(M, Np); }
+size_t a2s_tallk_wgrad_packed_ws_bytes(int M, int Np, int K) { return a2s_tallk_packed_ws_bytes_impl(M, Np, K); }
 int a2s_tallk_wgrad_eligible(int M, int Np, int K, long ldp, long lda, long ldg, int transposed) {
     return a2s_tallk_wgrad_ok(M, Np, K, ldp, lda, ldg, transposed, nullptr, nullptr, nullptr, nullptr) ? 1 : 0;
 }
@@ -88,6 +98,9 @@
     if (!strcmp(key, "attn_deferred_fast")) { a2s_attn_deferred_fast = value ? 1 : 0; return A2S_OK; }
     if (!strcmp(key, "tallk_wgrad")) { a2s_tallk_wgrad_on = value ? 1 : 0; return A2S_OK; }
     if (!strcmp(key, "tallk_wgrad_max_splits")) { a2s_tallk_wgrad_max_splits = value > 0 ? value : 0; return A2S_OK; }
+    if (!strcmp(key, "tallk_shared_planes")) { a2s_tallk_shared_planes = value ? 1 : 0; return A2S_OK; }
+    if (!strcmp(key, "tallk_wgrad_pair_blocks")) { a2s_tallk_pair_blocks = value ? 1 : 0; return A2S_OK; }
+    if (!strcmp(key, "tallk_wgrad_split_div")) { a2s_tallk_split_div = value > 1 ? value : 1; return A2S_OK; }
     if (!strcmp(key, "gemm_tile")) { a2s_gemm_debug_tile_impl(value); return A2S_OK; }
     snprintf(a2s_err_msg, sizeof(a2s_err_msg), "a2s_debug_set: unknown key %s", key);
     return A2S_ERR_ARG;
@@ -109,6 +122,9 @@
     if (!strcmp(key, "attn_deferred_fast")) return a2s_attn_deferred_fast;
     if (!strcmp(key, "tallk_wgrad")) return a2s_tallk_wgrad_on;
     if (!strcmp(key, "tallk_wgrad_max_splits")) return a2s_tallk_wgrad_max_splits;
+    if (!strcmp(key, "tallk_shared_planes")) return a2s_tallk_shared_planes;
+    if (!strcmp(key, "tallk_wgrad_pair_blocks")) return a2s_tallk_pair_blocks;
+    if (!strcmp(key, "tallk_wgrad_split_div")) return a2s_tallk_split_div;
     if (!strcmp(key, "tallk_wgrad_launches")) return (int)a2s_tallk_wgrad_launches();
     if (!strcmp(key, "attn_dk_ahead_launches")) return (int)a2s_attn_dk_ahead_launches();
     if (!strcmp(key, "attn_denc_launches")) return (int)a2s_attn_denc_launches();
diff --git a/piano_a2s_amd/csrc/a2s_internal.h b/piano_a2s_amd/csrc/a2s_internal.h
--- a/piano_a2s_amd/csrc/a2s_internal.h
+++ b/piano_a2s_amd/csrc/a2s_internal.h
@@ -46,6 +46,14 @@
 bool a2s_tallk_wgrad_ok(int M, int Np, int K, long ldp, long lda, long ldg, int transposed, const void* P, const void* A, const void* G, const void* bias);
 int a2s_tallk_wgrad_impl(hipStream_t st, int M, int Np, int K, const float* P, long ldp, const float* A, long lda, float* G, long ldg, int transposed,
     float* bias, const float* p_absmax, const float* a_absmax, float* ws, size_t ws_bytes);
+extern int a2s_tallk_shared_planes;
+extern int a2s_tallk_pair_blocks;
+extern int a2s_tallk_split_div;
+size_t a2s_tallk_planes_bytes_impl(int M, int Np);
+size_t a2s_tallk_packed_ws_bytes_impl(int M, int Np, int K);
+int a2s_tallk_pack_impl(hipStream_t st, int M, int Np, const float* P, long ldp, const float* p_absmax, void* planes, size_t planes_bytes);
+int a2s_tallk_wgrad_packed_impl(hipStream_t st, int M, int K, const void* planes, int planes_blocks, int first_block, int nblocks, const float* A, long lda,
+    float* G, long ldg, int transposed, float* bias, const float* p_absmax, const float* a_absmax, float* ws, size_t ws_bytes);
 
 int a2s_act_bound_impl(hipStream_t st, const float* scale, const float* shift, const float* absmax, int C, float* out);
 size_t a2s_conv3x3_workspace_floats_impl(int Cin);
diff --git a/piano_a2s_amd/csrc/a2s_linear.hip b/piano_a2s_amd/csrc/a2s_linear.hip
--- a/piano_a2s_amd/csrc/a2s_linear.hip
+++ b/piano_a2s_amd/csrc/a2s_linear.hip
@@ -395,12 +395,13 @@
     *reinterpret_cast<lu32x4*>(o + 64 * 16) = lo;
 }
 
-template <bool BIAS>
+template <bool BIAS, int NPB>
 __global__ __launch_bounds__(LIN_NTH) void lin_wgrad_roles(LinWgradArgs a) {
+    constexpr int NU = 2 / NPB;
     __shared__ __attribute__((aligned(16))) unsigned char lds[LF_NS * LF_STAGE];
     const int tid = threadIdx.x, lane = tid & 63, lr = lane & 15, lk = lane >> 4;
     const int wave = __builtin_amdgcn_readfirstlane(tid >> 6);
-    const int k0 = blockIdx.x * LIN_BM;
+    const int k0 = blockIdx.x * (LIN_BM / NPB);
     const int b_lo = blockIdx.y * a.blk_per_split, b_hi = min(a.nblk, b_lo + a.blk_per_split);
     const int ka = a.a_absmax ? pow2_scale_exp(*a.a_absmax, 12) : 0, kd = pow2_scale_exp(*a.d_absmax, 12);
     const float psa = ldexpf(1.f, ka), unscale = ldexpf(1.f, -(ka + kd));
@@ -408,18 +409,20 @@
     if (wave >= 4) {
         const int st_ = tid - 256;
         const int rq = st_ & 15, cq0 = st_ >> 4;
-        float sc[2], sh[2];
-#pragma unroll
-        for (int u = 0; u < 2; ++u) {
+        float sc[NU], sh[NU];
+#pragma unroll
+        for (int u = 0; u < NU; ++u) {
             const int ch = affine ? (k0 + 4 * (cq0 + 16 * u)) / a.period : 0;
             sc[u] = affine ? a.a_scale[ch] * psa : psa; sh[u] = affine ? a.a_shift[ch] * psa : 0.f;
         }
         const float floor_ = affine ? 0.f : -INFINITY;
-        f32x4 ar[2][8];
-        f32x4 bs[2] = {(f32x4){0.f, 0.f, 0.f, 0.f}, (f32x4){0.f, 0.f, 0.f, 0.f}};
-        auto issue_a = [&](int blk, f32x4 (&r)[8]) {
-#pragma unroll
-            for (int u = 0; u < 2; ++u)
+        f32x4 ar[2][4 * NU];
+        f32x4 bs[NU];
+#pragma unroll
+        for (int u = 0; u < NU; ++u) bs[u] = (f32x4){0.f, 0.f, 0.f, 0.f};
+        auto issue_a = [&](int blk, f32x4 (&r)[4 * NU]) {
+#pragma unroll
+            for (int u = 0; u < NU; ++u)
 #pragma unroll
                 for (int j = 0; j < 4; ++j) {
                     const int m = blk * 64 + 4 * rq + j;
@@ -427,19 +430,19 @@
                     if (m < a.M && blk < b_hi) r[4 * u + j] = __builtin_nontemporal_load(reinterpret_cast<const f32x4*>(a.A + (long)m * a.lda + k0 + 4 * (cq0 + 16 * u)));
                 }
         };
-        auto commit_a = [&](int blk, const f32x4 (&r)[8]) {
+        auto commit_a = [&](int blk, const f32x4 (&r)[4 * NU]) {
             if (blk >= b_hi) return;
             unsigned char* st = lds + (blk % LF_NS) * LF_STAGE;
             if (BIAS) {
 #pragma unroll
-                for (int u = 0; u < 2; ++u)
+                for (int u = 0; u < NU; ++u)
 #pragma unroll
                     for (int j = 0; j < 4; ++j)
 #pragma unroll
                         for (int c = 0; c < 4; ++c) bs[u][c] += r[4 * u + j][c];
             }
 #pragma unroll
-            for (int u = 0; u < 2; ++u)
+            for (int u = 0; u < NU; ++u)
 #pragma unroll
                 for (int c = 0; c < 4; ++c) {
                     float x[4];
@@ -468,7 +471,7 @@
         }
         if (BIAS && blockIdx.z == 0) {
 #pragma unroll
-            for (int u = 0; u < 2; ++u) {
+            for (int u = 0; u < NU; ++u) {
 #pragma unroll
                 for (int c = 0; c < 4; ++c)
 #pragma unroll
@@ -479,9 +482,10 @@
         return;
     }
     lu32x4 df[2][4][2];
-    const unsigned char* planes = a.planes + blockIdx.z * a.plane_stride;
-    auto load_d = [&](int step, lu32x4 (&dst)[4][2]) {
+    const unsigned char* planes0 = a.planes + (long)blockIdx.z * NPB * a.plane_stride;
+    auto load_d = [&](int step, int z, lu32x4 (&dst)[4][2]) {
         if (step >= 2 * b_hi) return;
+        const unsigned char* planes = planes0 + z * a.plane_stride;
 #pragma unroll
         for (int nt = 0; nt < 4; ++nt)
 #pragma unroll
@@ -517,7 +521,7 @@
         LW_PRODUCT(1, 0) LW_PRODUCT(0, 1) LW_PRODUCT(0, 0)
 #undef LW_PRODUCT
     };
-    load_d(2 * b_lo, df[0]);
+    load_d(2 * b_lo, 0, df[0]);
 #pragma unroll 1
     for (int blk = b_lo; blk < b_hi; ++blk) {
         const bool want = ((2 * blk) >> 3) & 1;
@@ -525,29 +529,54 @@
         __syncthreads();
         const unsigned char* st = lds + (blk % LF_NS) * LF_STAGE;
         lu32x4 fa[2][2], fb[2][2];
-        load_bf(st, 0, 0, fa);
-        load_d(2 * blk + 1, df[1]);
-        __builtin_amdgcn_sched_barrier(0);
-        load_bf(st, 0, 1, fb); multiply(0, fa, df[0]);
-        __builtin_amdgcn_sched_barrier(0);
-        load_bf(st, 0, 2, fa); multiply(1, fb, df[0]);
-        __builtin_amdgcn_sched_barrier(0);
-        load_bf(st, 0, 3, fb); multiply(2, fa, df[0]);
-        __builtin_amdgcn_sched_barrier(0);
-        load_bf(st, 1, 0, fa); multiply(3, fb, df[0]);
-        __builtin_amdgcn_sched_barrier(0);
-        load_d(2 * blk + 2, df[0]);
-        load_bf(st, 1, 1, fb); multiply(0, fa, df[1]);
-        __builtin_amdgcn_sched_barrier(0);
-        load_bf(st, 1, 2, fa); multiply(1, fb, df[1]);
-        __builtin_amdgcn_sched_barrier(0);
-        load_bf(st, 1, 3, fb); multiply(2, fa, df[1]);
-        __builtin_amdgcn_sched_barrier(0);
-        multiply(3, fb, df[1]);
-        __builtin_amdgcn_sched_barrier(0);
+        if constexpr (NPB == 1) {
+            load_bf(st, 0, 0, fa);
+            load_d(2 * blk + 1, 0, df[1]);
+            __builtin_amdgcn_sched_barrier(0);
+            load_bf(st, 0, 1, fb); multiply(0, fa, df[0]);
+            __builtin_amdgcn_sched_barrier(0);
+            load_bf(st, 0, 2, fa); multiply(1, fb, df[0]);
+            __builtin_amdgcn_sched_barrier(0);
+            load_bf(st, 0, 3, fb); multiply(2, fa, df[0]);
+            __builtin_amdgcn_sched_barrier(0);
+            load_bf(st, 1, 0, fa); multiply(3, fb, df[0]);
+            __builtin_amdgcn_sched_barrier(0);
+            load_d(2 * blk + 2, 0, df[0]);
+            load_bf(st, 1, 1, fb); multiply(0, fa, df[1]);
+            __builtin_amdgcn_sched_barrier(0);
+            load_bf(st, 1, 2, fa); multiply(1, fb, df[1]);
+            __builtin_amdgcn_sched_barrier(0);
+            load_bf(st, 1, 3, fb); multiply(2, fa, df[1]);
+            __builtin_amdgcn_sched_barrier(0);
+            multiply(3, fb, df[1]);
+            __builtin_amdgcn_sched_barrier(0);
+        } else {
+            load_bf(st, 0, 0, fa);
+            load_d(2 * blk, 1, df[1]);
+            __builtin_amdgcn_sched_barrier(0);
+            load_bf(st, 0, 1, fb); multiply(0, fa, df[0]);
+            __builtin_amdgcn_sched_barrier(0);
+            load_bf(st, 0, 0, fa); multiply(1, fb, df[0]);
+            __builtin_amdgcn_sched_barrier(0);
+            load_d(2 * blk + 1, 0, df[0]);
+            load_bf(st, 0, 1, fb); multiply(2, fa, df[1]);
+            __builtin_amdgcn_sched_barrier(0);
+            load_bf(st, 1, 0, fa); multiply(3, fb, df[1]);
+            __builtin_amdgcn_sched_barrier(0);
+            load_d(2 * blk + 1, 1, df[1]);
+            load_bf(st, 1, 1, fb); multiply(0, fa, df[0]);
+            __builtin_amdgcn_sched_barrier(0);
+            load_bf(st, 1, 0, fa); multiply(1, fb, df[0]);
+            __builtin_amdgcn_sched_barrier(0);
+            load_d(2 * blk + 2, 0, df[0]);
+            load_bf(st, 1, 1, fb); multiply(2, fa, df[1]);
+            __builtin_amdgcn_sched_barrier(0);
+            multiply(3, fb, df[1]);
+            __builtin_amdgcn_sched_barrier(0);
+        }
     }
     if (neg) flip();
-    float* slab = a.partial + ((long)blockIdx.y * a.np + blockIdx.z * 256) * a.K;
+    float* slab = a.partial + ((long)blockIdx.y * a.np + blockIdx.z * NPB * 256) * a.K;
 #pragma unroll
     for (int kt = 0; kt < 8; ++kt)
 #pragma unroll
@@ -555,7 +584,8 @@
             f32x4 v = acc[kt][nt];
 #pragma unroll
             for (int r = 0; r < 4; ++r) v[r] *= unscale;
-            *reinterpret_cast<f32x4*>(slab + (long)(wave * 64 + nt * 16 + lr) * a.K + k0 + kt * 16 + lk * 4) = v;
+            const int zb = NPB == 1 ? 0 : kt >> 2, kc = NPB == 1 ? kt : kt & 3;
+            *reinterpret_cast<f32x4*>(slab + (long)(zb * 256 + wave * 64 + nt * 16 + lr) * a.K + k0 + kc * 16 + lk * 4) = v;
         }
 }
 
@@ -623,7 +653,7 @@
     hipLaunchKernelGGL(lin_pack_dz_planes, dim3((unsigned)(((long)nsteps * 1024 + 255) / 256)), dim3(256), 0, st, dz, ldz, M, nsteps, dz_absmax, planes);
     A2S_CHECK_LAUNCH("lin_pack_dz_planes");
     LinWgradArgs a{A, lda, planes, partial, a_scale, a_shift, a_absmax, dz_absmax, M, K, a_scale ? period : K, nblk, (nblk + splits - 1) / splits, 0, 256, nullptr};
-    hipLaunchKernelGGL(lin_wgrad_roles<false>, dim3(K / LIN_BM, splits), dim3(LIN_NTH), 0, st, a);
+    hipLaunchKernelGGL((lin_wgrad_roles<false, 1>), dim3(K / LIN_BM, splits), dim3(LIN_NTH), 0, st, a);
     A2S_CHECK_LAUNCH("lin_wgrad");
     const long n = 256L * K;
     hipLaunchKernelGGL(lin_wgrad_reduce<false>, dim3((unsigned)((n / 4 + 255) / 256)), dim3(256), 0, st, partial, splits, n, G, ldg, K, nullptr, nullptr);
@@ -636,6 +666,10 @@
 int a2s_tallk_wgrad_max_splits = 0;
 static long long g_tallk_launches = 0;
 long a2s_tallk_wgrad_launches(void) { return (long)__atomic_load_n(&g_tallk_launches, __ATOMIC_RELAXED); }
+
+int a2s_tallk_shared_planes = 1;
+int a2s_tallk_pair_blocks = 1;
+int a2s_tallk_split_div = 1;
 
 static int tallk_splits(int M, int Np, int K) {
     const int tiles = (K / LIN_BM) * (Np / 256), nblk = (M + 63) / 64;
@@ -644,6 +678,7 @@
     int s = cus / tiles;
     const size_t slab = (size_t)Np * K * sizeof(float);
     if ((size_t)s * slab > TALLK_SLAB_BYTES) s = (int)(TALLK_SLAB_BYTES / slab);
+    if (a2s_tallk_split_div > 1) s /= a2s_tallk_split_div;
     if (s > nblk) s = nblk;
     if (a2s_tallk_wgrad_max_splits > 0 && s > a2s_tallk_wgrad_max_splits) s = a2s_tallk_wgrad_max_splits;
     return s < 1 ? 1 : s;
@@ -652,29 +687,56 @@
     return a2s_tallk_wgrad_on && M >= 64 && Np >= 256 && Np % 256 == 0 && Np <= 2048 && K >= LIN_BM && K % LIN_BM == 0 && K <= 4096 && ldp >= Np && lda >= K &&
            lda % 4 == 0 && ldg % 4 == 0 && ldg >= (transposed ? Np : K) && (((uintptr_t)P | (uintptr_t)A | (uintptr_t)G | (uintptr_t)bias) % 16 == 0);
 }
+static size_t tallk_plane_stride(int M) { return 2 * (size_t)((M + 63) / 64) * 16 * 2 * 1024; }
+size_t a2s_tallk_planes_bytes_impl(int M, int Np) {
+    if (M < 1 || Np < 256 || Np % 256) return 0;
+    return (size_t)(Np / 256) * tallk_plane_stride(M);
+}
+size_t a2s_tallk_packed_ws_bytes_impl(int M, int Np, int K) {
+    if (M < 1 || Np < 256 || Np % 256 || K < LIN_BM || K % LIN_BM) return 0;
+    const size_t splits = (size_t)tallk_splits(M, Np, K);
+    return splits * Np * K * sizeof(float) + splits * K * sizeof(float);
+}
 size_t a2s_tallk_wgrad_ws_bytes_impl(int M, int Np, int K) {
     if (M < 1 || Np < 256 || Np % 256 || K < LIN_BM || K % LIN_BM) return 0;
-    const size_t nsteps = 2 * (size_t)((M + 63) / 64), splits = (size_t)tallk_splits(M, Np, K);
-    return (size_t)(Np / 256) * nsteps * 16 * 2 * 1024 + splits * Np * K * sizeof(float) + splits * K * sizeof(float);
-}
-int a2s_tallk_wgrad_impl(hipStream_t st, int M, int Np, int K, const float* P, long ldp, const float* A, long lda, float* G, long ldg, int transposed,
-                         float* bias, const float* p_absmax, const float* a_absmax, float* ws, size_t ws_bytes) {
-    A2S_REQUIRE(P && A && G && p_absmax && a_absmax && ws, "tallk_wgrad: null argument");
-    A2S_REQUIRE(a2s_tallk_wgrad_ok(M, Np, K, ldp, lda, ldg, transposed, P, A, G, bias),
+    return a2s_tallk_planes_bytes_impl(M, Np) + a2s_tallk_packed_ws_bytes_impl(M, Np, K);
+}
+int a2s_tallk_pack_impl(hipStream_t st, int M, int Np, const float* P, long ldp, const float* p_absmax, void* planes, size_t planes_bytes) {
+    A2S_REQUIRE(P && p_absmax && planes, "tallk_pack: null argument");
+    A2S_REQUIRE(M >= 64 && Np >= 256 && Np % 256 == 0 && Np <= 2048 && ldp >= Np, "tallk_pack: needs M >= 64, Np %% 256 == 0, Np <= 2048, ldp >= Np");
+    A2S_REQUIRE(((uintptr_t)planes % 16 == 0) && planes_bytes >= a2s_tallk_planes_bytes_impl(M, Np), "tallk_pack: planes too small (%zu bytes needed)",
+                a2s_tallk_planes_bytes_impl(M, Np));
+    const int nsteps = 2 * ((M + 63) / 64);
+    hipLaunchKernelGGL(lin_pack_dz_planes, dim3((unsigned)(((long)nsteps * 1024 + 255) / 256), Np / 256), dim3(256), 0, st, P, ldp, M, nsteps, p_absmax,
+                       reinterpret_cast<unsigned char*>(planes));
+    A2S_CHECK_LAUNCH("lin_pack_dz_planes");
+    return A2S_OK;
+}
+int a2s_tallk_wgrad_packed_impl(hipStream_t st, int M, int K, const void* planes, int planes_blocks, int first_block, int nblocks, const float* A, long lda,
+                                float* G, long ldg, int transposed, float* bias, const float* p_absmax, const float* a_absmax, float* ws, size_t ws_bytes) {
+    A2S_REQUIRE(planes && A && G && p_absmax && a_absmax && ws, "tallk_wgrad_packed: null argument");
+    A2S_REQUIRE(first_block >= 0 && nblocks >= 1 && planes_blocks >= 1 && first_block <= planes_blocks - nblocks,
+                "tallk_wgrad_packed: blocks %d .. %d of a set of %d", first_block, first_block + nblocks - 1, planes_blocks);
+    const int Np = nblocks * 256;
+    A2S_REQUIRE(((uintptr_t)planes % 16 == 0) && a2s_tallk_wgrad_ok(M, Np, K, Np, lda, ldg, transposed, nullptr, A, G, bias),
                 "tallk_wgrad: needs M >= 64, Np %% 256 == 0, K %% 128 == 0, 16-byte aligned bases and rows (or the switch \"tallk_wgrad\" is off)");
-    A2S_REQUIRE(((uintptr_t)ws % 16 == 0) && ws_bytes >= a2s_tallk_wgrad_ws_bytes_impl(M, Np, K), "tallk_wgrad: workspace too small (%zu bytes needed)",
-                a2s_tallk_wgrad_ws_bytes_impl(M, Np, K));
-    const int nblk = (M + 63) / 64, nsteps = 2 * nblk, splits = tallk_splits(M, Np, K), npb = Np / 256;
-    const size_t plane_stride = (size_t)nsteps * 16 * 2 * 1024;
-    unsigned char* planes = reinterpret_cast<unsigned char*>(ws);
-    float* partial = reinterpret_cast<float*>(planes + npb * plane_stride);
+    A2S_REQUIRE(((uintptr_t)ws % 16 == 0) && ws_bytes >= a2s_tallk_packed_ws_bytes_impl(M, Np, K), "tallk_wgrad: workspace too small (%zu bytes needed)",
+                a2s_tallk_packed_ws_bytes_impl(M, Np, K));
+    const int nblk = (M + 63) / 64, splits = tallk_splits(M, Np, K);
+    const size_t plane_stride = tallk_plane_stride(M);
+    float* partial = ws;
     float* bias_partial = partial + (size_t)splits * Np * K;
-    hipLaunchKernelGGL(lin_pack_dz_planes, dim3((unsigned)(((long)nsteps * 1024 + 255) / 256), npb), dim3(256), 0, st, P, ldp, M, nsteps, p_absmax, planes);
-    A2S_CHECK_LAUNCH("lin_pack_dz_planes");
-    LinWgradArgs a{A, lda, planes, partial, nullptr, nullptr, a_absmax, p_absmax, M, K, K, nblk, (nblk + splits - 1) / splits, (long)plane_stride, Np,
-                   bias ? bias_partial : nullptr};
-    if (bias) hipLaunchKernelGGL(lin_wgrad_roles<true>, dim3(K / LIN_BM, splits, npb), dim3(LIN_NTH), 0, st, a);
-    else hipLaunchKernelGGL(lin_wgrad_roles<false>, dim3(K / LIN_BM, splits, npb), dim3(LIN_NTH), 0, st, a);
+    LinWgradArgs a{A, lda, reinterpret_cast<const unsigned char*>(planes) + first_block * plane_stride, partial, nullptr, nullptr, a_absmax, p_absmax, M, K, K, nblk,
+                   (nblk + splits - 1) / splits, (long)plane_stride, Np, bias ? bias_partial : nullptr};
+    if (nblocks % 2 == 0 && a2s_tallk_pair_blocks) {
+        const dim3 grid(K / (LIN_BM / 2), splits, nblocks / 2);
+        if (bias) hipLaunchKernelGGL((lin_wgrad_roles<true, 2>), grid, dim3(LIN_NTH), 0, st, a);
+        else hipLaunchKernelGGL((lin_wgrad_roles<false, 2>), grid, dim3(LIN_NTH), 0, st, a);
+    } else {
+        const dim3 grid(K / LIN_BM, splits, nblocks);
+        if (bias) hipLaunchKernelGGL((lin_wgrad_roles<true, 1>), grid, dim3(LIN_NTH), 0, st, a);
+        else hipLaunchKernelGGL((lin_wgrad_roles<false, 1>), grid, dim3(LIN_NTH), 0, st, a);
+    }
     A2S_CHECK_LAUNCH("lin_wgrad (tall-K)");
     const long n = (long)Np * K, nthreads = (n + (bias ? K : 0)) / 4;
     const dim3 rgrid((unsigned)((nthreads + 255) / 256));
@@ -684,3 +746,15 @@
     __atomic_fetch_add(&g_tallk_launches, 1LL, __ATOMIC_RELAXED);
     return A2S_OK;
 }
+int a2s_tallk_wgrad_impl(hipStream_t st, int M, int Np, int K, const float* P, long ldp, const float* A, long lda, float* G, long ldg, int transposed,
+                         float* bias, const float* p_absmax, const float* a_absmax, float* ws, size_t ws_bytes) {
+    A2S_REQUIRE(P && A && G && p_absmax && a_absmax && ws, "tallk_wgrad: null argument");
+    A2S_REQUIRE(a2s_tallk_wgrad_ok(M, Np, K, ldp, lda, ldg, transposed, P, A, G, bias),
+                "tallk_wgrad: needs M >= 64, Np %% 256 == 0, K %% 128 == 0, 16-byte aligned bases and rows (or the switch \"tallk_wgrad\" is off)");
+    A2S_REQUIRE(((uintptr_t)ws % 16 == 0) && ws_bytes >= a2s_tallk_wgrad_ws_bytes_impl(M, Np, K), "tallk_wgrad: workspace too small (%zu bytes needed)",
+                a2s_tallk_wgrad_ws_bytes_impl(M, Np, K));
+    const size_t pb = a2s_tallk_planes_bytes_impl(M, Np);
+    if (int e = a2s_tallk_pack_impl(st, M, Np, P, ldp, p_absmax, ws, pb)) return e;
+    return a2s_tallk_wgrad_packed_impl(st, M, K, ws, Np / 256, 0, Np / 256, A, lda, G, ldg, transposed, bias, p_absmax, a_absmax,
+                                       reinterpret_cast<float*>(reinterpret_cast<unsigned char*>(ws) + pb), ws_bytes - pb);
+}
diff --git a/piano_a2s_amd/engine_bwd.py b/piano_a2s_amd/engine_bwd.py
--- a/piano_a2s_amd/engine_bwd.py
+++ b/piano_a2s_amd/engine_bwd.py
@@ -535,6 +535,31 @@
     gws = [hip.gemm_workspace(B, dev), hip.gemm_workspace(B, dev)]
     two_term = True
     in_amax = hip.absmax(es["layers"][0]["in"]) if two_term else None
+    shared = bool(two_term and L.a2s_debug_get(b"tallk_wgrad") > 0 and L.a2s_debug_get(b"tallk_shared_planes") > 0)
+    l0, l1 = es["layers"]
+    assert l1["in"].data_ptr() == l0["out"].data_ptr() and l1["in"].shape[1] == 2 * H, "layer 1 reads layer 0's output in place"
+    packed = {}
+
+    def planes_of(which):
+        if not shared:
+            return None
+        if which not in packed:
+            if which == "in0":
+                packed[which] = hip.tallk_pack(l0["in"], 0, l0["in"].shape[1], B * T, l0["in"].shape[1], in_amax)
+            else:
+                t = (l0 if which == "out0" else l1)["out"]
+                packed[which] = hip.tallk_pack(t, 0, 2 * H, B * T, 2 * H, hip.one(dev)) if H % 256 == 0 else None
+        return packed[which]
+
+    if shared:
+        wg = _weight_grad_stream(dev)
+        ev = torch.cuda.Event()
+        ev.record()
+        wg.wait_event(ev)
+        in_amax.record_stream(wg)
+        with torch.cuda.stream(wg):
+            for which in ("out1", "out0", "in0"):
+                planes_of(which)
     dout = dEnc
     for layer in (1, 0):
         ls = es["layers"][layer]
@@ -585,13 +610,18 @@
             with torch.cuda.stream(wg):
                 dgi2, dghs2 = dgi.view(B * T, 3 * H), dghs.view(B * T, 3 * H)
                 x_bound = ((in_amax if layer == 0 else hip.one(dev)) if two_term else None)
-                if not hip.tallk_wgrad(inp, 0, I, dgi2, 0, 3 * H, G[f"encoder.gru.weight_ih_{sfx}"], 0, I, B * T, I, 3 * H, x_bound, dgi_amax[d],
-                                       transposed=True, bias=G[f"encoder.gru.bias_ih_{sfx}"]):
+                p_in, p_out = planes_of("in0" if layer == 0 else "out0"), planes_of(f"out{layer}")
+                if not (hip.tallk_wgrad_packed(p_in, 0, p_in.blocks, dgi2, 0, 3 * H, G[f"encoder.gru.weight_ih_{sfx}"], 0, I, 3 * H, dgi_amax[d],
+                                               transposed=True, bias=G[f"encoder.gru.bias_ih_{sfx}"]) if p_in is not None else
+                        hip.tallk_wgrad(inp, 0, I, dgi2, 0, 3 * H, G[f"encoder.gru.weight_ih_{sfx}"], 0, I, B * T, I, 3 * H, x_bound, dgi_amax[d],
+                                        transposed=True, bias=G[f"encoder.gru.bias_ih_{sfx}"])):
                     _linear_bwd(inp, S[f"encoder.gru.weight_ih_{sfx}"], dgi2, G, f"encoder.gru.weight_ih_{sfx}", f"encoder.gru.bias_ih_{sfx}",
                                 dy_amax=dgi_amax[d], x_bound=x_bound)
                 dghs_amax = (ranges[1:2] if ranges is not None else hip.absmax(dghs2)) if two_term else None
-                if not hip.tallk_wgrad(out, d * H, 2 * H, dghs2, 0, 3 * H, G[f"encoder.gru.weight_hh_{sfx}"], 0, H, B * T, H, 3 * H,
-                                       hip.one(dev) if two_term else None, dghs_amax, transposed=True, bias=G[f"encoder.gru.bias_hh_{sfx}"]):
+                if not (hip.tallk_wgrad_packed(p_out, d * H // 256, H // 256, dghs2, 0, 3 * H, G[f"encoder.gru.weight_hh_{sfx}"], 0, H, 3 * H, dghs_amax,
+                                               transposed=True, bias=G[f"encoder.gru.bias_hh_{sfx}"]) if p_out is not None else
+                        hip.tallk_wgrad(out, d * H, 2 * H, dghs2, 0, 3 * H, G[f"encoder.gru.weight_hh_{sfx}"], 0, H, B * T, H, 3 * H,
+                                        hip.one(dev) if two_term else None, dghs_amax, transposed=True, bias=G[f"encoder.gru.bias_hh_{sfx}"])):
                     sk = L.a2s_gemm_pick_splitk(3 * H, H, B * T, 1)
                     hip.gemm(dghs2, 1, 3 * H, out, 2 * H, 1, G[f"encoder.gru.weight_hh_{sfx}"], H, 3 * H, H, B * T, beta=1.0, splitk=sk, b_off=d * H,
                              two_term=(dghs_amax, hip.one(dev)) if two_term else None)
diff --git a/piano_a2s_amd/hip.py b/piano_a2s_amd/hip.py
--- a/piano_a2s_amd/hip.py
+++ b/piano_a2s_amd/hip.py
@@ -701,6 +701,42 @@
     return True
 
 
+class TallkPlanes:
+    __slots__ = ("buf", "M", "blocks", "p_absmax")
+
+    def __init__(self, buf, M, blocks, p_absmax):
+        self.buf, self.M, self.blocks, self.p_absmax = buf, M, blocks, p_absmax
+
+
+def tallk_pack(P, p_off, ldp, M, Np, p_absmax):
+    L = lib()
+    pp = P.data_ptr() + 4 * p_off
+    if (not hasattr(L, "a2s_tallk_pack") or p_absmax is None or pp % 16 or L.a2s_debug_get(b"tallk_wgrad") <= 0
+            or M < 64 or Np < 256 or Np % 256 or Np > 2048 or ldp < Np):
+        return None
+    nb = L.a2s_tallk_planes_bytes(M, Np)
+    buf = torch.empty((nb + 3) // 4, dtype=torch.float32, device=P.device)
+    check(L.a2s_tallk_pack(stream(), M, Np, C.c_void_p(pp), ldp, _p(p_absmax), _p(buf), buf.numel() * 4), "a2s_tallk_pack")
+    return TallkPlanes(buf, M, Np // 256, p_absmax)
+
+
+def tallk_wgrad_packed(planes, first_block, nblocks, A, a_off, lda, G, g_off, ldg, K, a_absmax, transposed=False, bias=None):
+    L = lib()
+    M, Np = planes.M, 256 * nblocks
+    pa, pg = A.data_ptr() + 4 * a_off, G.data_ptr() + 4 * g_off
+    if (a_absmax is None or (pa | pg | (bias.data_ptr() if bias is not None else 0)) % 16
+            or not L.a2s_tallk_wgrad_eligible(M, Np, K, Np, lda, ldg, int(transposed))):
+        return False
+    nb = L.a2s_tallk_wgrad_packed_ws_bytes(M, Np, K)
+    key = (A.device, torch.cuda.current_stream().cuda_stream, threading.get_ident())
+    ws = _TALLK_WS.get(key)
+    if ws is None or ws.numel() * 4 < nb:
+        ws = _TALLK_WS[key] = torch.empty((nb + 3) // 4, dtype=torch.float32, device=A.device)
+    check(L.a2s_tallk_wgrad_packed(stream(), M, K, _p(planes.buf), planes.blocks, first_block, nblocks, C.c_void_p(pa), lda, C.c_void_p(pg), ldg, int(transposed),
+                                   _p(bias), _p(planes.p_absmax), _p(a_absmax), _p(ws), ws.numel() * 4), "a2s_tallk_wgrad_packed")
+    return True
+
+
 def linear_forward_for_test(x, w, aff):
     period = aff[2]
     xmax = x.view(x.shape[0], -1, period).abs().amax(dim=(0, 2)).contiguous()
```

Measured after the change: 635.4, median of 4. No clear change (+0.2%).
